# tum-vision/lsd_slam

Measured on AMD Instinct MI355X. Metric: tracked frames/sec (full track+map loop) at 640x480, frames resident in HBM (8-bit upload excluded: value_pcie_inclusive has it), higher is better.
Workload: dtype f32

## Files before the change

### lsd_slam_amd/csrc/lsdhip_internal.hpp

```cpp
#pragma once
#include <hip/hip_runtime.h>
#include <cmath>
#include <cstddef>
#include <cstdint>
#include <cstdio>
#include <cstring>
#include <mutex>
#include <string>
#include <vector>
#include "../../include/lsdhip.h"

#define LSD_LEVELS LSDHIP_PYRAMID_LEVELS
#define LSD_TRACK_MIN_LEVEL 1
#define LSD_TRACK_MAX_LEVEL 5
#define LSD_QUICK_KF_CHECK_LVL 4

void lsd_set_error(const char* fmt, ...);
#define HIPCHK(expr)                                                                       \
  do {                                                                                     \
    hipError_t e_ = (expr);                                                                \
    if (e_ != hipSuccess) {                                                                \
      lsd_set_error("%s failed: %s (%s:%d)", #expr, hipGetErrorString(e_), __FILE__, __LINE__); \
      return LSDHIP_E_HIP;                                                                 \
    }                                                                                      \
  } while (0)

#include "pose_math.hpp"

#include "rcp_exact.hpp"

struct LevelIntr { float fx, fy, cx, cy, fxi, fyi, cxi, cyi; };

#define RS_NUM 48
enum {
  RS_M = 0,
  RS_GOOD, RS_BAD, RS_SUMRES2, RS_SUMSIGNED, RS_SXX, RS_SYY, RS_SX, RS_SY, RS_SW, RS_USAGE,
  RS_WERR,
  RS_A0,
  RS_B0 = RS_A0 + 21,
  RS_ERR = RS_B0 + 6,
  RS_NREF,
  RS_END,
  RS_TOP0 = RS_END
};
static_assert(RS_TOP0 + 3 <= RS_NUM, "record too small");
static_assert(RS_END <= RS_NUM, "record too small");

struct TrackLevel {
  const float* kf_idepth;
  const float* kf_idepthVar;
  const float* kf_image;
  const uint8_t* kf_refBlk;
  const float4* fr_grad;
  const float* pts_pos;
  const float* pts_colvar;
  int npts;
  int w, h;
  int nblocks;
  int singlePass;
  int tilePx;
  float fx, fy, cx, cy, fxi, fyi, cxi, cyi;
  float lambdaInitial, stepSizeMin, convergenceEps;
  int maxIts;
  float minWarped;
  int writeMask;
};

struct TrackJob {
  TrackLevel lv[LSD_LEVELS];
  uint8_t* wasGood;
  float cameraPixelNoise2, var_weight, huber_half;
  float lambdaSuccessFac, lambdaFailFac;
  int useAffine;
  int lastLevel;
  int topLevel;
  lsdm::SE3fH T0;
  float aff_a0, aff_b0;
  int evalOnly;
  int trackFrameSemantics;
};
struct TrackSpec {
  int specC;
  int specGrid;
  int trials[LSD_LEVELS];
  uint8_t* wasGoodSide;
  unsigned maskStride;
  int seq;
  int copyMask;
  unsigned long long dbgCum;
  unsigned long long* dbgCounters;
  int last;
#ifdef LSD_PHASE_TRACE
  int traceWg;
#endif
#ifdef LSD_DEVTOOLS
  int* dbgLog;
#endif
};

#define LSD_SPEC_MAX 6
struct TrackState {
  lsdm::SE3fH T;
  lsdm::SE3fH Tn;
  float R[9], t[3];
  float aff_a, aff_b, aff_a_lastIt, aff_b_lastIt;
  float lastErr, LM_lambda, last_residual;
  int level, iteration, incTry, phase;
  int pending;
  float A[36], b[6];
  float inc[6];
  float bytes;
  int done, diverged;
  int numEvaluations, numWarpUpdates;
  float pointUsage, goodCount, badCount, meanRes;
  int levelEvals[LSD_LEVELS];
  int ncand;
  int lastCand;
  int numLaunches;
};

struct TrackSummary {
  int done;
  int diverged, level, numEvaluations, numWarpUpdates, pad_[3];
  float q[4], t[3];
  float lastResidual, pointUsage, goodCount, badCount, meanRes, aff_a, aff_b, aff_a_lastIt, aff_b_lastIt;
  float sums[RS_NUM];
  double bytes;
  int levelEvals[LSD_LEVELS];
  int numLaunches;
  int lastCand;
  int seq;
  int exhausted;
  unsigned check;
};
#define LSD_SUMMARY_CHECK_WORDS (offsetof(TrackSummary, seq) / 4)
__host__ __device__ static inline unsigned lsd_summary_term(unsigned i, unsigned bits) { return bits * (2u * i + 1u); }

struct DeferredSlot { double sum, count, flag, pad; };
#define LSD_NUM_SLOTS 256
#define LSD_DEFAULT_ASYNC 0
#define LSD_DEFAULT_PIPELINE 0
#define LSD_SPEC_TRIALS_SMALL 6
#define LSD_SPEC_SMALL_PX 6144
#define LSD_SPEC_TRIALS_MID 5
#define LSD_SPEC_MID_PX 90112
#define LSD_SPEC_CAP_WORKGROUPS 80
#define LSD_SPEC_CAP_ABOVE_PX 24576
#ifndef LSD_OBS_SPLIT_MIN_MAPS
#define LSD_OBS_SPLIT_MIN_MAPS 4
#endif
#define LSD_OBS_WALK_WAVES 4096
#define LSD_BATCH_THROUGHPUT_MIN_JOBS 8
#define LSD_BATCH_SPEC_MAX 4
#define LSD_BATCH_SPEC_PIXELS 500000
#define LSD_BATCH_STRIP_WORKGROUPS 768
struct lsdhip_frame;

#define LSD_CTX_LOCK(c) std::lock_guard<std::recursive_mutex> lsd_ctx_lock_((c)->mtx)
struct lsdhip_ctx {
  std::recursive_mutex mtx;
  int device = 0;
  bool async = LSD_DEFAULT_ASYNC != 0;
  DeferredSlot* h_slots = nullptr;
  lsdhip_frame* slot_stats_owner[LSD_NUM_SLOTS] = {};
  lsdhip_frame* slot_rescale_owner[LSD_NUM_SLOTS] = {};
  int slot_next = 0;
  long long enqEpoch = 0, doneEpoch = 0;
  long long slot_epoch[LSD_NUM_SLOTS] = {};
  int w = 0, h = 0;
  bool refBlocksWanted = false;
  int wl[LSD_LEVELS], hl[LSD_LEVELS];
  LevelIntr intr[LSD_LEVELS];
  float K0[9], K0inv[9];
  lsdhip_params params;
  hipStream_t stream = nullptr;
#define LSD_EVR 64
  bool pipeline = LSD_DEFAULT_PIPELINE != 0;
  hipStream_t mstream = nullptr;
  hipEvent_t mEv[LSD_EVR] = {};
  long long mSeq = 0;
  long long mDoneSeq = 0;
  long long tWaitedM = 0;
  long long slot_mseq[LSD_NUM_SLOTS] = {};
  struct PendingMerge { uint8_t* plane; const uint8_t* side; long long* doneSeq; };
  std::vector<PendingMerge> pendingMerges;
  unsigned long long* d_sums = nullptr;
  std::vector<int> sums_meta;
  std::vector<unsigned long long> sums_host;
  int* d_gate = nullptr;
  int gateSeq = 0, gateWaited = 0;
  static constexpr int MAX_LANES = 16;
  hipStream_t lanes[MAX_LANES] = {};
  hipEvent_t lane_done[MAX_LANES] = {};
  hipEvent_t lane_fork = nullptr;
  int lanes_open = 0;
  int lane_cur = -1;
  bool lane_used[MAX_LANES] = {};
  bool lane_record_pending = false;
  hipStream_t aux_stream = nullptr;
  unsigned* d_flagArrive = nullptr;
  hipEvent_t aux_fork = nullptr, aux_done = nullptr;
  bool aux_active = false, aux_pending = false;
  bool prof_on = false;
  unsigned prof_tick = 0;
  hipEvent_t ev_a = nullptr, ev_b = nullptr;
  bool prof_pending = false;
  double prof_ms = 0, prof_bytes = 0;
  long long prof_launches = 0;
  std::vector<hipEvent_t> prof_events;
#define LSD_BPROF_KINDS 5
#define LSD_BPROF_SLOTS 16
#define LSD_BPROF_PERIOD 3
  struct BProfSlot { hipEvent_t a = nullptr, b = nullptr; int kind = -1; double units = 0; bool pending = false; } bprof[LSD_BPROF_SLOTS];
  int bprof_next = 0;
  unsigned bprof_tick[LSD_BPROF_KINDS] = {};
  double bprof_ms[LSD_BPROF_KINDS] = {}, bprof_units[LSD_BPROF_KINDS] = {};
  long long bprof_calls[LSD_BPROF_KINDS] = {};
  unsigned long long* d_obsBatchAcc = nullptr;
  std::vector<void*> free_arenas;
  size_t arena_keep = 16;
  float* d_gtStage = nullptr;
  uint8_t* d_kfPoints = nullptr;
  struct ArgRing {
    static constexpr int NS = 32;
    uint8_t* h = nullptr; uint8_t* d = nullptr; size_t slotBytes = 0; int next = 0; hipEvent_t ev[NS] = {}; bool used[NS] = {};
    int cur = -1; size_t curBytes = 0;
    unsigned long long serial = 0, gen = 0;
  } args;
  struct BatchForm {
    int n = 0, py = 0, nSet = 0, walkWorkgroups = 0;
    bool split = false, candidates = false, synced = false;
    const int* qcountDev = nullptr;
    unsigned long long argsSerial = 0, argsGen = 0;
  } batchForm[2];
  std::vector<struct lsdhip_depthmap*> depthmaps;
  size_t arena_bytes = 0;
};

struct lsdhip_frame {
  lsdhip_ctx* ctx = nullptr;
  int id = 0;
  uint8_t* d_gray = nullptr;
  float* d_image[LSD_LEVELS] = {};
  float4* d_grad[LSD_LEVELS] = {};
  float* d_absgrad = nullptr;
  float* d_maxgrad = nullptr;
  float* d_idepth[LSD_LEVELS] = {};
  float* d_idepthVar[LSD_LEVELS] = {};
  bool hasIDepth = false;
  bool level0Ready = false;
  uint16_t* d_gradCand = nullptr;
  float gradCandTh = -1.0f;
  float* d_idepthW[LSD_LEVELS] = {};
  float* d_idepthVarW[LSD_LEVELS] = {};
  bool depthPending = false;
  long long depthPendingSeq = 0;
  long long depthSeq = 0;
  long long readySeq = 0;
  unsigned depthVersion = 0;
  uint8_t* d_refBlk[LSD_LEVELS] = {};
  uint8_t* d_refBlkW[LSD_LEVELS] = {};
  bool refBlkValid = false, refBlkValidW = false;
  uint8_t* d_wasGood = nullptr;
  bool wasGoodValid = false;
  bool wasGoodPristine = false;
  lsdm::Sim3dH thisToParent_raw;
  lsdhip_frame* trackingParent = nullptr;
  int trackingParentID = -1;
  float initialTrackedResidual = 0;
  int numFramesTrackedOnThis = 0, numMappedOnThis = 0, numMappedOnThisTotal = 0;
  float meanIdepth = 1;
  int numPoints = 0;
  int pendStats = -1;
  int pendRescale = -1;
  bool depthHasBeenUpdatedFlag = false;
  float* d_idepth_reAct = nullptr;
  float* d_idepthVar_reAct = nullptr;
  uint8_t* d_validity_reAct = nullptr;
  bool reActValid = false;
};

struct lsdhip_tracker {
  lsdhip_ctx* ctx = nullptr;
  float lambdaSuccessFac = 0.5f, lambdaFailFac = 2.0f;
  float lambdaInitial[LSD_LEVELS], stepSizeMin[LSD_LEVELS], convergenceEps[LSD_LEVELS];
  int maxItsPerLvl[LSD_LEVELS];
  float lambdaInitialTestTrack = 0, stepSizeMinTestTrack = 1e-3, convergenceEpsTestTrack = 0.98, maxItsTestTrack = 5;
  float huber_d = 3, var_weight = 1.0;
  float pointUsage = 0, lastGoodCount = 0, lastMeanRes = 0, lastBadCount = 0, lastResidual = 0;
  float affineEstimation_a = 1, affineEstimation_b = 0, affineEstimation_a_lastIt = 1, affineEstimation_b_lastIt = 0;
  bool diverged = false, trackingWasGood = false;
  int numEvaluations = 0, numWarpUpdates = 0;
  void (*enqueueHook)(void*) = nullptr;
  void* enqueueHookUser = nullptr;
  bool spinWait = true;
  bool hostLM = false;
  float* d_partials = nullptr;
  int max_blocks = 0;
  TrackState* d_state = nullptr;
  int levelEvaluations[LSD_LEVELS] = {};
  int block = 256;
  int grid_cap = 304;
  int recent[4] = {0, 0, 0, 0};
  int specC = 6;
  int soloMinJobs = -1;
  bool specAuto = true;
  int specCaps[LSD_LEVELS] = {0, 0, 0, 0, 0};
  int specLevel[LSD_LEVELS] = {0, 0, 0, 0, 0};
  int specCap = LSD_SPEC_CAP_WORKGROUPS;
  uint8_t* d_maskSide = nullptr;
  int maskSet = 0;
  long long maskMergeSeq[2] = {0, 0};
  size_t maskStride = 0;
  int numLaunches = 0;
  long long sumPolled = 0, sumLate = 0, sumLateMaxNs = 0, sumLateWords = 0;
  int sumLateFirstWord = -1, sumLateLastWord = -1;
  unsigned long long dbgCum = 0;
  std::vector<unsigned> dumpL0;
  unsigned long long* d_dbg = nullptr;
#ifdef LSD_DEVTOOLS
  int* d_log = nullptr;
  std::vector<int> lastLog;
#endif
  TrackSpec spec = {};
  const lsdhip_frame* jobKf = nullptr;
  unsigned jobKfVersion = 0;
  int jobTag = 0, launchOrdinal = 0;
  int budgetExtra = 2;
  int budgetFixed = 0;
  long long dbgJobs = 0, dbgEnqueued = 0, dbgMisses = 0, dbgWaitNs = 0, dbgLaunchNs = 0;
  TrackSummary* h_summary = nullptr;
  TrackSummary* d_summary = nullptr;
  unsigned long long* d_trace = nullptr;
  int batch_capacity = 0;
  TrackJob* d_bjobs = nullptr;
  TrackJob* h_bjobs = nullptr;
  TrackState* d_bstate = nullptr;
  float* d_bscratch = nullptr;
  int batchRecent[4] = {0, 0, 0, 0};
  int batchTag = 1;
  TrackSummary* h_bsummary = nullptr;
  float* d_pts = nullptr;
  int pts_capacity = 0;
};

#ifdef __HIP_DEVICE_COMPILE__
#define LSD_G __attribute__((address_space(1)))
#else
#define LSD_G
#endif
template <typename T> __host__ __device__ inline LSD_G T* lsd_g(T* p) { return (LSD_G T*)p; }
struct HypPlanes {
  LSD_G uint8_t* valid;
  LSD_G int32_t* blacklisted;
  LSD_G float* nextID;
  LSD_G int32_t* validity;
  LSD_G float* idepth;
  LSD_G float* var;
  LSD_G float* idepth_s;
  LSD_G float* var_s;
};

struct StereoRef {
  LSD_G const float* image;
  LSD_G const uint8_t* wasGood;
  int parentIsKF;
  int id;
  float initialTrackedResidual;
  float K_otherToThis_R[9];
  float K_otherToThis_t[3];
  float otherToThis_t[3];
  float thisToOther_t[3];
  float row0[3], row1[3], row2[3];
};

struct lsdhip_depthmap {
  lsdhip_ctx* ctx = nullptr;
  HypPlanes cur;
  HypPlanes oth;
  uint8_t* d_validSnap = nullptr;
  void* bases[3] = {nullptr, nullptr, nullptr};
  lsdhip_frame* activeKeyFrame = nullptr;
  bool activeKeyFrameIsReactivated = false;
  char* h_stage = nullptr;
  char* d_stage = nullptr;
  size_t stage_bytes = 0;
  int* d_slotCount = nullptr;
  int* d_slots = nullptr;
  int* d_ovfHead = nullptr;
  int2* d_ovf = nullptr;
  float4* d_cand = nullptr;
  int* d_flags = nullptr;
  double* d_red = nullptr;
  size_t redStride = 0;
  bool propClean = false;
  bool lowGradHypPossible = true;
  double* h_red = nullptr;
  hipEvent_t ev[8][2] = {};
  int ev_kind[8] = {};
  bool ev_pending[8] = {};
  int ev_next = 0;
  unsigned long long* d_obs_trace = nullptr;
  size_t obs_trace_words = 0;
  double gpu_ms[4] = {0, 0, 0, 0};
  long long gpu_calls[4] = {0, 0, 0, 0};
  unsigned obs_tick = 0;
  unsigned long long* d_obsCounters = nullptr;
  unsigned long long* d_obsAcc = nullptr;
  int obsCounterWaves = 0;
  float4* d_obsQueue = nullptr;
  unsigned ev_tick[3] = {0, 0, 0};
  float msUpdate = 0, msCreate = 0, msFinalize = 0, msObserve = 0, msRegularize = 0, msPropagate = 0, msFillHoles = 0,
        msSetDepth = 0;
};

inline hipStream_t lsd_transport_stream(lsdhip_ctx* c) { return c->aux_active ? c->aux_stream : c->stream; }
inline hipStream_t lsd_map_stream(lsdhip_ctx* c) { return c->lane_cur >= 0 ? c->lanes[c->lane_cur] : (c->pipeline ? c->mstream : c->stream); }
int lsd_m_begin(lsdhip_ctx* c);
long long lsd_m_record(lsdhip_ctx* c);
int lsd_t_wait_m(lsdhip_ctx* c, long long seq);
bool lsd_m_done(lsdhip_ctx* c, long long seq);
int lsd_sync_all(lsdhip_ctx* c);
struct LsdDevBuf {
  void* p = nullptr;
  ~LsdDevBuf() { if (p) (void)hipFree(p); }
};
#ifdef LSD_DEVTOOLS
int lsd_gate_wait(lsdhip_ctx* c);
int lsd_gate_open(lsdhip_ctx* c);
int lsd_pipe_dummy(lsdhip_ctx* c);
void lsd_trace_sum(lsdhip_ctx* c, hipStream_t s, int kind, int id, const void* p, size_t bytes);
void lsd_trace_val(lsdhip_ctx* c, int kind, int id, unsigned long long v);
#else
inline int lsd_gate_wait(lsdhip_ctx*) { return LSDHIP_OK; }
inline int lsd_gate_open(lsdhip_ctx*) { return LSDHIP_OK; }
inline int lsd_pipe_dummy(lsdhip_ctx*) { return LSDHIP_OK; }
inline void lsd_trace_sum(lsdhip_ctx*, hipStream_t, int, int, const void*, size_t) {}
inline void lsd_trace_val(lsdhip_ctx*, int, int, unsigned long long) {}
#endif
inline float** lsd_depth_w(lsdhip_frame* f) { return f->ctx->pipeline ? f->d_idepthW : f->d_idepth; }
inline float** lsd_depthvar_w(lsdhip_frame* f) { return f->ctx->pipeline ? f->d_idepthVarW : f->d_idepthVar; }
inline uint8_t** lsd_refblk_w(lsdhip_frame* f) { return f->ctx->pipeline ? f->d_refBlkW : f->d_refBlk; }
inline int lsd_gradcand_groups(int pixels) { return (pixels + 1023) >> 10; }
inline size_t lsd_gradcand_bytes(int pixels) { return ((size_t)lsd_gradcand_groups(pixels) * 1024 + (size_t)lsd_gradcand_groups(pixels)) * 2; }
inline int lsd_refblk_blocks(int pixels) { return (pixels + 255) >> 8; }
inline size_t lsd_refblk_bytes(int pixels) { return (size_t)lsd_refblk_blocks(pixels) * (256 + 4); }
inline float** lsd_depth_latest(lsdhip_frame* f) { return f->depthPending ? f->d_idepthW : f->d_idepth; }
inline float** lsd_depthvar_latest(lsdhip_frame* f) { return f->depthPending ? f->d_idepthVarW : f->d_idepthVar; }
int lsd_frame_publish_depth(lsdhip_frame* f);
int lsd_flush_merges(lsdhip_ctx* c);
struct LsdTrackJobScope {
  lsdhip_ctx* c;
  int rc = LSDHIP_OK;
  bool drain;
  LsdTrackJobScope(lsdhip_ctx* c_, bool waitAll) : c(c_), drain(waitAll) { if (c->pipeline && waitAll) rc = lsd_t_wait_m(c, c->mSeq); }
  ~LsdTrackJobScope() { if (c->pipeline && drain) (void)hipStreamSynchronize(c->stream); }
};
int lsd_frame_build_pyramids(lsdhip_frame* f, const uint8_t* src, hipStream_t stream);
int lsd_frames_require_ref_blocks(lsdhip_frame** kfs, int n, hipStream_t stream);
int lsd_frames_require_level0(lsdhip_frame** fs, int n);
int lsd_frame_require_level0(lsdhip_frame* f);
int lsd_frame_require_level0_for_tracking(lsdhip_frame* f);
int lsd_args_push(lsdhip_ctx* c, const void* src, size_t bytes, hipStream_t s, void** dev_out);
int lsd_args_begin(lsdhip_ctx* c, size_t bytes, void** host_out, void** dev_out);
int lsd_args_commit(lsdhip_ctx* c, hipStream_t s);
int lsd_args_release(lsdhip_ctx* c, const void* dev, hipStream_t s);
int lsd_frame_build_idepth_pyramid_batch(lsdhip_frame** f, int n, const double* const* redPartials, int redN, double* const* redOut,
                                         const int* redNs = nullptr);
int lsd_frame_build_idepth_pyramid(lsdhip_frame* f, const double* redPartials = nullptr, int redN = 0, double* redOut = nullptr);
int lsd_frame_ensure_depth_planes(lsdhip_frame* f);
int lsd_frame_ensure_wasgood(lsdhip_frame* f);
void lsd_depthmaps_forget_frame(lsdhip_ctx* c, lsdhip_frame* f);
int lsd_prof_collect(lsdhip_ctx* c);
int lsd_bprof_begin(lsdhip_ctx* c, int kind, hipStream_t s);
int lsd_bprof_end(lsdhip_ctx* c, int slot, hipStream_t s, double units);
int lsd_frame_resolve(lsdhip_frame* f);
int lsd_ctx_take_slot(lsdhip_ctx* c);
int lsd_ctx_claim_stats_slot(lsdhip_ctx* c, lsdhip_frame* f);
int lsd_ctx_claim_rescale_slot(lsdhip_ctx* c, lsdhip_frame* f);
```

### lsd_slam_amd/csrc/track_device.hpp

```cpp
#pragma once
#include "lsdhip_internal.hpp"
#include <type_traits>

template <int CTRL, int ROW_MASK, int BANK_MASK>
__device__ __forceinline__ float dpp_f(float v) {
  return __builtin_bit_cast(float, __builtin_amdgcn_update_dpp(0, __builtin_bit_cast(int, v), CTRL, ROW_MASK, BANK_MASK, true));
}
__device__ __forceinline__ int dpp_max_i(int a, int b) { return a > b ? a : b; }
template <int CTRL, int ROW_MASK, int BANK_MASK>
__device__ __forceinline__ int dpp_i(int v) {
  return __builtin_amdgcn_update_dpp(-1, v, CTRL, ROW_MASK, BANK_MASK, false);
}
template <int CTRL, int ROW_MASK, int BANK_MASK>
__device__ __forceinline__ int dpp_i0(int v) {
  return __builtin_amdgcn_update_dpp(0, v, CTRL, ROW_MASK, BANK_MASK, true);
}
__device__ __forceinline__ int wave_max_to_lane63(int v) {
  int t = dpp_max_i(v, dpp_i<0x111, 0xf, 0xf>(v));
  t = dpp_max_i(t, dpp_i<0x112, 0xf, 0xf>(v));
  t = dpp_max_i(t, dpp_i<0x113, 0xf, 0xf>(v));
  t = dpp_max_i(t, dpp_i<0x114, 0xf, 0xe>(t));
  t = dpp_max_i(t, dpp_i<0x118, 0xf, 0xc>(t));
  t = dpp_max_i(t, dpp_i<0x142, 0xa, 0xf>(t));
  t = dpp_max_i(t, dpp_i<0x143, 0xc, 0xf>(t));
  return t;
}
__device__ __forceinline__ float wave_sum_to_lane63(float v) {
  float t = v + dpp_f<0x111, 0xf, 0xf>(v);
  t = t + dpp_f<0x112, 0xf, 0xf>(v);
  t = t + dpp_f<0x113, 0xf, 0xf>(v);
  t = t + dpp_f<0x114, 0xf, 0xe>(t);
  t = t + dpp_f<0x118, 0xf, 0xc>(t);
  t = t + dpp_f<0x142, 0xa, 0xf>(t);
  t = t + dpp_f<0x143, 0xc, 0xf>(t);
  return t;
}

__device__ __forceinline__ void block_top3(int c0, int c1, int c2, int (*s_wave)[3], int* s_out) {
  const int tid = threadIdx.x, wave = tid >> 6, lane = tid & 63;
#pragma unroll
  for (int r = 0; r < 3; r++) {
    int m = __builtin_amdgcn_readlane(wave_max_to_lane63(c0), 63);
    if (lane == 0) s_wave[wave][r] = m;
    if (c0 == m && m >= 0) { c0 = c1; c1 = c2; c2 = -1; }
  }
  __syncthreads();
  if (wave == 0) {
    const int nw = blockDim.x >> 6;
    int v = (lane < nw * 3) ? s_wave[lane / 3][lane % 3] : -1;
#pragma unroll
    for (int r = 0; r < 3; r++) {
      int m = __builtin_amdgcn_readlane(wave_max_to_lane63(v), 63);
      if (lane == 0) s_out[r] = m;
      if (v == m) v = -1;
    }
  }
  __syncthreads();
}
__device__ __forceinline__ constexpr int tri_index(int r, int c) { return RS_A0 + r * 6 - (r * (r - 1)) / 2 + (c - r); }

__device__ __forceinline__ void top3_insert(int k, int& c0, int& c1, int& c2) {
  const int n0 = max(c0, k);
  int t = min(c0, k);
  const int n1 = max(c1, t);
  t = min(c1, t);
  c2 = max(c2, t);
  c1 = n1;
  c0 = n0;
}

typedef const __attribute__((address_space(1))) float gfloat;
typedef float v4f __attribute__((ext_vector_type(4)));
typedef const __attribute__((address_space(1))) v4f gv4f;
typedef __attribute__((address_space(1))) uint8_t gbyte;
struct EvalCtx {
  gfloat* kf_idepth;
  gfloat* kf_idepthVar;
  gfloat* kf_image;
  gfloat* fr_grad;
  gfloat* pts_pos;
  gfloat* pts_colvar;
  int npts, w, h;
  float fx, fy, cx, cy, fxi, fyi, cxi, cyi;
  float R[9], t[3];
  float aff_a, aff_b;
  float cameraPixelNoise2, var_weight, huber_half;
};
struct PointOut {
  bool in_image;
  bool good;
  float res, c1, c2, hw;
  float usage;
  float werr;
  float w;
  float J[6];
};

struct PointWarp { float Wx, Wy, Wz, u_new, v_new; bool in_image; };
struct Texel3 { float x, y, z; };
struct PointTexels { Texel3 t00, t10, t01, t11; };
__device__ __forceinline__ void eval_warp(const EvalCtx& a, float px, float py, float pz, PointWarp& q) {
  q.Wx = ((a.R[0] * px + a.R[1] * py) + a.R[2] * pz) + a.t[0];
  q.Wy = ((a.R[3] * px + a.R[4] * py) + a.R[5] * pz) + a.t[1];
  q.Wz = ((a.R[6] * px + a.R[7] * py) + a.R[8] * pz) + a.t[2];
  q.u_new = (q.Wx / q.Wz) * a.fx + a.cx;
  q.v_new = (q.Wy / q.Wz) * a.fy + a.cy;
  q.in_image = (q.u_new > 1 && q.v_new > 1 && q.u_new < a.w - 2 && q.v_new < a.h - 2);
}
__device__ __forceinline__ void eval_fetch(const EvalCtx& a, const PointWarp& q, bool fetch, PointTexels& t) {
  const int ix = fetch ? (int)q.u_new : 0;
  const int iy = fetch ? (int)q.v_new : 0;
  gfloat* bp = a.fr_grad + 4 * (ix + __mul24(iy, a.w));
  auto ld = [](gfloat* f) { Texel3 r = {f[0], f[1], f[2]}; return r; };
  t.t00 = ld(bp); t.t10 = ld(bp + 4); t.t01 = ld(bp + 4 * a.w); t.t11 = ld(bp + 4 + 4 * a.w);
}
#ifndef LSD_EVAL_FMA
#define LSD_EVAL_FMA 1
#endif
__device__ __forceinline__ float frcp(float x) { return __builtin_amdgcn_rcpf(x); }
__device__ __forceinline__ float fsqrt(float x) { return __builtin_amdgcn_sqrtf(x); }
__device__ __forceinline__ void eval_finish(const EvalCtx& a, const PointWarp& q, const PointTexels& t, float pz, float I_ref, float var,
                                            PointOut& o) {
  const float Wx = q.Wx, Wy = q.Wy, Wz = q.Wz, u_new = q.u_new, v_new = q.v_new;
  const Texel3 t00 = t.t00, t10 = t.t10, t01 = t.t01, t11 = t.t11;
  int ix = (int)u_new;
  int iy = (int)v_new;
  float dx = u_new - ix;
  float dy = v_new - iy;
  float dxdy = dx * dy;
  float w11 = dxdy, w01 = dy - dxdy, w10 = dx - dxdy, w00 = 1 - dx - dy + dxdy;
  float rx = w11 * t11.x + w01 * t01.x + w10 * t10.x + w00 * t00.x;
  float ry = w11 * t11.y + w01 * t01.y + w10 * t10.y + w00 * t00.y;
  float rz = w11 * t11.z + w01 * t01.z + w10 * t10.z + w00 * t00.z;

  float c1 = a.aff_a * I_ref + a.aff_b;
  float c2 = rz;
  float residual = c1 - c2;
  o.res = residual; o.c1 = c1; o.c2 = c2;
  o.hw = fabsf(residual) < 5.0f ? 1 : 5.0f * frcp(fabsf(residual));
  o.good = residual * residual < (40.0f * 40.0f + 0.5f * 0.5f * (rx * rx + ry * ry));
  float gx = a.fx * rx;
  float gy = a.fy * ry;
  float d = frcp(pz);
  float z = frcp(Wz);
  float depthChange = pz * z;
  o.usage = depthChange < 1 ? depthChange : 1;

  float pz2d = frcp((Wz * Wz) * d);
#if LSD_EVAL_FMA
  float g0 = __builtin_fmaf(Wz, a.t[0], 0.0f - Wx * a.t[2]) * pz2d;
  float g1 = __builtin_fmaf(Wz, a.t[1], 0.0f - Wy * a.t[2]) * pz2d;
  float drpdd = __builtin_fmaf(g0, gx, g1 * gy);
  float w_p = frcp(__builtin_fmaf(drpdd, drpdd * (a.var_weight * var), a.cameraPixelNoise2));
#else
  float g0 = (Wz * a.t[0] - Wx * a.t[2]) * pz2d;
  float g1 = (Wz * a.t[1] - Wy * a.t[2]) * pz2d;
  float drpdd = g0 * gx + g1 * gy;
  float w_p = frcp(a.cameraPixelNoise2 + drpdd * (drpdd * (a.var_weight * var)));
#endif
  float wr = residual * fsqrt(w_p);
  wr = fmaxf(wr, 0.0f - wr);
  float wh = (wr < a.huber_half) ? 1.0f : a.huber_half * frcp(wr);
  o.werr = wh * (wr * wr);
  o.w = wh * w_p;

  o.J[0] = z * gx;
  o.J[1] = z * gy;
  float v1 = (Wx * gy) * z;
  float v2 = (Wy * gx) * z;
  o.J[5] = v1 - v2;
  float z2 = z * z;
  v1 = (Wx * gx) * z2;
  v2 = (Wy * gy) * z2;
  o.J[2] = 0.0f - (v1 + v2);
#if LSD_EVAL_FMA
  o.J[3] = 0.0f - __builtin_fmaf(v2, Wy, __builtin_fmaf(v1, Wy, gy));
  o.J[4] = __builtin_fmaf(v2, Wx, __builtin_fmaf(v1, Wx, gx));
#else
  o.J[3] = 0.0f - ((v2 * Wy) + (gy + v1 * Wy));
  o.J[4] = (gx + v1 * Wx) + v2 * Wx;
#endif
}
__device__ __forceinline__ void eval_point(const EvalCtx& a, float px, float py, float pz, float I_ref, float var, PointOut& o) {
  PointWarp q;
  eval_warp(a, px, py, pz, q);
  o.in_image = q.in_image;
  if (!o.in_image) return;
  PointTexels t;
  eval_fetch(a, q, true, t);
  eval_finish(a, q, t, pz, I_ref, var, o);
}

__device__ __forceinline__ bool fetch_point(const EvalCtx& a, int i, float& px, float& py, float& pz, float& I_ref,
                                            float& var, int& maskIdx) {
  if (a.npts >= 0) {
    if (i >= a.npts) return false;
    px = a.pts_pos[3 * i]; py = a.pts_pos[3 * i + 1]; pz = a.pts_pos[3 * i + 2];
    I_ref = a.pts_colvar[2 * i]; var = a.pts_colvar[2 * i + 1];
    maskIdx = -1;
    return true;
  }
  if (i >= a.w * a.h) return false;
  int x = i % a.w, y = i / a.w;
  if (x < 1 || x >= a.w - 1 || y < 1 || y >= a.h - 1) return false;
  var = a.kf_idepthVar[i];
  float id = a.kf_idepth[i];
  if (var <= 0 || id == 0) return false;
  float inv = lsd_rcp_exact(id);
  px = inv * (a.fxi * x + a.cxi);
  py = inv * (a.fyi * y + a.cyi);
  pz = inv * 1.0f;
  I_ref = a.kf_image[i];
  maskIdx = i;
  return true;
}

__device__ __forceinline__ void set_eval_pose(TrackState& s, const lsdm::SE3fH& T) {
  s.Tn = T;
  lsdm::quatf_to_rot(T.q, s.R);
  s.t[0] = T.t[0]; s.t[1] = T.t[1]; s.t[2] = T.t[2];
}
__device__ __forceinline__ float rl(float v, int l) { return __int_as_float(__builtin_amdgcn_readlane(__float_as_int(v), l)); }
__device__ __forceinline__ int rli(int v, int l) { return __builtin_amdgcn_readlane(v, l); }

__device__ __forceinline__ void gj6_solve_wave(const float* A , const float* bvec , const float damp, float* s_m ,
                                               const int lane, float (&x)[6]) {
  const int i = lane >> 3, j = lane & 7;
  const bool act = i < 6 && j < 7;
  const int ii = act ? i : 0, jj = act ? (j < 6 ? j : 0) : 0;
  float m = (j == 6) ? -bvec[ii] : A[ii * 6 + jj];
  if (i == j) m *= damp;
#pragma unroll
  for (int k = 0; k < 6; k++) {
    if (act) s_m[i * 8 + j] = m;
    __builtin_amdgcn_fence(__ATOMIC_RELEASE, "wavefront");
    __builtin_amdgcn_wave_barrier();
    __builtin_amdgcn_fence(__ATOMIC_ACQUIRE, "wavefront");
    const float d = s_m[k * 8 + k], rk = s_m[k * 8 + (act ? j : 0)], ck = s_m[ii * 8 + k];
    const float f = ck * frcp(d);
    const float upd = m - f * rk;
    m = (i == k || d == 0.0f) ? m : upd;
    __builtin_amdgcn_wave_barrier();
  }
  if (act) s_m[i * 8 + j] = m;
  __builtin_amdgcn_fence(__ATOMIC_RELEASE, "wavefront");
  __builtin_amdgcn_wave_barrier();
  __builtin_amdgcn_fence(__ATOMIC_ACQUIRE, "wavefront");
#pragma unroll
  for (int r = 0; r < 6; r++) {
    const float d = s_m[r * 8 + r];
    x[r] = d != 0.0f ? s_m[r * 8 + 6] * frcp(d) : 0.0f;
  }
}

__device__ __forceinline__ void sincos_small(const float xx, float* sn, float* cs) {
  if (fabsf(xx) < 0.5f) {
    const float x2 = xx * xx;
    *sn = xx * (1.0f + x2 * (-1.0f / 6.0f + x2 * (1.0f / 120.0f + x2 * (-1.0f / 5040.0f + x2 * (1.0f / 362880.0f + x2 * (-1.0f / 39916800.0f))))));
    *cs = 1.0f + x2 * (-0.5f + x2 * (1.0f / 24.0f + x2 * (-1.0f / 720.0f + x2 * (1.0f / 40320.0f + x2 * (-1.0f / 3628800.0f + x2 * (1.0f / 479001600.0f))))));
  } else {
    sincosf(xx, sn, cs);
  }
}

__device__ __forceinline__ void q_normalize_wave(lsdm::Quatf& q, const int lane) {
  const float rn = __builtin_amdgcn_rsqf(q.x * q.x + q.y * q.y + q.z * q.z + q.w * q.w);
  const float c = (lane & 3) == 0 ? q.w : ((lane & 3) == 1 ? q.x : ((lane & 3) == 2 ? q.y : q.z));
  const float r = c * rn;
  q.w = rl(r, 0); q.x = rl(r, 1); q.y = rl(r, 2); q.z = rl(r, 3);
}

__device__ __forceinline__ lsdm::SE3fH se3f_exp_wave(const float (&a)[6], const int lane) {
  const float eps = static_cast<float>(1e-5);
  const float ox = a[3], oy = a[4], oz = a[5];
  const float theta_sq = ox * ox + (oy * oy + oz * oz);
  const float theta = fsqrt(theta_sq);
  const float half_theta = 0.5f * theta;
  float sn, cs;
  sincos_small((lane & 1) ? theta : half_theta, &sn, &cs);
  const float sin_half = rl(sn, 0), cos_half = rl(cs, 0), sin_theta = rl(sn, 1), cos_theta = rl(cs, 1);
  float imag, real;
  if (theta < eps) {
    const float theta_po4 = theta_sq * theta_sq;
    imag = 0.5f - static_cast<float>(1.0 / 48.0) * theta_sq + static_cast<float>(1.0 / 3840.0) * theta_po4;
    real = 1.0f - 0.5f * theta_sq + static_cast<float>(1.0 / 384.0) * theta_po4;
  } else {
    imag = sin_half * frcp(theta);
    real = cos_half;
  }
  lsdm::SE3fH r;
  r.q = {real, imag * ox, imag * oy, imag * oz};
  q_normalize_wave(r.q, lane);
  const float Om[9] = {0, -oz, oy, oz, 0, -ox, -oy, ox, 0};
  float Om2[9];
#pragma unroll
  for (int i = 0; i < 3; i++)
#pragma unroll
    for (int j = 0; j < 3; j++) {
      float acc = Om[i * 3 + 0] * Om[0 * 3 + j];
      acc += Om[i * 3 + 1] * Om[1 * 3 + j];
      acc += Om[i * 3 + 2] * Om[2 * 3 + j];
      Om2[i * 3 + j] = acc;
    }
  float V[9];
  if (theta < eps) {
    lsdm::q_to_rot<lsdm::Quatf, float>(r.q, V);
  } else {
    const float tsq = theta * theta;
    const float ca = (1.0f - cos_theta) * frcp(tsq);
    const float cb = (theta - sin_theta) * frcp(tsq * theta);
#pragma unroll
    for (int i = 0; i < 9; i++) V[i] = (((i % 4) == 0 ? 1.0f : 0.0f) + ca * Om[i]) + cb * Om2[i];
  }
#pragma unroll
  for (int i = 0; i < 3; i++) {
    float acc = V[i * 3 + 0] * a[0];
    acc += V[i * 3 + 1] * a[1];
    acc += V[i * 3 + 2] * a[2];
    r.t[i] = acc;
  }
  return r;
}
__device__ __forceinline__ lsdm::SE3fH se3f_mul_wave(const lsdm::SE3fH& a, const lsdm::SE3fH& b, const int lane) {
  lsdm::SE3fH r = a;
  float rt[3];
  lsdm::q_rotate<lsdm::Quatf, float>(a.q, b.t, rt);
#pragma unroll
  for (int i = 0; i < 3; i++) r.t[i] = a.t[i] + rt[i];
  r.q = lsdm::q_mul(a.q, b.q);
  q_normalize_wave(r.q, lane);
  return r;
}

__device__ __forceinline__ void write_summary(const TrackState& s, const float* tot, TrackSummary* out, const int doneWord) {
  unsigned chk = (unsigned)doneWord;
#define SUM_PUT_I(field, value) do { const int v_ = (value); out->field = v_; chk += lsd_summary_term((unsigned)(offsetof(TrackSummary, field) / 4), (unsigned)v_); } while (0)
#define SUM_PUT_F(field, value) do { const float v_ = (value); out->field = v_; chk += lsd_summary_term((unsigned)(offsetof(TrackSummary, field) / 4), __float_as_uint(v_)); } while (0)
#define SUM_PUT_IA(field, i, value) do { const int v_ = (value); out->field[i] = v_; chk += lsd_summary_term((unsigned)(offsetof(TrackSummary, field) / 4 + (i)), (unsigned)v_); } while (0)
#define SUM_PUT_FA(field, i, value) do { const float v_ = (value); out->field[i] = v_; chk += lsd_summary_term((unsigned)(offsetof(TrackSummary, field) / 4 + (i)), __float_as_uint(v_)); } while (0)
  SUM_PUT_I(diverged, s.diverged); SUM_PUT_I(level, s.level); SUM_PUT_I(numEvaluations, s.numEvaluations); SUM_PUT_I(numWarpUpdates, s.numWarpUpdates);
  SUM_PUT_IA(pad_, 0, 0); SUM_PUT_IA(pad_, 1, 0); SUM_PUT_IA(pad_, 2, 0);
  SUM_PUT_FA(q, 0, s.T.q.w); SUM_PUT_FA(q, 1, s.T.q.x); SUM_PUT_FA(q, 2, s.T.q.y); SUM_PUT_FA(q, 3, s.T.q.z);
  SUM_PUT_FA(t, 0, s.T.t[0]); SUM_PUT_FA(t, 1, s.T.t[1]); SUM_PUT_FA(t, 2, s.T.t[2]);
  SUM_PUT_F(lastResidual, s.last_residual); SUM_PUT_F(pointUsage, s.pointUsage); SUM_PUT_F(goodCount, s.goodCount); SUM_PUT_F(badCount, s.badCount);
  SUM_PUT_F(meanRes, s.meanRes); SUM_PUT_F(aff_a, s.aff_a); SUM_PUT_F(aff_b, s.aff_b); SUM_PUT_F(aff_a_lastIt, s.aff_a_lastIt); SUM_PUT_F(aff_b_lastIt, s.aff_b_lastIt);
  for (int i = 0; i < RS_NUM; i++) SUM_PUT_FA(sums, i, tot[i]);
  {
    const double b = (double)s.bytes;
    out->bytes = b;
    const unsigned long long u = (unsigned long long)__double_as_longlong(b);
    chk += lsd_summary_term((unsigned)(offsetof(TrackSummary, bytes) / 4), (unsigned)u) + lsd_summary_term((unsigned)(offsetof(TrackSummary, bytes) / 4 + 1), (unsigned)(u >> 32));
  }
  for (int l = 0; l < LSD_LEVELS; l++) SUM_PUT_IA(levelEvals, l, s.levelEvals[l]);
  SUM_PUT_I(numLaunches, s.numLaunches);
  SUM_PUT_I(lastCand, s.lastCand);
#undef SUM_PUT_I
#undef SUM_PUT_F
#undef SUM_PUT_IA
#undef SUM_PUT_FA
  out->check = chk;
  __threadfence_system();
  out->done = doneWord;
}

struct LmShared {
  float gj[48];
  float tot[RS_NUM];
};
struct LmPar {
  float lambdaInitial, stepSizeMin, convergenceEps, minWarped, lambdaSuccessFac, lambdaFailFac;
  int maxIts, w, h, writeMask, evalOnly, useAffine, tfSemantics, lastLevel, trials;
};
__device__ __forceinline__ void stage_lm_par(const TrackJob& job, int level, LmPar& p, const int trials = 1) {
  const TrackLevel& L = job.lv[level];
  LmPar v;
  v.lambdaInitial = L.lambdaInitial; v.stepSizeMin = L.stepSizeMin; v.convergenceEps = L.convergenceEps; v.minWarped = L.minWarped;
  v.lambdaSuccessFac = job.lambdaSuccessFac; v.lambdaFailFac = job.lambdaFailFac;
  v.maxIts = L.maxIts; v.w = L.w; v.h = L.h; v.writeMask = L.writeMask; v.evalOnly = job.evalOnly; v.useAffine = job.useAffine;
  v.tfSemantics = job.trackFrameSemantics; v.lastLevel = job.lastLevel;
  v.trials = trials;
  p = v;
}

#ifdef LSD_PHASE_TRACE
#define LM_MARK(k) do { if (trp && lane == 0) trp[k] = clock64(); } while (0)
#else
#define LM_MARK(k) do { } while (0)
#endif
__device__ __forceinline__ float lm_werr(float sumWeightedErr, int M) { return sumWeightedErr * frcp((float)((M >> 2) << 2)); }
__device__ __forceinline__ float lm_lambda_fail(float LM_lambda, int incTry, float lambdaFailFac) {
  if (LM_lambda == 0) return 0.2f;
  double p = 1.0;
  for (int i = 0; i < incTry; i++) p *= (double)lambdaFailFac;
  return (float)((double)LM_lambda * p);
}
template <bool SPEC = false>
__device__ __forceinline__ bool lm_wave(const LmPar& par, TrackState& S, const float col, float* tot, const int lane,
                                        TrackSummary* out, unsigned long long* trp, const int consumed = 0, const int mycand = 0, const int doneWord = 1) {
  float* const s_gj = tot - 48;
  S.lastCand = consumed;
  S.ncand = 1;
  const LmPar L = par;
  const int maxIts = L.maxIts;
  const int M = (int)rl(col, RS_M);
  const float refNum = rl(col, RS_NREF);
  const float goodCount = rl(col, RS_GOOD), badCount = rl(col, RS_BAD);
  float aff_a_lastIt, aff_b_lastIt;
  {
    const float sxx = rl(col, RS_SXX), syy = rl(col, RS_SYY), sx = rl(col, RS_SX), sy = rl(col, RS_SY), sw = rl(col, RS_SW);
    const float isw = frcp(sw);
    aff_a_lastIt = fsqrt((syy - sy * sy * isw) * frcp(sxx - sx * sx * isw));
    aff_b_lastIt = (sy - aff_a_lastIt * sx) * isw;
  }
  S.pointUsage = rl(col, RS_USAGE) * frcp(refNum);
  S.goodCount = goodCount;
  S.badCount = badCount;
  S.meanRes = rl(col, RS_SUMSIGNED) * frcp(goodCount);
  S.aff_a_lastIt = aff_a_lastIt;
  S.aff_b_lastIt = aff_b_lastIt;
  S.numEvaluations = S.numEvaluations + 1;
  if (lane == 0) S.levelEvals[S.level] = S.levelEvals[S.level] + 1;
  {
    const float N = refNum, wh = (float)L.w * (float)L.h;
    const float texels = 4.0f * N < wh ? 4.0f * N : wh;
    S.bytes = S.bytes + (20.0f * N + (L.writeMask ? 5.0f * N : 0.0f) + 12.0f * texels);
  }
  S.pending = 0;
  LM_MARK(12);
  if (L.evalOnly) { S.done = 1; if (out && lane == 0) write_summary(S, tot, out, doneWord); return false; }

  if (M < L.minWarped) {
    S.diverged = 1; S.done = 1;
    if (out && lane == 0) write_summary(S, tot, out, doneWord);
    return false;
  }
  const float werr = lm_werr(rl(col, RS_WERR), M);
  const bool useAffine = L.useAffine != 0;
  const bool tfSemantics = L.tfSemantics != 0;

  float LM_lambda = S.LM_lambda, lastErr = S.lastErr;
  int iteration = S.iteration, incTry = S.incTry;
  lsdm::SE3fH T = S.T;
  bool propose = false, start_iteration = false, accepted = false, rejected = false;
  if (S.phase == 0) {
    accepted = true;
    lastErr = werr;
    LM_lambda = L.lambdaInitial;
    iteration = 0;
    start_iteration = true;
  } else {
    const float error = werr;
    if (error < lastErr) {
      accepted = true;
      T = S.Tn;
      S.T = T;
      if (error > L.convergenceEps * lastErr) iteration = maxIts;
      lastErr = error;
      if (tfSemantics) S.last_residual = error;
      if (LM_lambda <= 0.2) LM_lambda = 0;
      else LM_lambda *= L.lambdaSuccessFac;
      iteration++;
      start_iteration = true;
    } else {
      const float i0 = S.inc[0], i1 = S.inc[1], i2 = S.inc[2], i3 = S.inc[3], i4 = S.inc[4], i5 = S.inc[5];
      const float incdot = (i0 * i0 + (i1 * i1 + i2 * i2)) + (i3 * i3 + (i4 * i4 + i5 * i5));
      if (!(incdot > L.stepSizeMin)) {
        iteration = maxIts;
        iteration++;
        start_iteration = true;
      } else {
        LM_lambda = lm_lambda_fail(LM_lambda, incTry, L.lambdaFailFac);
        propose = true;
        rejected = true;
      }
    }
  }
  if (accepted) {
    if (useAffine) { S.aff_a = aff_a_lastIt; S.aff_b = aff_b_lastIt; }
    const float rn = frcp((float)((size_t)6 * (size_t)(M >> 2)));
    const int k = lane - RS_A0;
    if (k >= 0 && k < 21) {
      const int i = (k >= 6) + (k >= 11) + (k >= 15) + (k >= 18) + (k >= 20);
      const int j = k - (i * 6 - (i * (i - 1)) / 2) + i;
      const float v = (0.0f + col) * rn;
      S.A[i * 6 + j] = v;
      S.A[j * 6 + i] = v;
    }
    if (lane >= RS_B0 && lane < RS_B0 + 6) S.b[lane - RS_B0] = (0.0f - col) * rn;
  }
  if (start_iteration && iteration < maxIts) { S.numWarpUpdates = S.numWarpUpdates + 1; incTry = 0; propose = true; }
  S.lastErr = lastErr;
  S.LM_lambda = LM_lambda;
  S.iteration = iteration;
  LM_MARK(13);
  if (propose) {
    const int extra = SPEC ? mycand : 0;
    for (int j = 0; j < extra; j++) { incTry++; LM_lambda = lm_lambda_fail(LM_lambda, incTry, L.lambdaFailFac); }
    S.ncand = L.trials;
    float inc[6];
    const float damp = 1 + LM_lambda;
    LM_MARK(14);
    gj6_solve_wave(S.A, S.b, damp, s_gj, lane, inc);
    LM_MARK(15);
    S.incTry = incTry + 1;
#pragma unroll
    for (int i = 0; i < 6; i++) S.inc[i] = inc[i];
    const lsdm::SE3fH Tn = se3f_mul_wave(se3f_exp_wave(inc, lane), T, lane);
    S.Tn = Tn;
    float R[9];
    lsdm::quatf_to_rot(Tn.q, R);
#pragma unroll
    for (int i = 0; i < 9; i++) S.R[i] = R[i];
    S.t[0] = Tn.t[0]; S.t[1] = Tn.t[1]; S.t[2] = Tn.t[2];
    S.phase = 1;
    LM_MARK(16);
    return true;
  }
  S.incTry = incTry;
  if (!tfSemantics) S.last_residual = lastErr;
  if (S.level == L.lastLevel) {
    S.done = 1;
    if (out && lane == 0) write_summary(S, tot, out, doneWord);
  } else {
    S.level = S.level - 1;
    S.phase = 0;
    S.Tn = T;
    float R[9];
    lsdm::quatf_to_rot(T.q, R);
#pragma unroll
    for (int i = 0; i < 9; i++) S.R[i] = R[i];
    S.t[0] = T.t[0]; S.t[1] = T.t[1]; S.t[2] = T.t[2];
  }
  return false;
}

__device__ __forceinline__ void accumulate_point(const PointOut& o, float (&acc)[RS_END]) {
  acc[RS_M] += 1.f;
  acc[RS_SXX] = __builtin_fmaf(o.c1 * o.c1, o.hw, acc[RS_SXX]);
  acc[RS_SYY] = __builtin_fmaf(o.c2 * o.c2, o.hw, acc[RS_SYY]);
  acc[RS_SX] = __builtin_fmaf(o.c1, o.hw, acc[RS_SX]);
  acc[RS_SY] = __builtin_fmaf(o.c2, o.hw, acc[RS_SY]);
  acc[RS_SW] += o.hw;
  if (o.good) { acc[RS_GOOD] += 1.f; acc[RS_SUMRES2] = __builtin_fmaf(o.res, o.res, acc[RS_SUMRES2]); acc[RS_SUMSIGNED] += o.res; }
  else acc[RS_BAD] += 1.f;
  acc[RS_USAGE] += o.usage;
  acc[RS_WERR] += o.werr;
#pragma unroll
  for (int r = 0; r < 6; r++) {
    float Jw = o.J[r] * o.w;
#pragma unroll
    for (int c = r; c < 6; c++) acc[tri_index(r, c)] = __builtin_fmaf(Jw, o.J[c], acc[tri_index(r, c)]);
  }
  float resw = o.res * o.w;
#pragma unroll
  for (int r = 0; r < 6; r++) acc[RS_B0 + r] = __builtin_fmaf(resw, o.J[r], acc[RS_B0 + r]);
  acc[RS_ERR] = __builtin_fmaf(resw, o.res, acc[RS_ERR]);
}

__device__ __forceinline__ void make_ctx_dev(const TrackJob& jobr, const TrackState& S, int level, EvalCtx& a) {
  const TrackJob* job = &jobr;
  const TrackLevel& L = job->lv[level];
  a.kf_idepth = (gfloat*)L.kf_idepth; a.kf_idepthVar = (gfloat*)L.kf_idepthVar; a.kf_image = (gfloat*)L.kf_image; a.fr_grad = (gfloat*)L.fr_grad;
  a.pts_pos = (gfloat*)L.pts_pos; a.pts_colvar = (gfloat*)L.pts_colvar; a.npts = L.npts; a.w = L.w; a.h = L.h;
  a.fx = L.fx; a.fy = L.fy; a.cx = L.cx; a.cy = L.cy; a.fxi = L.fxi; a.fyi = L.fyi; a.cxi = L.cxi; a.cyi = L.cyi;
#pragma unroll
  for (int i = 0; i < 9; i++) a.R[i] = S.R[i];
#pragma unroll
  for (int i = 0; i < 3; i++) a.t[i] = S.t[i];
  a.aff_a = S.aff_a; a.aff_b = S.aff_b;
  a.cameraPixelNoise2 = job->cameraPixelNoise2; a.var_weight = job->var_weight; a.huber_half = job->huber_half;
}

template <int N>
__device__ __forceinline__ void copy_words(void* dst, const void* src, int tid, int nthreads) {
  const unsigned* s = (const unsigned*)src;
  unsigned* d = (unsigned*)dst;
  for (int i = tid; i < N; i += nthreads) d[i] = s[i];
}

__device__ __forceinline__ int xcd_tile(int b, int nb) { return (nb & 7) == 0 ? (b & 7) * (nb >> 3) + (b >> 3) : b; }


#define RS_COLS 44
struct TrackScratch {
  float* sums;
  int4* topkey;
  float* topval;
  int max_rows;
  int cmax;
  float* recs;
#ifdef LSD_PHASE_TRACE
  unsigned long long* trace;
#endif
};
```

### lsd_slam_amd/csrc/tracker.hip

```cpp
#include <atomic>
#include <chrono>
#include "track_device.hpp"


#ifdef LSD_PHASE_TRACE
#define PHASE_MARK(k) do { if (trOn_ && threadIdx.x == 0) tr_[k] = clock64(); } while (0)
#define LSD_TRACE_WORDS 32
#else
#define PHASE_MARK(k) do { } while (0)
#endif

#ifdef LSD_DEVTOOLS
#define LAUNCH_LOG(exitCode, pendingIn, ncandIn, pcUsed) do { \
    if (!BATCH && MODE == TS_FUSED && blockIdx.x == 0 && threadIdx.x == 0 && spec.dbgLog && spec.seq != 0) { \
      int* lg_ = spec.dbgLog + ((spec.seq & 0xFFF) * 16); \
      lg_[0] = spec.seq; lg_[1] = (exitCode); lg_[2] = parity | (first << 1) | (spec.last << 2); lg_[3] = lvlIn_; lg_[4] = (pendingIn); lg_[5] = (ncandIn); \
      lg_[6] = (pcUsed); lg_[7] = S.level; lg_[8] = S.numEvaluations; lg_[9] = S.numLaunches; lg_[10] = S.done; lg_[11] = S.phase; lg_[12] = S.incTry; \
      lg_[13] = S.ncand; lg_[14] = S.pending; lg_[15] = numLaunchesIn_; } } while (0)
#else
#define LAUNCH_LOG(exitCode, pendingIn, ncandIn, pcUsed) do { } while (0)
#endif

enum { TS_FUSED = 0, TS_LM = 1, TS_EVAL = 2 };
__device__ __forceinline__ void track_state_begin(TrackState& S, const TrackJob& job, const int tid) {
  if (tid == 0) {
    S.T = job.T0;
    set_eval_pose(S, job.T0);
    S.aff_a = job.aff_a0; S.aff_b = job.aff_b0; S.aff_a_lastIt = job.aff_a0; S.aff_b_lastIt = job.aff_b0;
    S.lastErr = 0; S.LM_lambda = 0; S.last_residual = 0;
    S.level = job.topLevel; S.iteration = 0; S.incTry = 0; S.phase = 0; S.pending = 0;
    S.done = 0; S.diverged = 0; S.numEvaluations = 0; S.numWarpUpdates = 0;
    S.pointUsage = 0; S.goodCount = 0; S.badCount = 0; S.meanRes = 0;
    S.bytes = 0;
    for (int l = 0; l < LSD_LEVELS; l++) S.levelEvals[l] = 0;
    S.ncand = 1; S.lastCand = 0; S.numLaunches = 0;
  }
  if (tid < 36) S.A[tid] = 0;
  if (tid < 6) { S.b[tid] = 0; S.inc[tid] = 0; }
}
__device__ __forceinline__ void tail_row(const PointOut& o, float* row) {
  row[0] = o.werr;
  int k = 1;
#pragma unroll
  for (int rr = 0; rr < 6; rr++) {
    const float Jw = o.J[rr] * o.w;
#pragma unroll
    for (int cc = rr; cc < 6; cc++) row[k++] = Jw * o.J[cc];
  }
  const float resw = o.res * o.w;
#pragma unroll
  for (int rr = 0; rr < 6; rr++) row[k++] = resw * o.J[rr];
  row[k++] = resw * o.res;
}

template <int BLOCK, bool BATCH, int MODE>
__device__ __forceinline__ void track_step_impl(const TrackJob& jobv, const TrackJob* __restrict__ jobs, TrackState* __restrict__ st2,
                                                TrackScratch sc, TrackSummary* __restrict__ out, int parity, int first, const TrackSpec& spec) {
  const TrackJob& job = BATCH ? jobs[blockIdx.y] : jobv;
  unsigned warm = 0;
  if (!BATCH) {
    typedef const unsigned __attribute__((address_space(4))) cuint;
    cuint* ka = (cuint*)__builtin_amdgcn_kernarg_segment_ptr();
#pragma unroll
    for (int i = 0; i < (int)(sizeof(TrackJob) / 4); i += 32) warm ^= ka[i];
    asm volatile("" ::"s"(warm));
  }
  if (BATCH) {
    const size_t j = blockIdx.y, rows = (size_t)sc.max_rows, cm = (size_t)sc.cmax;
    st2 += 2 * j;
    out += j;
    sc.sums += j * 2 * cm * RS_COLS * rows;
    sc.topkey += j * 2 * cm * rows;
    sc.topval += j * 2 * cm * rows * 96;
    if (sc.recs) sc.recs += j * 2 * cm * 32;
  }
  constexpr int WAVES = BLOCK / 64;
  constexpr int SUMW = WAVES - 1;
  constexpr int NSLICE = (SUMW * 64) / RS_END;
  constexpr int QMAX = 20;
  __shared__ TrackState S;
  __shared__ LmShared sh;
  __shared__ LmPar s_par;
  constexpr int NPASS = 1;
  constexpr int CPP = (RS_END + NPASS - 1) / NPASS;
  constexpr int RSLICE_ = BLOCK / CPP;
  __shared__ float s_sum[(NSLICE > RSLICE_ ? NSLICE : RSLICE_)][64];
  __shared__ __attribute__((aligned(16))) float s_red[CPP * (BLOCK + 1) + 8];
  __shared__ int s_wtop[WAVES][3];
  __shared__ int s_top[3];
  const int tid = threadIdx.x;
  const int wave = tid >> 6, lane = tid & 63;
  const int max_rows = sc.max_rows;
  int cand = 0, bx = (int)blockIdx.x;
  const bool leader = blockIdx.x == 0;
  const int cmax = sc.cmax;
  TrackState* next = st2 + (1 - parity);
  const int outp = MODE == TS_EVAL ? parity : 1 - parity;
  const float* sums_in0 = sc.sums + (size_t)parity * cmax * RS_COLS * max_rows;
  float* sums_out = sc.sums + (size_t)outp * cmax * RS_COLS * max_rows;
  const int4* topkey_in0 = sc.topkey + (size_t)parity * cmax * max_rows;
  int4* topkey_out = sc.topkey + (size_t)outp * cmax * max_rows;
  const float* topval_in0 = sc.topval + (size_t)parity * cmax * max_rows * 96;
  float* topval_out = sc.topval + (size_t)outp * cmax * max_rows * 96;
  constexpr int NSLOT = 16;
  constexpr int TRIALS_MAX = BATCH ? (MODE == TS_EVAL ? 1 : LSD_BATCH_SPEC_MAX) : LSD_SPEC_MAX;
  constexpr bool SPEC_LM = MODE != TS_EVAL;
  static_assert(TRIALS_MAX * (NSLOT * RS_COLS + 96 + 1) <= CPP * (BLOCK + 1) + 8, "the finishing phase's tables must fit the reduction buffer");
  float (*const s_sumT)[NSLOT][RS_COLS] = (float (*)[NSLOT][RS_COLS])s_red;
  float (*const s_subT)[3][32] = (float (*)[3][32])(s_red + TRIALS_MAX * NSLOT * RS_COLS);
  int* const s_nsubT = (int*)(s_red + TRIALS_MAX * (NSLOT * RS_COLS + 96));
  __shared__ float s_rec[TRIALS_MAX][32];
#ifdef LSD_PHASE_TRACE
  __shared__ unsigned long long* s_trp;
  unsigned long long* tr_ = sc.trace;
  const bool trOn_ = sc.trace != nullptr && (int)blockIdx.x == (BATCH ? spec.traceWg : 0) && (!BATCH || blockIdx.y == 0);
  if (trOn_ && tid == 0) {
    unsigned long long n = sc.trace[0];
    sc.trace[0] = n + 1;
    tr_ = sc.trace + 1 + (n % 4096) * LSD_TRACE_WORDS;
    for (int k = 0; k < LSD_TRACE_WORDS; k++) tr_[k] = 0;
    tr_[8] = wall_clock64();
    tr_[24] = (unsigned long long)gridDim.x; tr_[25] = (unsigned long long)gridDim.y;
    s_trp = tr_;
  }
#endif
  PHASE_MARK(0);
  if (!BATCH && MODE == TS_FUSED && !first && !leader && st2[parity].done) return;
  if (!BATCH && MODE == TS_FUSED && leader && tid == 0 && spec.seq != 0) out->seq = spec.seq;
  if (first) {
    track_state_begin(S, job, tid);
  } else {
    copy_words<sizeof(TrackState) / 4>(&S, st2 + parity, tid, BLOCK);
    if (SPEC_LM && cmax > 1 && tid < 32 * TRIALS_MAX) (&s_rec[0][0])[tid] = sc.recs[(size_t)parity * cmax * 32 + (tid < 32 * cmax ? tid : 0)];
  }
  __syncthreads();
  PHASE_MARK(1);
#ifdef LSD_DEVTOOLS
  const int lvlIn_ = S.level, numLaunchesIn_ = S.numLaunches, pendingIn_ = S.pending, ncandIn_ = S.ncand;
  int pcLog_ = -1;
#endif
  if (S.done) {
    LAUNCH_LOG(1, pendingIn_, ncandIn_, -1);
    if (MODE != TS_EVAL && leader) { copy_words<sizeof(TrackState) / 4>(next, &S, tid, BLOCK); }
    return;
  }
  const int lvlPending = S.level;
  const int doneWord = (MODE == TS_FUSED && spec.seq != 0) ? (BATCH ? spec.seq : (spec.seq >> 12)) : 1;
  if (MODE == TS_FUSED) {
    const int nbl = job.lv[lvlPending].nblocks;
    const int tr = (spec.specC > 1 && spec.trials[lvlPending] > 1) ? spec.trials[lvlPending] : 1;
    cand = (int)blockIdx.x / nbl;
    bx = (int)blockIdx.x - cand * nbl;
    const bool needTrial = S.pending ? cand < tr : cand == 0;
    const bool needNext = S.pending && lvlPending > job.lastLevel && (int)blockIdx.x < job.lv[lvlPending - 1].nblocks;
    if (!leader && !needTrial && !needNext) return;
  }

  if (BATCH && MODE == TS_LM) {
    cand = (int)blockIdx.x;
    bx = 0;
    const int tr = (spec.specC > 1 && spec.trials[lvlPending] > 1) ? spec.trials[lvlPending] : 1;
    if (!leader && !(S.pending && cand < tr)) return;
  }
  if (BATCH && MODE == TS_EVAL) {
    const int nbl = job.lv[lvlPending].nblocks;
    cand = (int)blockIdx.x / nbl;
    bx = (int)blockIdx.x - cand * nbl;
  }

  constexpr int CHMAX = 8;
  int cntv = 0;
  unsigned ow[CHMAX];
  auto strip_request = [&](const int lvl, const int tile_) {
    const TrackLevel& L = job.lv[lvl];
    const int px = L.w * L.h;
    const int base_ = tile_ * L.tilePx;
    const int b0_ = base_ >> 8;
    const int mblk_ = (min(base_ + L.tilePx, px) - base_ + 255) >> 8;
    const gbyte* offs = (const gbyte*)L.kf_refBlk;
    const __attribute__((address_space(1))) int* cnts = (const __attribute__((address_space(1))) int*)(offs + ((size_t)((px + 255) >> 8) << 8));
    cntv = lane < mblk_ ? cnts[b0_ + lane] : 0;
#pragma unroll
    for (int c = 0; c < CHMAX; c++) {
      const int blk = c * 4 + wave;
      ow[c] = blk < mblk_ ? *(const __attribute__((address_space(1))) unsigned*)(offs + ((size_t)(b0_ + blk) << 8) + (lane << 2)) : 0u;
    }
  };
  bool havePre = false;
  if (BATCH && MODE == TS_FUSED && S.pending && job.lv[lvlPending].tilePx > 0) {
    const int tr = (spec.specC > 1 && spec.trials[lvlPending] > 1) ? spec.trials[lvlPending] : 1;
    havePre = cand < tr;
    if (havePre) strip_request(lvlPending, xcd_tile(bx, job.lv[lvlPending].nblocks));
  }

  if (MODE != TS_EVAL && S.pending) {
    const int ncandPending = S.ncand < 1 ? 1 : (S.ncand > TRIALS_MAX ? TRIALS_MAX : S.ncand);
    const int level = S.level;
    const int nb = job.lv[level].nblocks;
    const size_t trialStrideF4 = (size_t)RS_COLS * max_rows / 4;
      auto tail_two = [&](const int ca, const int cb, auto krn) {
        constexpr int KROWS = decltype(krn)::value;
        const int cbb = cb < 0 ? ca : cb;
        const int4* tka = topkey_in0 + (size_t)ca * max_rows;
        const int4* tkb = topkey_in0 + (size_t)cbb * max_rows;
        int4 kva[KROWS], kvb[KROWS];
#pragma unroll
        for (int q = 0; q < KROWS; q++) {
          const int row = lane + 64 * q;
          const int4 ka = tka[row < max_rows ? row : 0];
          const int4 kb = tkb[row < max_rows ? row : 0];
          kva[q] = row < nb ? ka : make_int4(-1, -1, -1, -1);
          kvb[q] = row < nb ? kb : make_int4(-1, -1, -1, -1);
        }
        auto merge = [&](const int4 (&kv)[KROWS], int (&keys)[3], int (&src)[3]) {
          int k0 = -1, k1 = -1, k2 = -1, e0 = 0, e1 = 0, e2 = 0;
#pragma unroll
          for (int q = 0; q < KROWS; q++) {
            const int e = (lane + 64 * q) * 3;
            const int ks[3] = {kv[q].x, kv[q].y, kv[q].z};
#pragma unroll
            for (int rr = 0; rr < 3; rr++) {
              const int k = ks[rr], ek = e + rr;
              const bool g0 = k > k0, g1 = k > k1, g2 = k > k2;
              k2 = g1 ? k1 : (g2 ? k : k2); e2 = g1 ? e1 : (g2 ? ek : e2);
              k1 = g0 ? k0 : (g1 ? k : k1); e1 = g0 ? e0 : (g1 ? ek : e1);
              k0 = g0 ? k : k0; e0 = g0 ? ek : e0;
            }
          }
#pragma unroll
          for (int r = 0; r < 3; r++) {
            const int m = __builtin_amdgcn_readlane(wave_max_to_lane63(k0), 63);
            const unsigned long long own = __ballot(k0 == m && m >= 0);
            const int owner = own ? (int)__ffsll((long long)own) - 1 : 0;
            keys[r] = m;
            src[r] = __builtin_amdgcn_readlane(e0, owner);
            if (k0 == m && m >= 0) { k0 = k1; e0 = e1; k1 = k2; e1 = e2; k2 = -1; }
          }
        };
        const bool single = job.lv[level].singlePass != 0 || job.lv[level].tilePx > 0;
        const int j = lane & 31, rj = lane >> 5;
        int keysA[3], srcA[3], keysB[3], srcB[3];
        float a0 = 0.f, a2 = 0.f, b0 = 0.f, b2 = 0.f;
        merge(kva, keysA, srcA);
        if (single && j < 29) {
          const float* tv = topval_in0 + (size_t)ca * max_rows * 96;
          if (keysA[rj] >= 0) a0 = tv[(size_t)srcA[rj] * 32 + j];
          if (rj == 0 && keysA[2] >= 0) a2 = tv[(size_t)srcA[2] * 32 + j];
        }
        if (cb >= 0) {
          merge(kvb, keysB, srcB);
          if (single && j < 29) {
            const float* tv = topval_in0 + (size_t)cb * max_rows * 96;
            if (keysB[rj] >= 0) b0 = tv[(size_t)srcB[rj] * 32 + j];
            if (rj == 0 && keysB[2] >= 0) b2 = tv[(size_t)srcB[2] * 32 + j];
          }
        }
        if (lane == 0) {
          s_nsubT[ca] = (keysA[0] >= 0) + (keysA[1] >= 0) + (keysA[2] >= 0);
          if (cb >= 0) s_nsubT[cb] = (keysB[0] >= 0) + (keysB[1] >= 0) + (keysB[2] >= 0);
        }
        if (single) {
          if (j < 29) {
            if (keysA[rj] >= 0) s_subT[ca][rj][j] = a0;
            if (rj == 0 && keysA[2] >= 0) s_subT[ca][2][j] = a2;
            if (cb >= 0) {
              if (keysB[rj] >= 0) s_subT[cb][rj][j] = b0;
              if (rj == 0 && keysB[2] >= 0) s_subT[cb][2][j] = b2;
            }
          }
        } else {
          const bool second = lane >= 3;
          const int r = second ? lane - 3 : lane;
          const int c = second ? cb : ca;
          int key = -1;
          if (lane < 6 && c >= 0) key = second ? (r == 0 ? keysB[0] : (r == 1 ? keysB[1] : keysB[2])) : (r == 0 ? keysA[0] : (r == 1 ? keysA[1] : keysA[2]));
          if (key >= 0) {
            EvalCtx a;
            make_ctx_dev(job, S, level, a);
            if (c > 0) {
              const float* rec = s_rec[c];
#pragma unroll
              for (int i = 0; i < 9; i++) a.R[i] = rec[13 + i];
#pragma unroll
              for (int i = 0; i < 3; i++) a.t[i] = rec[22 + i];
            }
            const int idx = (a.npts >= 0) ? key : ((key / a.h) + (key % a.h) * a.w);
            float px, py, pz, I_ref, var;
            int maskIdx;
            fetch_point(a, idx, px, py, pz, I_ref, var, maskIdx);
            PointOut o;
            eval_point(a, px, py, pz, I_ref, var, o);
            float* sub = s_subT[c][r];
            sub[0] = o.werr;
            int k = 1;
#pragma unroll
            for (int rr = 0; rr < 6; rr++) {
              float Jw = o.J[rr] * o.w;
#pragma unroll
              for (int cc = rr; cc < 6; cc++) sub[k++] = Jw * o.J[cc];
            }
            float resw = o.res * o.w;
#pragma unroll
            for (int rr = 0; rr < 6; rr++) sub[k++] = resw * o.J[rr];
            sub[k++] = resw * o.res;
          }
        }
      };
      auto tail_rows = [&](const int ca, const int cb, auto nqn) {
        constexpr int NQ = decltype(nqn)::value;
        const int cbb = cb < 0 ? ca : cb;
        const float4* ta = (const float4*)(topval_in0 + (size_t)ca * max_rows * 96);
        const float4* tb = (const float4*)(topval_in0 + (size_t)cbb * max_rows * 96);
        const int nf4 = nb * 24;
        float4 va[NQ], vb[NQ];
#pragma unroll
        for (int q = 0; q < NQ; q++) {
          const int f = q * 64 + lane;
          va[q] = ta[f < nf4 ? f : 0];
          vb[q] = tb[f < nf4 ? f : 0];
        }
        auto pick = [&](const float4 (&v)[NQ], const int c) {
          int k0 = -1, k1 = -1, k2 = -1, e0 = 0, e1 = 0, e2 = 0;
#pragma unroll
          for (int q = 0; q < NQ; q++) {
            const int f = q * 64 + lane;
            const int k = ((lane & 7) == 7 && f < nf4) ? __float_as_int(v[q].w) : -1, ek = f >> 3;
            const bool g0 = k > k0, g1 = k > k1, g2 = k > k2;
            k2 = g1 ? k1 : (g2 ? k : k2); e2 = g1 ? e1 : (g2 ? ek : e2);
            k1 = g0 ? k0 : (g1 ? k : k1); e1 = g0 ? e0 : (g1 ? ek : e1);
            k0 = g0 ? k : k0; e0 = g0 ? ek : e0;
          }
          int nsub = 0;
#pragma unroll
          for (int r = 0; r < 3; r++) {
            const int m = __builtin_amdgcn_readlane(wave_max_to_lane63(k0), 63);
            const unsigned long long own = __ballot(k0 == m && m >= 0);
            const int owner = own ? (int)__ffsll((long long)own) - 1 : 0;
            const int row = __builtin_amdgcn_readlane(e0, owner);
            if (k0 == m && m >= 0) { k0 = k1; e0 = e1; k1 = k2; e1 = e2; k2 = -1; }
            if (m >= 0) {
              nsub++;
              const int qsel = row >> 3;
#pragma unroll
              for (int q = 0; q < NQ; q++) {
                if (q == qsel) {
                  float4 w4 = v[q];
                  asm volatile("" : "+v"(w4.x), "+v"(w4.y), "+v"(w4.z), "+v"(w4.w));
                  if ((lane >> 3) == (row & 7)) *(float4*)&s_subT[c][r][(lane & 7) * 4] = w4;
                }
              }
            }
          }
          if (lane == 0) s_nsubT[c] = nsub;
        };
        pick(va, ca);
        if (cb >= 0) pick(vb, cb);
      };
    auto wave_tail = [&]() {
      const int ca = WAVES - 1 - wave;
      const int cb = ca + WAVES < ncandPending ? ca + WAVES : -1;
      if (ca < ncandPending) {
        if (BATCH && job.lv[level].tilePx > 0 && nb <= 24) {
          if (nb <= 5) tail_rows(ca, cb, std::integral_constant<int, 2>());
          else if (nb <= 13) tail_rows(ca, cb, std::integral_constant<int, 5>());
          else tail_rows(ca, cb, std::integral_constant<int, 9>());
        } else if (nb <= 128) tail_two(ca, cb, std::integral_constant<int, 2>());
        else tail_two(ca, cb, std::integral_constant<int, 5>());
      }
    };
    if (tid == SUMW * 64 - 1) stage_lm_par(job, level, s_par, (spec.specC > 1 && spec.trials[level] > 1) ? spec.trials[level] : 1);
    if (wave < SUMW) {
      const int t = tid;
      const int slot_ = t / (RS_COLS / 4);
      const bool sumLane = slot_ < NSLOT;
      const int slot = sumLane ? slot_ : 0, c4 = sumLane ? t - slot_ * (RS_COLS / 4) : 0;
      {
        const int K = (nb + NSLOT - 1) / NSLOT;
        const float4* p = (const float4*)sums_in0 + c4;
        const size_t trialStrideF4 = (size_t)RS_COLS * max_rows / 4;
        auto colsum = [&](auto qn, auto ntn, const int base) {
          constexpr int Q = decltype(qn)::value, NT = decltype(ntn)::value;
          float4 v[NT][Q];
#pragma unroll
          for (int c = 0; c < NT; c++) {
            const int pc = base + c < ncandPending ? base + c : ncandPending - 1;
            const float4* pp = p + (size_t)pc * trialStrideF4;
#pragma unroll
            for (int q = 0; q < Q; q++) {
              const int r = slot + NSLOT * q;
              v[c][q] = pp[(size_t)(r < nb ? r : slot) * (RS_COLS / 4)];
            }
          }
#pragma unroll
          for (int c = 0; c < NT; c++) {
            float4 a4 = make_float4(0.f, 0.f, 0.f, 0.f);
#pragma unroll
            for (int q = 0; q < Q; q++) {
              const bool live = q < K && slot + NSLOT * q < nb;
              a4.x += live ? v[c][q].x : 0.f;
              a4.y += live ? v[c][q].y : 0.f;
              a4.z += live ? v[c][q].z : 0.f;
              a4.w += live ? v[c][q].w : 0.f;
            }
            if (sumLane && base + c < ncandPending) *(float4*)&s_sumT[base + c][slot][c4 * 4] = a4;
          }
        };
        typedef std::integral_constant<int, 1> I1;
        typedef std::integral_constant<int, 3> I3;
        typedef std::integral_constant<int, TRIALS_MAX> IM;
        if (ncandPending == 1) {
          if (K <= 2) colsum(std::integral_constant<int, 2>(), I1(), 0);
          else if (K <= 5) colsum(std::integral_constant<int, 5>(), I1(), 0);
          else if (K <= 10) colsum(std::integral_constant<int, 10>(), I1(), 0);
          else colsum(std::integral_constant<int, QMAX>(), I1(), 0);
        } else if (K <= 2) colsum(std::integral_constant<int, 2>(), IM(), 0);
        else if (K <= 5) colsum(std::integral_constant<int, 5>(), IM(), 0);
        else if (K <= 10) { for (int base = 0; base < ncandPending; base += 3) colsum(std::integral_constant<int, 10>(), I3(), base); }
        else { for (int base = 0; base < ncandPending; base++) colsum(std::integral_constant<int, QMAX>(), I1(), base); }
#ifdef LSD_PHASE_TRACE
        if (trOn_ && tid == 0) tr_[17] = clock64();
#endif
      }
    }
    wave_tail();
#ifdef LSD_PHASE_TRACE
    if (trOn_ && tid == SUMW * 64) s_trp[18] = clock64();
#endif
    __syncthreads();
    PHASE_MARK(2);
    if (wave == 0) {
      int pc = 0;
      if (ncandPending > 1) {
        const int c = tid < ncandPending ? tid : 0;
        float Mf = s_sumT[c][0][RS_M], ws = s_sumT[c][0][RS_WERR];
#pragma unroll
        for (int k = 1; k < NSLOT; k++) { Mf += s_sumT[c][k][RS_M]; ws += s_sumT[c][k][RS_WERR]; }
        const int Mc = (int)Mf;
        int needc = Mc & 3;
        if (needc > s_nsubT[c]) needc = s_nsubT[c];
        if (needc > 0) ws -= s_subT[c][0][0];
        if (needc > 1) ws -= s_subT[c][1][0];
        if (needc > 2) ws -= s_subT[c][2][0];
        const float werrc = lm_werr(ws, Mc);
        const float* ic = c == 0 ? S.inc : s_rec[c];
        const float i0 = ic[0], i1 = ic[1], i2 = ic[2], i3 = ic[3], i4 = ic[4], i5 = ic[5];
        const float incdot = (i0 * i0 + (i1 * i1 + i2 * i2)) + (i3 * i3 + (i4 * i4 + i5 * i5));
        const bool stop = Mc < s_par.minWarped || werrc < S.lastErr || !(incdot > s_par.stepSizeMin);
        const unsigned long long sm = __ballot(stop && tid < ncandPending);
        pc = sm ? (int)__ffsll((long long)sm) - 1 : ncandPending - 1;
        if (pc > 0) {
          float lam = S.LM_lambda;
          const int it0 = S.incTry;
          for (int j = 0; j < pc; j++) lam = lm_lambda_fail(lam, it0 + j, s_par.lambdaFailFac);
          float skipped;
          {
            float NR = s_sumT[0][0][RS_NREF];
#pragma unroll
            for (int k = 1; k < NSLOT; k++) NR += s_sumT[0][k][RS_NREF];
            const float wh = (float)s_par.w * (float)s_par.h;
            const float texels = 4.0f * NR < wh ? 4.0f * NR : wh;
            skipped = 20.0f * NR + (s_par.writeMask ? 5.0f * NR : 0.0f) + 12.0f * texels;
          }
          const float* rec = s_rec[pc];
          const float bytes0 = S.bytes;
          const int ne0 = S.numEvaluations, le0 = S.levelEvals[level];
          float bytes1 = bytes0;
          for (int j = 0; j < pc; j++) bytes1 = bytes1 + skipped;
          S.LM_lambda = lam;
          S.incTry = it0 + pc;
          S.numEvaluations = ne0 + pc;
          if (tid == 0) S.levelEvals[level] = le0 + pc;
          S.bytes = bytes1;
          if (tid < 6) S.inc[tid] = rec[tid];
          if (tid < 7) ((float*)&S.Tn)[tid] = rec[6 + tid];
          if (tid < 9) S.R[tid] = rec[13 + tid];
          if (tid < 3) S.t[tid] = rec[22 + tid];
        }
      }
      {
        float Mf = s_sumT[pc][0][RS_M];
#pragma unroll
        for (int k = 1; k < NSLOT; k++) Mf += s_sumT[pc][k][RS_M];
        float s = 0.f;
        if (tid < RS_END) {
          s = s_sumT[pc][0][tid];
#pragma unroll
          for (int k = 1; k < NSLOT; k++) s += s_sumT[pc][k][tid];
        }
        const int M = (int)Mf;
        int need = M & 3;
        if (need > s_nsubT[pc]) need = s_nsubT[pc];
        const int subIdx = (tid == RS_WERR) ? 0 : ((tid >= RS_A0 && tid < RS_B0) ? 1 + tid - RS_A0 : ((tid >= RS_B0 && tid < RS_ERR) ? 22 + tid - RS_B0 : (tid == RS_ERR ? 28 : -1)));
        const float sub0 = s_subT[pc][0][subIdx < 0 ? 0 : subIdx], sub1 = s_subT[pc][1][subIdx < 0 ? 0 : subIdx], sub2 = s_subT[pc][2][subIdx < 0 ? 0 : subIdx];
        if (subIdx >= 0) {
          if (need > 0) s -= sub0;
          if (need > 1) s -= sub1;
          if (need > 2) s -= sub2;
        }
        if (tid < RS_NUM) sh.tot[tid] = s;
#ifdef LSD_ORDER_CHECK
        if (!BATCH && spec.dbgCounters) {
          unsigned hv = tid < RS_END ? __float_as_uint(s) * (2654435761u * (unsigned)(tid + 1)) : 0u;
          hv += (unsigned)pc * 97u;
          for (int off = 32; off > 0; off >>= 1) hv += __shfl_xor(hv, off);
          if (tid == 0) {
            const unsigned long long slot = 8 + 2 * ((spec.dbgCum / 400ull) % 8192ull);
            __hip_atomic_fetch_min(&spec.dbgCounters[slot], (unsigned long long)hv, __ATOMIC_RELAXED, __HIP_MEMORY_SCOPE_AGENT);
            __hip_atomic_fetch_max(&spec.dbgCounters[slot + 1], (unsigned long long)hv, __ATOMIC_RELAXED, __HIP_MEMORY_SCOPE_AGENT);
          }
        }
#endif
        PHASE_MARK(3);
#ifdef LSD_PHASE_TRACE
        if (trOn_ && tid == 0) { tr_[19] = (unsigned long long)ncandPending; tr_[7] = (unsigned long long)pc; }
        lm_wave<SPEC_LM>(s_par, S, s, sh.tot, tid, leader ? out : nullptr, trOn_ ? tr_ : nullptr, pc, cand, doneWord);
#else
        lm_wave<SPEC_LM>(s_par, S, s, sh.tot, tid, leader ? out : nullptr, nullptr, pc, cand, doneWord);
#endif
      }
    }
    __syncthreads();
    PHASE_MARK(4);
    if (S.done) {
      if (!BATCH && MODE == TS_FUSED && S.lastCand > 0 && spec.copyMask != 0 && job.lv[level].writeMask && cand == 0 && bx < nb) {
        const uint8_t* side = spec.wasGoodSide + (size_t)(S.lastCand - 1) * spec.maskStride;
        EvalCtx a;
        make_ctx_dev(job, S, level, a);
        const int work = a.npts >= 0 ? a.npts : a.w * a.h;
        for (int i = bx * BLOCK + tid; i < work; i += nb * BLOCK) {
          float px, py, pz, I_ref, var;
          int maskIdx;
          if (fetch_point(a, i, px, py, pz, I_ref, var, maskIdx) && maskIdx >= 0) job.wasGood[maskIdx] = side[maskIdx];
        }
      }
      if (leader) copy_words<sizeof(TrackState) / 4>(next, &S, tid, BLOCK);
      LAUNCH_LOG(2, pendingIn_, ncandIn_, S.lastCand);
      return;
    }
    if (cand > 0 && bx == 0 && S.phase == 1 && cand < S.ncand && tid < 25) {
      float v;
      if (tid < 6) v = S.inc[tid];
      else if (tid < 13) v = ((const float*)&S.Tn)[tid - 6];
      else if (tid < 22) v = S.R[tid - 13];
      else v = S.t[tid - 22];
      sc.recs[((size_t)outp * cmax + cand) * 32 + tid] = v;
    }
  }

  if (MODE == TS_LM) {
    __syncthreads();
    if (tid == 0) { S.pending = 1; S.numLaunches = S.numLaunches + 1; }
    __syncthreads();
    if (leader) copy_words<sizeof(TrackState) / 4>(next, &S, tid, BLOCK);
    return;
  }

  const int level = S.level;
  const int nb = job.lv[level].nblocks;
  if (MODE == TS_FUSED && level != lvlPending) { cand = 0; bx = (int)blockIdx.x; }
  if (bx >= nb || cand >= S.ncand) return;
  sums_out += (size_t)cand * RS_COLS * max_rows;
  topkey_out += (size_t)cand * max_rows;
  topval_out += (size_t)cand * max_rows * 96;
  const int tile = xcd_tile(bx, nb);
  EvalCtx a;
  make_ctx_dev(job, S, level, a);
  if (BATCH && MODE == TS_EVAL && cand > 0) {
    const float* rec = sc.recs + ((size_t)parity * cmax + cand) * 32;
#pragma unroll
    for (int i = 0; i < 9; i++) a.R[i] = rec[13 + i];
#pragma unroll
    for (int i = 0; i < 3; i++) a.t[i] = rec[22 + i];
  }
  gbyte* wasGood = (gbyte*)(job.lv[level].writeMask ? (cand == 0 ? job.wasGood : spec.wasGoodSide + (size_t)(cand - 1) * spec.maskStride) : nullptr);
  const int work = a.npts >= 0 ? a.npts : a.w * a.h;
  float acc[RS_END];
#pragma unroll
  for (int k = 0; k < RS_END; k++) acc[k] = 0.f;
  int key0 = -1, key1 = -1, key2 = -1;

  if (BATCH && job.lv[level].tilePx > 0) {
    unsigned* s_list = (unsigned*)s_red;
    const int tilePx = job.lv[level].tilePx;
    const int base = tile * tilePx;
    const int stripEnd = min(base + tilePx, work);
    const int b0 = base >> 8;
    const int mblk = (stripEnd - base + 255) >> 8;
    const float inv_w = 1.0f / (float)a.w;
    if (!(havePre && level == lvlPending)) strip_request(level, tile);
    int incl = cntv + dpp_i0<0x111, 0xf, 0xf>(cntv);
    incl += dpp_i0<0x112, 0xf, 0xf>(cntv);
    incl += dpp_i0<0x113, 0xf, 0xf>(cntv);
    incl += dpp_i0<0x114, 0xf, 0xe>(incl);
    incl += dpp_i0<0x118, 0xf, 0xc>(incl);
    incl += dpp_i0<0x142, 0xa, 0xf>(incl);
    const int total = __builtin_amdgcn_readlane(incl, 31);
    const int waveU = __builtin_amdgcn_readfirstlane(wave);
    PHASE_MARK(20);
#pragma unroll
    for (int c = 0; c < CHMAX; c++) {
      const int blk = c * 4 + waveU;
      if (blk < mblk) {
        const int cb = __builtin_amdgcn_readlane(cntv, blk);
        const int pb = __builtin_amdgcn_readlane(incl, blk) - cb;
#pragma unroll
        for (int k = 0; k < 4; k++) {
          const int sl = lane + 64 * k;
          if (sl < cb) {
            const int i = ((b0 + blk) << 8) + (int)((ow[c] >> (8 * k)) & 255u);
            int y = (int)((float)i * inv_w);
            int x = i - y * a.w;
            if (x < 0) { y--; x += a.w; }
            if (x >= a.w) { y++; x -= a.w; }
            s_list[pb + sl] = (unsigned)x | ((unsigned)y << 16);
          }
        }
      }
    }
    __syncthreads();
    PHASE_MARK(21);
#ifdef LSD_PHASE_TRACE
    if (trOn_ && tid == 0) tr_[23] = (unsigned long long)total;
#endif
    if (total > 0) {
      struct StA { unsigned xy; float var, id, img; bool live; };
      struct StB { unsigned xy; float pz, I_ref, var; PointWarp q; PointTexels t; bool live; };
      auto stageA = [&](int p, StA& A) {
        A.live = p < total;
        A.xy = s_list[A.live ? p : 0];
        const int i = __mul24((int)(A.xy >> 16), a.w) + (int)(A.xy & 0xffffu);
        A.var = a.kf_idepthVar[i];
        A.id = a.kf_idepth[i];
        A.img = a.kf_image[i];
      };
      auto stageB = [&](const StA& A, StB& B) {
        B.live = A.live;
        B.xy = A.xy;
        const int bx_ = (int)(A.xy & 0xffffu), by_ = (int)(A.xy >> 16);
        const float inv = lsd_rcp_exact(A.id);
        const float px = inv * (a.fxi * bx_ + a.cxi), py = inv * (a.fyi * by_ + a.cyi);
        B.pz = inv * 1.0f;
        B.I_ref = A.img; B.var = A.var;
        eval_warp(a, px, py, B.pz, B.q);
        eval_fetch(a, B.q, B.live && B.q.in_image, B.t);
      };
      const int rounds = (total + BLOCK - 1) / BLOCK;
      StA A1, A2;
      StB B0, B1;
      stageA(tid, A1);
      stageB(A1, B0);
      stageA(tid + BLOCK, A1);
      PHASE_MARK(22);
      auto stageC = [&](const StB& B) {
        if (B.live) {
          const int x_ = (int)(B.xy & 0xffffu), y_ = (int)(B.xy >> 16);
          const int i = __mul24(y_, a.w) + x_;
          acc[RS_NREF] += 1.f;
          if (!B.q.in_image) {
            if (wasGood) wasGood[i] = 0;
          } else {
            PointOut o;
            eval_finish(a, B.q, B.t, B.pz, B.I_ref, B.var, o);
            if (wasGood) wasGood[i] = o.good ? 1 : 0;
            top3_insert(__mul24(x_, a.h) + y_, key0, key1, key2);
            accumulate_point(o, acc);
          }
        }
      };
      for (int r = 0; r < rounds; r += 2) {
        stageB(A1, B1);
        stageA(tid + (r + 2) * BLOCK, A2);
        stageC(B0);
        stageB(A2, B0);
        stageA(tid + (r + 3) * BLOCK, A1);
        stageC(B1);
      }
    }
    __syncthreads();
  } else
  for (int i = tile * BLOCK + tid; i < work; i += nb * BLOCK) {
    float px, py, pz, I_ref, var;
    int maskIdx;
    if (fetch_point(a, i, px, py, pz, I_ref, var, maskIdx)) {
      acc[RS_NREF] += 1.f;
      PointOut o;
      eval_point(a, px, py, pz, I_ref, var, o);
      if (!o.in_image) {
        if (wasGood && maskIdx >= 0) wasGood[maskIdx] = 0;
      } else {
        if (wasGood && maskIdx >= 0) wasGood[maskIdx] = o.good ? 1 : 0;
        top3_insert(a.npts >= 0 ? i : (i % a.w) * a.h + (i / a.w), key0, key1, key2);
        accumulate_point(o, acc);
      }
    }
  }

  PHASE_MARK(5);
#ifdef LSD_PHASE_TRACE
  if (trOn_ && tid == 0) { tr_[10] = (unsigned long long)level; tr_[11] = (unsigned long long)nb; tr_[26] = (unsigned long long)lvlPending; }
#endif
  constexpr int RSLICE = BLOCK / CPP;
  constexpr int RRUN = (BLOCK + RSLICE - 1) / RSLICE;
  const bool stripRows = BATCH && job.lv[level].tilePx > 0;
  const bool candLane = tid >= BLOCK - 64 && tid < BLOCK - 61;
  int cKey = -1, cX = 0, cY = 0;
  float cVar = 0.f, cId = 1.f, cImg = 0.f, cPz = 0.f;
  PointWarp cq;
  PointTexels ct;
  if (stripRows) {
    block_top3(key0, key1, key2, s_wtop, s_top);
    if (candLane) {
      cKey = s_top[tid - (BLOCK - 64)];
      if (cKey >= 0) {
        cX = cKey / a.h;
        cY = cKey - cX * a.h;
        const int ci = __mul24(cY, a.w) + cX;
        cVar = a.kf_idepthVar[ci];
        cId = a.kf_idepth[ci];
        cImg = a.kf_image[ci];
      }
    }
  }
#pragma unroll
  for (int hp = 0; hp < NPASS; hp++) {
    if (hp > 0) __syncthreads();
#pragma unroll
    for (int k = 0; k < CPP; k++)
      if (hp * CPP + k < RS_END) s_red[k * (BLOCK + 1) + tid] = acc[hp * CPP + k];
    __syncthreads();
    if (MODE == TS_FUSED && hp == 0 && tid == 0) { S.pending = 1; S.numLaunches = S.numLaunches + 1; }
    if (stripRows && hp == 0 && candLane && cKey >= 0) {
      const float inv = lsd_rcp_exact(cId);
      const float px = inv * (a.fxi * cX + a.cxi), py = inv * (a.fyi * cY + a.cyi);
      cPz = inv * 1.0f;
      eval_warp(a, px, py, cPz, cq);
      eval_fetch(a, cq, cq.in_image, ct);
    }
    {
      const int slice = tid / CPP, k = tid - slice * CPP;
      if (slice < RSLICE) {
        const float* row = s_red + k * (BLOCK + 1);
        const int j0 = slice * RRUN;
        float v[RRUN];
#pragma unroll
        for (int j = 0; j < RRUN; j++) v[j] = row[j0 + j];
        float s = 0.f;
#pragma unroll
        for (int j = 0; j < RRUN; j++) s += (j0 + j < BLOCK) ? v[j] : 0.f;
        s_sum[slice][k] = s;
      }
    }
    __syncthreads();
    if (stripRows && hp == 0 && candLane) {
      float* row = topval_out + (size_t)(tile * 3 + (tid - (BLOCK - 64))) * 32;
      if (cKey >= 0) {
        PointOut o;
        eval_finish(a, cq, ct, cPz, cImg, cVar, o);
        tail_row(o, row);
      }
      ((int*)row)[31] = cKey;
    }
    if (tid < CPP && hp * CPP + tid < RS_END) {
      float s = s_sum[0][tid];
#pragma unroll
      for (int sl = 1; sl < RSLICE; sl++) s += s_sum[sl][tid];
      sums_out[(size_t)tile * RS_COLS + (hp * CPP + tid)] = s;
    }
  }
  if (!stripRows) block_top3(key0, key1, key2, s_wtop, s_top);
  if (tid == 0) topkey_out[tile] = make_int4(s_top[0], s_top[1], s_top[2], -1);
  if (job.lv[level].singlePass && key0 >= 0) {
    const int r = key0 == s_top[0] ? 0 : (key0 == s_top[1] ? 1 : (key0 == s_top[2] ? 2 : -1));
    if (r >= 0) {
      float* dst = topval_out + (size_t)(tile * 3 + r) * 32;
      dst[0] = acc[RS_WERR];
#pragma unroll
      for (int k = 0; k < 21; k++) dst[1 + k] = acc[RS_A0 + k];
#pragma unroll
      for (int k = 0; k < 6; k++) dst[22 + k] = acc[RS_B0 + k];
      dst[28] = acc[RS_ERR];
    }
  }
  if (MODE == TS_FUSED && leader) copy_words<sizeof(TrackState) / 4>(next, &S, tid, BLOCK);
 
  if (MODE == TS_FUSED && leader && tid == 0 && spec.last != 0) out->exhausted = spec.seq;
  LAUNCH_LOG(3, pendingIn_, ncandIn_, S.lastCand);
  PHASE_MARK(6);
#ifdef LSD_PHASE_TRACE
  if (trOn_ && tid == 0) tr_[9] = wall_clock64();
#endif
}

template <int BLOCK, bool BATCH, int MODE = TS_FUSED>
__global__ __launch_bounds__(BLOCK) void k_track_step(TrackJob jobv, const TrackJob* __restrict__ jobs, TrackState* __restrict__ st2,
                                                       TrackScratch sc, TrackSummary* __restrict__ out, int parity, int first, TrackSpec spec) {
#ifdef LSD_ORDER_CHECK
  if (!BATCH && spec.dbgCounters && threadIdx.x == 0) {
    const unsigned long long fin = __hip_atomic_load(&spec.dbgCounters[0], __ATOMIC_RELAXED, __HIP_MEMORY_SCOPE_AGENT);
    if (fin < spec.dbgCum) {
      __hip_atomic_fetch_add(&spec.dbgCounters[1], 1ull, __ATOMIC_RELAXED, __HIP_MEMORY_SCOPE_AGENT);
      __hip_atomic_fetch_max(&spec.dbgCounters[2], spec.dbgCum - fin, __ATOMIC_RELAXED, __HIP_MEMORY_SCOPE_AGENT);
    }
  }
#endif
  track_step_impl<BLOCK, BATCH, MODE>(jobv, jobs, st2, sc, out, parity, first, spec);
#ifdef LSD_ORDER_CHECK
  __syncthreads();
  if (!BATCH && spec.dbgCounters && threadIdx.x == 0) __hip_atomic_fetch_add(&spec.dbgCounters[0], 1ull, __ATOMIC_RELEASE, __HIP_MEMORY_SCOPE_AGENT);
#endif
}

#define LSD_SOLO_MAX_PX 4800
#define LSD_SOLO_TRIPS 9
#define LSD_SOLO_MAX_PTS (LSD_SOLO_TRIPS * 512)
#define LSD_SOLO_LDS_PTS 4544
static_assert(LSD_SOLO_LDS_PTS <= LSD_SOLO_MAX_PTS, "every point of the LDS lists has a register slot");
constexpr int lsd_solo_max_interior() {
  int best = 0;
  for (int w = 3; w <= LSD_SOLO_MAX_PX / 3; w++) {
    const int h = LSD_SOLO_MAX_PX / w;
    if ((w - 2) * (h - 2) > best) best = (w - 2) * (h - 2);
  }
  return best;
}
static_assert(lsd_solo_max_interior() <= LSD_SOLO_LDS_PTS, "the dense interior of any level k_track_solo takes fits its LDS lists");
#define LSD_SOLO_MIN_JOBS 24
template <int BLOCK>
__global__ __launch_bounds__(BLOCK) void k_track_solo(const TrackJob* __restrict__ jobs, TrackState* __restrict__ st2, TrackSummary* __restrict__ outs,
                                                          const int parity, const int doneWord) {
  const TrackJob& job = jobs[blockIdx.x];
  st2 += 2 * (size_t)blockIdx.x;
  TrackSummary* out = outs + blockIdx.x;
  constexpr int WAVES = BLOCK / 64;
  constexpr int HALF = BLOCK / 2;
  constexpr int CPP = RS_END;
  constexpr int RSLICE = BLOCK / CPP;
  constexpr int RRUN = (HALF + RSLICE - 1) / RSLICE;
  constexpr int TRIPS = LSD_SOLO_TRIPS;
  static_assert(WAVES * 3 <= 64, "top-3 merge in one wave");
  static_assert((size_t)TRIPS * BLOCK * 4 <= sizeof(float) * (CPP * (HALF + 1) + RRUN), "the level's list borrows the reduction buffer");
  __shared__ TrackState S;
  __shared__ LmShared sh;
  __shared__ LmPar s_par;
  __shared__ __attribute__((aligned(16))) float s_red[CPP * (HALF + 1) + RRUN];
  __shared__ float s_sum[RSLICE][64];
  __shared__ float s_sub[3][32];
  __shared__ int s_wtop[WAVES][3];
  __shared__ v4f s_tex[LSD_SOLO_MAX_PX];
  __shared__ float s_var[LSD_SOLO_LDS_PTS], s_img[LSD_SOLO_LDS_PTS];
  const int tid = threadIdx.x, wave = tid >> 6, lane = tid & 63;
  track_state_begin(S, job, tid);
  __syncthreads();
  int listLevel = -1, total = 0;
  EvalCtx a;
  unsigned pXY[TRIPS];
  float pZ[TRIPS];
  auto taps = [&](const PointWarp& q, const bool fetch, PointTexels& t) {
    const int ix = fetch ? (int)q.u_new : 0;
    const int iy = fetch ? (int)q.v_new : 0;
    const v4f* bp = s_tex + (ix + __mul24(iy, a.w));
    const v4f v00 = bp[0], v10 = bp[1], v01 = bp[a.w], v11 = bp[a.w + 1];
    t.t00 = Texel3{v00.x, v00.y, v00.z}; t.t10 = Texel3{v10.x, v10.y, v10.z};
    t.t01 = Texel3{v01.x, v01.y, v01.z}; t.t11 = Texel3{v11.x, v11.y, v11.z};
  };
  for (int guard = 0; guard < 4096; guard++) {
    const int level = S.level;
    if (S.done) break;
    const TrackLevel& L = job.lv[level];
    const int work = L.w * L.h;
    if (L.tilePx <= 0 || work > LSD_SOLO_MAX_PX || L.writeMask) break;
    if (level != listLevel) {
      make_ctx_dev(job, S, level, a);
      if (tid == BLOCK - 1) stage_lm_par(job, level, s_par, 1);
      const int mblk = (work + 255) >> 8;
      const gbyte* offs = (const gbyte*)L.kf_refBlk;
      const __attribute__((address_space(1))) int* cnts = (const __attribute__((address_space(1))) int*)(offs + ((size_t)mblk << 8));
      const int cntv = lane < mblk ? cnts[lane] : 0;
      int incl = cntv + dpp_i0<0x111, 0xf, 0xf>(cntv);
      incl += dpp_i0<0x112, 0xf, 0xf>(cntv);
      incl += dpp_i0<0x113, 0xf, 0xf>(cntv);
      incl += dpp_i0<0x114, 0xf, 0xe>(incl);
      incl += dpp_i0<0x118, 0xf, 0xc>(incl);
      incl += dpp_i0<0x142, 0xa, 0xf>(incl);
      total = __builtin_amdgcn_readlane(incl, 31);
      if (total > LSD_SOLO_LDS_PTS) break;
      {
        gv4f* src = (gv4f*)a.fr_grad;
        for (int i = tid; i < work; i += BLOCK) s_tex[i] = src[i];
      }
      unsigned* s_list = (unsigned*)s_red;
      const int waveU = __builtin_amdgcn_readfirstlane(wave);
      const float inv_w = 1.0f / (float)a.w;
      for (int blk = waveU; blk < mblk; blk += WAVES) {
        const int cb = __builtin_amdgcn_readlane(cntv, blk);
        const int pb = __builtin_amdgcn_readlane(incl, blk) - cb;
        const unsigned ow = *(const __attribute__((address_space(1))) unsigned*)(offs + ((size_t)blk << 8) + (lane << 2));
#pragma unroll
        for (int k = 0; k < 4; k++) {
          const int sl = lane + 64 * k;
          if (sl < cb) {
            const int i = (blk << 8) + (int)((ow >> (8 * k)) & 255u);
            int y = (int)((float)i * inv_w);
            int x = i - y * a.w;
            if (x < 0) { y--; x += a.w; }
            if (x >= a.w) { y++; x -= a.w; }
            s_list[pb + sl] = (unsigned)x | ((unsigned)y << 16);
          }
        }
      }
      __syncthreads();
      {
        float var[TRIPS], id[TRIPS], img[TRIPS];
#pragma unroll
        for (int r = 0; r < TRIPS; r++) {
          const int p = tid + r * BLOCK;
          const unsigned xy = s_list[p < total ? p : 0];
          const int i = __mul24((int)(xy >> 16), a.w) + (int)(xy & 0xffffu);
          pXY[r] = xy;
          var[r] = a.kf_idepthVar[i];
          id[r] = a.kf_idepth[i];
          img[r] = a.kf_image[i];
        }
#pragma unroll
        for (int r = 0; r < TRIPS; r++) {
          const int p = tid + r * BLOCK;
          if (p < total) { s_var[p] = var[r]; s_img[p] = img[r]; }
          pZ[r] = (p < total) ? lsd_rcp_exact(id[r]) * 1.0f : 1.0f;
        }
      }
      listLevel = level;
      __syncthreads();
    } else {
#pragma unroll
      for (int i = 0; i < 9; i++) a.R[i] = S.R[i];
#pragma unroll
      for (int i = 0; i < 3; i++) a.t[i] = S.t[i];
      a.aff_a = S.aff_a; a.aff_b = S.aff_b;
    }
    auto uni = [](float v) { return __int_as_float(__builtin_amdgcn_readfirstlane(__float_as_int(v))); };
#pragma unroll
    for (int i = 0; i < 9; i++) a.R[i] = uni(a.R[i]);
#pragma unroll
    for (int i = 0; i < 3; i++) a.t[i] = uni(a.t[i]);
    a.aff_a = uni(a.aff_a); a.aff_b = uni(a.aff_b);
    float acc[RS_END];
#pragma unroll
    for (int k = 0; k < RS_END; k++) acc[k] = 0.f;
    int key0 = -1, key1 = -1, key2 = -1;
    {
      const int rounds = (total + BLOCK - 1) / BLOCK;
      struct StT { PointWarp q; PointTexels t; };
      StT T0;
      auto stageB = [&](const int r, StT& T) {
        const bool live = tid + r * BLOCK < total;
        const int bx_ = (int)(pXY[r] & 0xffffu), by_ = (int)(pXY[r] >> 16);
        const float px = pZ[r] * (a.fxi * bx_ + a.cxi), py = pZ[r] * (a.fyi * by_ + a.cyi);
        eval_warp(a, px, py, pZ[r], T.q);
        taps(T.q, live && T.q.in_image, T.t);
      };
      auto stageC = [&](const int r, const StT& T) {
        if (tid + r * BLOCK < total) {
          acc[RS_NREF] += 1.f;
          if (T.q.in_image) {
            PointOut o;
            eval_finish(a, T.q, T.t, pZ[r], s_img[tid + r * BLOCK], s_var[tid + r * BLOCK], o);
            top3_insert(__mul24((int)(pXY[r] & 0xffffu), a.h) + (int)(pXY[r] >> 16), key0, key1, key2);
            accumulate_point(o, acc);
          }
        }
      };
#pragma unroll
      for (int r = 0; r < TRIPS; r++) {
        if (r < rounds) { stageB(r, T0); stageC(r, T0); }
      }
    }
    {
      int c0 = key0, c1 = key1, c2 = key2;
#pragma unroll
      for (int r = 0; r < 3; r++) {
        const int m = __builtin_amdgcn_readlane(wave_max_to_lane63(c0), 63);
        if (lane == 0) s_wtop[wave][r] = m;
        if (c0 == m && m >= 0) { c0 = c1; c1 = c2; c2 = -1; }
      }
    }
    if (tid >= HALF) {
#pragma unroll
      for (int k = 0; k < CPP; k++) s_red[k * (HALF + 1) + tid - HALF] = acc[k];
    }
    __syncthreads();
    int cKey = -1, cX = 0, cY = 0;
    float cVar = 0.f, cId = 1.f, cImg = 0.f;
    if (wave == 0) {
      int v = lane < WAVES * 3 ? s_wtop[lane / 3][lane - 3 * (lane / 3)] : -1;
      int top[3];
#pragma unroll
      for (int r = 0; r < 3; r++) {
        top[r] = __builtin_amdgcn_readlane(wave_max_to_lane63(v), 63);
        if (v == top[r]) v = -1;
      }
      cKey = lane == 0 ? top[0] : (lane == 1 ? top[1] : (lane == 2 ? top[2] : -1));
      if (cKey >= 0) {
        cX = cKey / a.h;
        cY = cKey - cX * a.h;
        const int ci = __mul24(cY, a.w) + cX;
        cVar = a.kf_idepthVar[ci];
        cId = a.kf_idepth[ci];
        cImg = a.kf_image[ci];
      }
    }
    if (tid < HALF) {
#pragma unroll
      for (int k = 0; k < CPP; k++) s_red[k * (HALF + 1) + tid] = acc[k] + s_red[k * (HALF + 1) + tid];
    }
    __syncthreads();
    {
      const int slice = tid / CPP, k = tid - slice * CPP;
      if (slice < RSLICE) {
        const float* row = s_red + k * (HALF + 1);
        const int j0 = slice * RRUN;
        float sacc = 0.f;
#pragma unroll
        for (int j = 0; j < RRUN; j++) { const float v = row[j0 + j]; sacc += (j0 + j < HALF) ? v : 0.f; }
        s_sum[slice][k] = sacc;
      }
    }
    __syncthreads();
    if (wave == 0) {
      float sv = 0.f;
      if (lane < CPP) {
        sv = s_sum[0][lane];
#pragma unroll
        for (int sl = 1; sl < RSLICE; sl++) sv += s_sum[sl][lane];
      }
      if (cKey >= 0) {
        const float inv = lsd_rcp_exact(cId);
        const float px = inv * (a.fxi * cX + a.cxi), py = inv * (a.fyi * cY + a.cyi);
        const float cPz = inv * 1.0f;
        PointWarp cq;
        PointTexels ct;
        eval_warp(a, px, py, cPz, cq);
        taps(cq, cq.in_image, ct);
        PointOut o;
        eval_finish(a, cq, ct, cPz, cImg, cVar, o);
        float* row = s_sub[lane];
        tail_row(o, row);
      }
      __builtin_amdgcn_fence(__ATOMIC_RELEASE, "wavefront");
      __builtin_amdgcn_wave_barrier();
      __builtin_amdgcn_fence(__ATOMIC_ACQUIRE, "wavefront");
      const int M = (int)rl(sv, RS_M);
      const int nsub = (__builtin_amdgcn_readlane(cKey, 0) >= 0) + (__builtin_amdgcn_readlane(cKey, 1) >= 0) + (__builtin_amdgcn_readlane(cKey, 2) >= 0);
      int need = M & 3;
      if (need > nsub) need = nsub;
      const int subIdx = (lane == RS_WERR) ? 0 : ((lane >= RS_A0 && lane < RS_B0) ? 1 + lane - RS_A0 : ((lane >= RS_B0 && lane < RS_ERR) ? 22 + lane - RS_B0 : (lane == RS_ERR ? 28 : -1)));
      if (subIdx >= 0) {
        if (need > 0) sv -= s_sub[0][subIdx];
        if (need > 1) sv -= s_sub[1][subIdx];
        if (need > 2) sv -= s_sub[2][subIdx];
      }
      if (lane < RS_NUM) sh.tot[lane] = sv;
      lm_wave<false>(s_par, S, sv, sh.tot, lane, out, nullptr, 0, 0, doneWord);
    }
    __syncthreads();
  }
  copy_words<sizeof(TrackState) / 4>(st2 + (1 - parity), &S, tid, BLOCK);
  if (S.done) copy_words<sizeof(TrackState) / 4>(st2 + parity, &S, tid, BLOCK);
}

__global__ __launch_bounds__(256) void k_mask_merge(uint32_t* __restrict__ plane, const uint32_t* __restrict__ side, int nwords) {
  const int i = blockIdx.x * 256 + threadIdx.x;
  if (i >= nwords) return;
  const uint32_t a = plane[i], b = side[i];
  uint32_t m = 0;
#pragma unroll
  for (int k = 0; k < 4; k++) if (((a >> (8 * k)) & 0xFFu) != 0xFFu) m |= 0xFFu << (8 * k);
  plane[i] = (a & ~m) | (b & m);
}

int lsd_flush_merges(lsdhip_ctx* c) {
  const int nwords = (int)((((size_t)c->wl[LSD_TRACK_MIN_LEVEL] * c->hl[LSD_TRACK_MIN_LEVEL]) + 3) / 4);
  for (const lsdhip_ctx::PendingMerge& m : c->pendingMerges) {
    hipLaunchKernelGGL(k_mask_merge, dim3((nwords + 255) / 256), dim3(256), 0, c->mstream, (uint32_t*)m.plane, (const uint32_t*)m.side, nwords);
    *m.doneSeq = c->mSeq + 1;
  }
  c->pendingMerges.clear();
  HIPCHK(hipGetLastError());
  return LSDHIP_OK;
}

__global__ __launch_bounds__(256) void k_overlap(const float* __restrict__ pos, int n, EvalCtx a, float* __restrict__ out) {
  __shared__ float s_w[4];
  float acc = 0.f;
  for (int i = threadIdx.x; i < n; i += 256) {
    float px = pos[3 * i], py = pos[3 * i + 1], pz = pos[3 * i + 2];
    float Wx = ((a.R[0] * px + a.R[1] * py) + a.R[2] * pz) + a.t[0];
    float Wy = ((a.R[3] * px + a.R[4] * py) + a.R[5] * pz) + a.t[1];
    float Wz = ((a.R[6] * px + a.R[7] * py) + a.R[8] * pz) + a.t[2];
    float u_new = (Wx / Wz) * a.fx + a.cx;
    float v_new = (Wy / Wz) * a.fy + a.cy;
    if (u_new > 0 && v_new > 0 && u_new < a.w - 1 && v_new < a.h - 1) {
      float depthChange = pz / Wz;
      acc += depthChange < 1 ? depthChange : 1;
    }
  }
  float s = wave_sum_to_lane63(acc);
  if ((threadIdx.x & 63) == 63) s_w[threadIdx.x >> 6] = s;
  __syncthreads();
  if (threadIdx.x == 0) out[0] = ((s_w[0] + s_w[1]) + s_w[2]) + s_w[3];
}

__global__ __launch_bounds__(64) void k_devtest_se3f_lm_step(const float* __restrict__ A, const float* __restrict__ b, const float* __restrict__ damp,
                                                              const float* __restrict__ T7, float* __restrict__ inc6, float* __restrict__ Tn7) {
  __shared__ TrackState S;
  __shared__ LmShared sh;
  const int lane = threadIdx.x, c = blockIdx.x;
  if (lane < 36) S.A[lane] = A[c * 36 + lane];
  if (lane < 6) S.b[lane] = b[c * 6 + lane];
  __syncthreads();
  const float* p = T7 + c * 7;
  lsdm::SE3fH T;
  T.q = {p[0], p[1], p[2], p[3]};
  T.t[0] = p[4]; T.t[1] = p[5]; T.t[2] = p[6];
  float inc[6];
  gj6_solve_wave(S.A, S.b, damp[c], sh.gj, lane, inc);
  const lsdm::SE3fH Tn = se3f_mul_wave(se3f_exp_wave(inc, lane), T, lane);
  if (lane == 0) {
#pragma unroll
    for (int i = 0; i < 6; i++) inc6[c * 6 + i] = inc[i];
    float* o = Tn7 + c * 7;
    o[0] = Tn.q.w; o[1] = Tn.q.x; o[2] = Tn.q.y; o[3] = Tn.q.z; o[4] = Tn.t[0]; o[5] = Tn.t[1]; o[6] = Tn.t[2];
  }
}

struct ScratchLayout { size_t topkey, topval, recs, end; };
static constexpr ScratchLayout scratch_layout(size_t jobs, size_t trials, size_t rows) {
  const size_t slots = jobs * 2 * trials;
  const size_t topkey = slots * RS_COLS * rows, topval = topkey + slots * 4 * rows, recs = topval + slots * 96 * rows;
  return {topkey, topval, recs, recs + slots * 32};
}
static_assert(scratch_layout(1, LSD_SPEC_MAX, 304).end * 4 == (size_t)LSD_SPEC_MAX * (2 * RS_COLS * 304 * 4 + 2 * 304 * 16 + 2 * 304 * 96 * 4 + 2 * 32 * 4) &&
              scratch_layout(8, LSD_BATCH_SPEC_MAX, 304).end * 4 == 8 * (size_t)LSD_BATCH_SPEC_MAX * (2 * RS_COLS * 304 * 4 + 2 * 304 * 16 + 2 * 304 * 96 * 4 + 2 * 32 * 4) &&
              scratch_layout(8, LSD_BATCH_SPEC_MAX, 304).recs == 8 * (size_t)LSD_BATCH_SPEC_MAX * (2 * RS_COLS * 304 + 2 * 4 * 304 + 2 * 96 * 304),
              "scratch arena: byte count and offsets");
static TrackScratch scratch_at(const lsdhip_tracker* t, float* base, size_t jobs, size_t trials, int cmax) {
  const ScratchLayout lay = scratch_layout(jobs, trials, (size_t)t->max_blocks);
  TrackScratch sc;
  sc.sums = base;
  sc.topkey = (int4*)(base + lay.topkey);
  sc.topval = base + lay.topval;
  sc.recs = cmax > 1 ? base + lay.recs : nullptr;
  sc.max_rows = t->max_blocks;
  sc.cmax = cmax;
#ifdef LSD_PHASE_TRACE
  sc.trace = t->d_trace;
#endif
  return sc;
}

extern "C" int lsdhip_tracker_create(lsdhip_ctx* c, lsdhip_tracker** out) {
  if (!c || !out) return LSDHIP_E_ARG;
  HIPCHK(hipSetDevice(c->device));
  lsdhip_tracker* t = new lsdhip_tracker();
  t->ctx = c;
  const int maxIterations[6] = {5, 20, 50, 100, 100, 100};
  for (int l = 0; l < LSD_LEVELS; l++) {
    t->lambdaInitial[l] = 0;
    t->stepSizeMin[l] = 1e-8;
    t->convergenceEps[l] = 0.999f;
    t->maxItsPerLvl[l] = maxIterations[l];
  }
  if (const char* e = getenv("LSDHIP_TRACK_BLOCK")) t->block = atoi(e);
  if (const char* e = getenv("LSDHIP_TRACK_CAP")) t->grid_cap = atoi(e);
  if (t->block != 256) { lsd_set_error("LSDHIP_TRACK_BLOCK must be 256"); delete t; return LSDHIP_E_ARG; }
  if (t->grid_cap < 8) t->grid_cap = 8;
  t->grid_cap &= ~7;
  {
    const int nslice = ((t->block / 64 - 1) * 64) / RS_END;
    if (t->grid_cap > 80 * nslice) t->grid_cap = (80 * nslice) & ~7;
  }
  t->max_blocks = t->grid_cap;
  const size_t partials_bytes = scratch_layout(1, LSD_SPEC_MAX, (size_t)t->max_blocks).end * sizeof(float);
  if (const char* e = getenv("LSDHIP_SPEC")) t->specC = atoi(e);
  if (t->specC < 1) t->specC = 1;
  if (t->specC > LSD_SPEC_MAX) t->specC = LSD_SPEC_MAX;
  if (const char* e = getenv("LSDHIP_SPEC_CAP")) t->specCap = atoi(e) & ~7;
  if (const char* e = getenv("LSDHIP_SPEC_CAPS")) {
    int v[LSD_LEVELS] = {0, 0, 0, 0, 0};
    sscanf(e, "%d,%d,%d,%d,%d", &v[0], &v[1], &v[2], &v[3], &v[4]);
    for (int l = 0; l < LSD_LEVELS; l++) t->specCaps[l] = v[l] < 0 ? 0 : (v[l] & ~7);
  }
  if (const char* e = getenv("LSDHIP_SPEC_LEVELS")) {
    int v[LSD_LEVELS] = {0, 0, 0, 0, 0};
    sscanf(e, "%d,%d,%d,%d,%d", &v[0], &v[1], &v[2], &v[3], &v[4]);
    for (int l = 0; l < LSD_LEVELS; l++) t->specLevel[l] = v[l] < 0 ? 0 : (v[l] > LSD_SPEC_MAX ? LSD_SPEC_MAX : v[l]);
  }
  t->maskStride = (((size_t)c->wl[LSD_TRACK_MIN_LEVEL] * c->hl[LSD_TRACK_MIN_LEVEL]) + 255) & ~(size_t)255;
  HIPCHK(hipMalloc((void**)&t->d_maskSide, 2 * t->maskStride * (LSD_SPEC_MAX - 1)));
  HIPCHK(hipMemsetAsync(t->d_maskSide, 0, 2 * t->maskStride * (LSD_SPEC_MAX - 1), c->stream));
  HIPCHK(hipMalloc((void**)&t->d_partials, partials_bytes));
  HIPCHK(hipMemsetAsync(t->d_partials, 0, partials_bytes, c->stream));
#ifdef LSD_ORDER_CHECK
  {
    const size_t nd = 8 + 2 * 8192;
    HIPCHK(hipMalloc((void**)&t->d_dbg, nd * 8));
    std::vector<unsigned long long> init(nd, 0);
    for (size_t i = 8; i < nd; i += 2) init[i] = ~0ull;
    HIPCHK(hipMemcpy(t->d_dbg, init.data(), nd * 8, hipMemcpyHostToDevice));
  }
#endif
#ifdef LSD_DEVTOOLS
  HIPCHK(hipMalloc((void**)&t->d_log, 4096 * 16 * 4));
  HIPCHK(hipMemset(t->d_log, 0, 4096 * 16 * 4));
#endif
  HIPCHK(hipMalloc((void**)&t->d_state, 2 * sizeof(TrackState)));
  HIPCHK(hipMemsetAsync(t->d_state, 0, 2 * sizeof(TrackState), c->stream));
#ifdef LSD_PHASE_TRACE
  HIPCHK(hipMalloc((void**)&t->d_trace, (1 + 4096 * LSD_TRACE_WORDS) * 8));
  HIPCHK(hipMemsetAsync(t->d_trace, 0, (1 + 4096 * LSD_TRACE_WORDS) * 8, c->stream));
#endif
  HIPCHK(hipHostMalloc((void**)&t->h_summary, sizeof(TrackSummary), hipHostMallocMapped));
  HIPCHK(hipHostGetDevicePointer((void**)&t->d_summary, t->h_summary, 0));
  memset(t->h_summary, 0, sizeof(TrackSummary));
  const char* env = getenv("LSDHIP_HOST_LM");
  t->hostLM = env && env[0] == '1';
  if (const char* e = getenv("LSDHIP_SPIN")) t->spinWait = e[0] != '0';
  if (const char* e = getenv("LSDHIP_BUDGET_EXTRA")) { t->budgetExtra = atoi(e); if (t->budgetExtra < 1) t->budgetExtra = 1; }
  if (const char* e = getenv("LSDHIP_BUDGET_FIXED")) { t->budgetFixed = atoi(e); if (t->budgetFixed < 1) t->budgetFixed = 0; }
  *out = t;
  return LSDHIP_OK;
}
extern "C" void lsdhip_tracker_destroy(lsdhip_tracker* t) {
  if (!t) return;
  {
    lsdhip_ctx* c = t->ctx;
    LSD_CTX_LOCK(c);
    for (size_t i = 0; i < c->pendingMerges.size();)
      if (c->pendingMerges[i].doneSeq == &t->maskMergeSeq[0] || c->pendingMerges[i].doneSeq == &t->maskMergeSeq[1]) c->pendingMerges.erase(c->pendingMerges.begin() + i);
      else i++;
  }
#ifdef LSD_DEVTOOLS
  if (getenv("LSDHIP_TRACK_DEBUG") && t->dbgJobs > 0)
    fprintf(stderr, "TRACKDBG jobs %lld launches enqueued %.2f/job, budget misses %lld, host launch %.1f us/job, host wait %.1f us/job\n", t->dbgJobs,
            (double)t->dbgEnqueued / t->dbgJobs, t->dbgMisses, t->dbgLaunchNs / 1e3 / t->dbgJobs, t->dbgWaitNs / 1e3 / t->dbgJobs);
#endif
  (void)hipSetDevice(t->ctx->device);
  (void)hipStreamSynchronize(t->ctx->stream);
#ifdef LSD_ORDER_CHECK
  {
    std::vector<unsigned long long> h(8 + 2 * 8192, 0);
    (void)hipMemcpy(h.data(), t->d_dbg, h.size() * 8, hipMemcpyDeviceToHost);
    int used = 0, split = 0;
    for (size_t i = 8; i < h.size(); i += 2) if (h[i] != ~0ull) { used++; if (h[i] != h[i + 1]) split++; }
    if (const char* path = getenv("LSDHIP_ORDER_DUMP")) {
      if (FILE* f = fopen(path, "w")) {
        for (size_t i = 8; i < h.size(); i += 2) if (h[i] != ~0ull) fprintf(f, "%zu %llx %llx\n", (i - 8) / 2, h[i], h[i + 1]);
        fclose(f);
      }
    }
    fprintf(stderr, "ORDERCHECK: %llu workgroups finished (%llu launched), %llu started before every earlier workgroup had finished (largest deficit %llu); "
                    "%d launch slots hashed, %d in which the workgroups did NOT all see the same totals\n", h[0], t->dbgCum, h[1], h[2], used, split);
  }
#endif
  if (t->d_dbg) (void)hipFree(t->d_dbg);
#ifdef LSD_PHASE_TRACE
  if (const char* path = getenv("LSDHIP_TRACE_FILE")) {
    std::vector<unsigned long long> h(1 + 4096 * LSD_TRACE_WORDS);
    if (hipMemcpy(h.data(), t->d_trace, h.size() * 8, hipMemcpyDeviceToHost) == hipSuccess) {
      if (FILE* f = fopen(path, "w")) {
        unsigned long long n = h[0] < 4096 ? h[0] : 4096;
        for (unsigned long long i = 0; i < n; i++) {
          for (int k = 0; k < LSD_TRACE_WORDS; k++) fprintf(f, "%llu ", h[1 + i * LSD_TRACE_WORDS + k]);
          fprintf(f, "\n");
        }
        fclose(f);
      }
    }
  }
  (void)hipFree(t->d_trace);
#endif
  if (t->d_bjobs) { (void)hipFree(t->d_bjobs); (void)hipFree(t->d_bstate); (void)hipFree(t->d_bscratch); (void)hipHostFree(t->h_bjobs); (void)hipHostFree(t->h_bsummary); }
  (void)hipFree(t->d_partials);
  (void)hipFree(t->d_maskSide);
  (void)hipFree(t->d_state);
#ifdef LSD_DEVTOOLS
  (void)hipFree(t->d_log);
#endif
  (void)hipHostFree(t->h_summary);
  if (t->d_pts) (void)hipFree(t->d_pts);
  delete t;
}
extern "C" int lsdhip_tracker_set_enqueue_hook(lsdhip_tracker* t, lsdhip_enqueue_hook fn, void* user) {
  if (!t) return LSDHIP_E_ARG;
  t->enqueueHook = fn;
  t->enqueueHookUser = user;
  return LSDHIP_OK;
}
extern "C" int lsdhip_tracker_get_settings(const lsdhip_tracker* t, lsdhip_tracker_settings* o) {
  if (!t || !o) return LSDHIP_E_ARG;
  o->lambdaSuccessFac = t->lambdaSuccessFac; o->lambdaFailFac = t->lambdaFailFac;
  for (int l = 0; l < LSD_LEVELS; l++) {
    o->lambdaInitial[l] = t->lambdaInitial[l]; o->stepSizeMin[l] = t->stepSizeMin[l]; o->convergenceEps[l] = t->convergenceEps[l];
    o->maxItsPerLvl[l] = t->maxItsPerLvl[l];
  }
  o->lambdaInitialTestTrack = t->lambdaInitialTestTrack; o->stepSizeMinTestTrack = t->stepSizeMinTestTrack;
  o->convergenceEpsTestTrack = t->convergenceEpsTestTrack; o->maxItsTestTrack = t->maxItsTestTrack;
  o->huber_d = t->huber_d; o->var_weight = t->var_weight;
  return LSDHIP_OK;
}
extern "C" int lsdhip_tracker_set_settings(lsdhip_tracker* t, const lsdhip_tracker_settings* in) {
  if (!t || !in) return LSDHIP_E_ARG;
  t->lambdaSuccessFac = in->lambdaSuccessFac; t->lambdaFailFac = in->lambdaFailFac;
  for (int l = 0; l < LSD_LEVELS; l++) {
    t->lambdaInitial[l] = in->lambdaInitial[l]; t->stepSizeMin[l] = in->stepSizeMin[l]; t->convergenceEps[l] = in->convergenceEps[l];
    t->maxItsPerLvl[l] = in->maxItsPerLvl[l];
  }
  t->lambdaInitialTestTrack = in->lambdaInitialTestTrack; t->stepSizeMinTestTrack = in->stepSizeMinTestTrack;
  t->convergenceEpsTestTrack = in->convergenceEpsTestTrack; t->maxItsTestTrack = in->maxItsTestTrack;
  t->huber_d = in->huber_d; t->var_weight = in->var_weight;
  return LSDHIP_OK;
}
extern "C" int lsdhip_tracker_exec_stats(const lsdhip_tracker* t, int out[8]) {
  if (!t || !out) return LSDHIP_E_ARG;
  out[0] = 0; out[1] = 0; out[2] = 0;
  for (int l = 0; l < LSD_LEVELS; l++) out[3 + l] = t->levelEvaluations[l];
  return LSDHIP_OK;
}
extern "C" int lsdhip_tracker_set_speculation(lsdhip_tracker* t, int trials, int finestLevelWorkgroups) {
  if (!t || trials < 1 || trials > LSD_SPEC_MAX || finestLevelWorkgroups < 0) { lsd_set_error("lsdhip_tracker_set_speculation: trials must be 1..%d", LSD_SPEC_MAX); return LSDHIP_E_ARG; }
  LSD_CTX_LOCK(t->ctx);
  t->specC = trials;
  t->specAuto = false;
  if (finestLevelWorkgroups > 0) t->specCap = finestLevelWorkgroups < 8 ? 8 : (finestLevelWorkgroups & ~7);
  for (int l = 0; l < LSD_LEVELS; l++) t->specLevel[l] = 0;
  for (int i = 0; i < 4; i++) t->recent[i] = 0;
  return LSDHIP_OK;
}
extern "C" int lsdhip_tracker_set_batch_coarse_min_jobs(lsdhip_tracker* t, int minJobs) {
  if (!t || minJobs < 0) { lsd_set_error("lsdhip_tracker_set_batch_coarse_min_jobs: minJobs must be >= 0"); return LSDHIP_E_ARG; }
  LSD_CTX_LOCK(t->ctx);
  t->soloMinJobs = minJobs;
  return LSDHIP_OK;
}
#ifdef LSD_DEVTOOLS
extern "C" int lsdhip_tracker_debug_log(const lsdhip_tracker* t, int* out, int maxInts) {
  if (!t || !out) return -1;
  const int n = (int)t->lastLog.size() < maxInts ? (int)t->lastLog.size() : maxInts;
  memcpy(out, t->lastLog.data(), (size_t)n * 4);
  return n;
}
#endif
extern "C" int lsdhip_tracker_launch_stats(const lsdhip_tracker* t, int out[2]) {
  if (!t || !out) return LSDHIP_E_ARG;
  out[0] = t->numLaunches; out[1] = t->specC;
  return LSDHIP_OK;
}
extern "C" int lsdhip_tracker_step_stats(const lsdhip_tracker* t, int out[4]) {
  if (!t || !out) return LSDHIP_E_ARG;
  out[0] = t->numLaunches; out[1] = 0; out[2] = 0; out[3] = t->specC;
  return LSDHIP_OK;
}
extern "C" int lsdhip_tracker_set_max_its(lsdhip_tracker* t, const int its[LSD_LEVELS]) {
  if (!t || !its) return LSDHIP_E_ARG;
  for (int l = 0; l < LSD_LEVELS; l++) t->maxItsPerLvl[l] = its[l];
  return LSDHIP_OK;
}

static const float MIN_GOODPERGOODBAD_PIXEL = 0.5f;
static const float MIN_GOODPERALL_PIXEL = 0.04f;
static const float MIN_GOODPERALL_PIXEL_ABSMIN = 0.01f;

struct BatchShape { int jobs, cap; };
static BatchShape batch_shape(const lsdhip_tracker* t, int n) {
  if (n <= 1) return {0, 0};
  const int cap = (t->grid_cap / n) & ~7;
  return {n, cap < 16 ? 16 : cap};
}

static long long env_num(const char* name, long long dflt) { const char* e = getenv(name); return e ? atoll(e) : dflt; }
struct BatchEnv {
  int specMax = (int)std::clamp<long long>(env_num("LSDHIP_BATCH_SPEC", LSD_BATCH_SPEC_MAX), 1, LSD_BATCH_SPEC_MAX);
  long long specPixels = env_num("LSDHIP_BATCH_SPEC_PIXELS", LSD_BATCH_SPEC_PIXELS);
  int fused = (int)env_num("LSDHIP_BATCH_FUSED", 2);
  int margin = (int)env_num("LSDHIP_BATCH_MARGIN", 3);
  bool poll = !(getenv("LSDHIP_BATCH_POLL") && getenv("LSDHIP_BATCH_POLL")[0] == '0');
  int soloMin = (int)env_num("LSDHIP_BATCH_SOLO_MIN", LSD_SOLO_MIN_JOBS);
  int stripWgs = (int)env_num("LSDHIP_BATCH_WGS", LSD_BATCH_STRIP_WORKGROUPS);
  int traceWg = (int)env_num("LSDHIP_TRACE_WG", 0);
};
static const BatchEnv& batch_env() { static const BatchEnv env; return env; }

static int fill_level(lsdhip_tracker* t, TrackJob& job, BatchShape shape, int level, lsdhip_frame* kf, lsdhip_frame* frame, const float* pts_pos,
                      const float* pts_colvar, int npts) {
  lsdhip_ctx* c = t->ctx;
  LSD_CTX_LOCK(c);
  TrackLevel& L = job.lv[level];
  const LevelIntr& in = c->intr[level];
  L.w = c->wl[level]; L.h = c->hl[level];
  L.fx = in.fx; L.fy = in.fy; L.cx = in.cx; L.cy = in.cy; L.fxi = in.fxi; L.fyi = in.fyi; L.cxi = in.cxi; L.cyi = in.cyi;
  L.fr_grad = frame->d_grad[level];
  if (level == 0) { if (int rc = lsd_frame_require_level0_for_tracking(frame)) return rc; }
  if (npts >= 0) {
    L.pts_pos = pts_pos; L.pts_colvar = pts_colvar; L.npts = npts;
    L.kf_idepth = L.kf_idepthVar = L.kf_image = nullptr;
    L.kf_refBlk = nullptr;
  } else {
    L.kf_idepth = kf->d_idepth[level]; L.kf_idepthVar = kf->d_idepthVar[level]; L.kf_image = kf->d_image[level];
    L.kf_refBlk = kf->d_refBlk[level];
    L.pts_pos = L.pts_colvar = nullptr; L.npts = -1;
  }
  int work = npts >= 0 ? npts : L.w * L.h;
  L.nblocks = (work + t->block - 1) / t->block;
  if (L.nblocks >= 16) L.nblocks = (L.nblocks + 7) & ~7;
  const int cap = shape.cap > 0 ? shape.cap : t->grid_cap;
  if (L.nblocks > cap) L.nblocks = cap;
  if (L.nblocks < 1) L.nblocks = 1;
  L.singlePass = (long long)L.nblocks * t->block >= work ? 1 : 0;
  L.tilePx = 0;
  if (shape.jobs >= LSD_BATCH_THROUGHPUT_MIN_JOBS && npts < 0 && L.kf_refBlk != nullptr) {
    const int wgTarget = batch_env().stripWgs;
    long long px = (((long long)work * shape.jobs + wgTarget - 1) / wgTarget + 255) & ~255LL;
    if (px < 1024) px = 1024;
    if (px > 8192) px = 8192;
    if ((work + px - 1) / px <= t->max_blocks) {
      L.tilePx = (int)px;
      L.nblocks = (int)((work + px - 1) / px);
      L.singlePass = 0;
    }
  }
  L.lambdaInitial = t->lambdaInitial[level]; L.stepSizeMin = t->stepSizeMin[level]; L.convergenceEps = t->convergenceEps[level];
  L.maxIts = t->maxItsPerLvl[level];
  L.minWarped = MIN_GOODPERALL_PIXEL_ABSMIN * (c->w >> level) * (c->h >> level);
  L.writeMask = 0;
  return LSDHIP_OK;
}
static void fill_job_common(lsdhip_tracker* t, TrackJob& job) {
  lsdhip_ctx* c = t->ctx;
  LSD_CTX_LOCK(c);
  memset(&job, 0, sizeof(job));
  job.cameraPixelNoise2 = c->params.cameraPixelNoise2;
  job.var_weight = t->var_weight;
  job.huber_half = t->huber_d / 2;
  job.lambdaSuccessFac = t->lambdaSuccessFac;
  job.lambdaFailFac = t->lambdaFailFac;
  job.useAffine = c->params.useAffineLightningEstimation;
}
static lsdm::SE3fH pose_from7(const float* T7) {
  lsdm::SE3fH T;
  T.q = {T7[0], T7[1], T7[2], T7[3]};
  T.t[0] = T7[4]; T.t[1] = T7[5]; T.t[2] = T7[6];
  return T;
}
static lsdm::SE3fH pose_of(const TrackSummary* S) {
  const float T7[7] = {S->q[0], S->q[1], S->q[2], S->q[3], S->t[0], S->t[1], S->t[2]};
  return pose_from7(T7);
}
static void take_summary(lsdhip_tracker* t, const TrackSummary* S) {
  t->numEvaluations = S->numEvaluations;
  t->numWarpUpdates = S->numWarpUpdates;
  t->pointUsage = S->pointUsage; t->lastGoodCount = S->goodCount; t->lastBadCount = S->badCount; t->lastMeanRes = S->meanRes;
  t->affineEstimation_a = S->aff_a; t->affineEstimation_b = S->aff_b;
  t->affineEstimation_a_lastIt = S->aff_a_lastIt; t->affineEstimation_b_lastIt = S->aff_b_lastIt;
  t->lastResidual = S->lastResidual;
}
static bool tracking_was_good(const lsdhip_tracker* t, int level) {
  const lsdhip_ctx* c = t->ctx;
  return t->lastGoodCount / (c->wl[level] * c->hl[level]) > MIN_GOODPERALL_PIXEL &&
         t->lastGoodCount / (t->lastGoodCount + t->lastBadCount) > MIN_GOODPERGOODBAD_PIXEL;
}

static TrackScratch scratch_of(lsdhip_tracker* t) { return scratch_at(t, t->d_partials, 1, LSD_SPEC_MAX, LSD_SPEC_MAX); }
static void launch_step(lsdhip_tracker* t, const TrackJob& job, int grid, int parity, int first) {
  lsdhip_ctx* c = t->ctx;
  LSD_CTX_LOCK(c);
  TrackScratch sc = scratch_of(t);
  t->launchOrdinal++;
  t->spec.seq = t->jobTag ? ((t->jobTag << 12) | (t->launchOrdinal & 0xFFF)) : 0;
#ifdef LSD_DEVTOOLS
  t->spec.dbgLog = t->d_log;
#endif
#ifdef LSD_ORDER_CHECK
  t->spec.dbgCum = t->dbgCum;
  t->spec.dbgCounters = t->d_dbg;
  t->dbgCum += (unsigned long long)grid;
#endif
  hipLaunchKernelGGL((k_track_step<256, false>), dim3(grid), dim3(256), 0, c->stream, job, (const TrackJob*)nullptr, t->d_state, sc,
                     t->d_summary, parity, first, t->spec);
}
static int launch_steps(lsdhip_tracker* t, TrackJob& job, int steps, int* parity, int* first) {
  int grid = 1;
  for (int l = job.lastLevel; l <= job.topLevel; l++) if (job.lv[l].nblocks > grid) grid = job.lv[l].nblocks;
  t->spec.specGrid = 0;
  if (t->spec.specC > 1) {
    for (int l = job.lastLevel; l <= job.topLevel; l++) {
      const int g = job.lv[l].nblocks * (t->spec.trials[l] > 1 ? t->spec.trials[l] : 1);
      if (g > grid) grid = g;
    }
    t->spec.specGrid = grid;
  }
#ifdef LSD_DEVTOOLS
  const auto tl0 = std::chrono::steady_clock::now();
#endif
  for (int i = 0; i < steps; i++) {
    t->spec.last = (i + 1 == steps) ? 1 : 0;
    launch_step(t, job, grid, *parity, *first);
    lsdhip_host_mark(20);
    *first = 0;
    *parity ^= 1;
  }
#ifdef LSD_DEVTOOLS
  t->dbgEnqueued += steps;
  t->dbgLaunchNs += std::chrono::duration_cast<std::chrono::nanoseconds>(std::chrono::steady_clock::now() - tl0).count();
#endif
  HIPCHK(hipGetLastError());
  return LSDHIP_OK;
}

static int prof_collect(lsdhip_ctx* c);
struct EvalOut {
  int warped_size;
  float retval;
  float weightedError;
  float A[36], b[6], lsError;
  double num_constraints;
};

static void eval_out_of(const TrackSummary* S, EvalOut* eo) {
  const float* r = S->sums;
  int M = (int)r[RS_M];
  eo->warped_size = M;
  eo->retval = r[RS_SUMRES2] / r[RS_GOOD];
  eo->weightedError = r[RS_WERR] / ((M >> 2) << 2);
  size_t num_constraints = (size_t)6 * (size_t)(M >> 2);
  float n = (float)num_constraints;
  int k = RS_A0;
  for (int i = 0; i < 6; i++)
    for (int j = i; j < 6; j++, k++) {
      float v = (0.0f + r[k]) / n;
      eo->A[i * 6 + j] = v;
      eo->A[j * 6 + i] = v;
    }
  for (int i = 0; i < 6; i++) eo->b[i] = (0.0f - r[RS_B0 + i]) / n;
  eo->lsError = (0.0f + r[RS_ERR]) / n;
  eo->num_constraints = (double)num_constraints;
}

static int evaluate_pose(lsdhip_tracker* t, TrackJob& job, const lsdm::SE3fH& T, int level, EvalOut* eo) {
  lsdhip_ctx* c = t->ctx;
  LSD_CTX_LOCK(c);
  job.evalOnly = 1;
  job.lastLevel = level;
  job.topLevel = level;
  job.T0 = T;
  job.aff_a0 = t->affineEstimation_a; job.aff_b0 = t->affineEstimation_b;
  t->h_summary->done = 0;
  t->spec = TrackSpec{};
  t->jobTag = 0;
  if (int rcp = prof_collect(c)) return rcp;
  if (c->prof_on) HIPCHK(hipEventRecord(c->ev_a, c->stream));
  t->spec.last = 0;
  launch_step(t, job, job.lv[level].nblocks, 0, 1);
  if (c->prof_on) HIPCHK(hipEventRecord(c->ev_b, c->stream));
  launch_step(t, job, 1, 1, 0);
  HIPCHK(hipGetLastError());
  HIPCHK(hipStreamSynchronize(c->stream));
  const TrackSummary* S = t->h_summary;
  if (c->prof_on) {
    float ms = 0;
    HIPCHK(hipEventElapsedTime(&ms, c->ev_a, c->ev_b));
    c->prof_ms += ms;
    c->prof_launches++;
    c->prof_bytes += S->bytes;
  }
  t->numEvaluations++;
  t->pointUsage = S->pointUsage; t->lastGoodCount = S->goodCount; t->lastBadCount = S->badCount; t->lastMeanRes = S->meanRes;
  t->affineEstimation_a_lastIt = S->aff_a_lastIt; t->affineEstimation_b_lastIt = S->aff_b_lastIt;
  eval_out_of(S, eo);
  return LSDHIP_OK;
}

static void record_of(const TrackSummary* S, lsdhip_residual_record* out) {
  EvalOut ev;
  eval_out_of(S, &ev);
  out->warped_size = ev.warped_size;
  out->goodCount = S->goodCount; out->badCount = S->badCount; out->pointUsage = S->pointUsage;
  out->meanRes = S->meanRes; out->retval = ev.retval;
  out->affine_a_lastIt = S->aff_a_lastIt; out->affine_b_lastIt = S->aff_b_lastIt;
  out->weightedError = ev.weightedError;
  memcpy(out->A, ev.A, sizeof(ev.A)); memcpy(out->b, ev.b, sizeof(ev.b));
  out->lsError = ev.lsError; out->num_constraints = ev.num_constraints;
}

static int lm_level_host(lsdhip_tracker* t, TrackJob& job, int lvl, lsdm::SE3fH& referenceToFrame, float* lastResidualOut) {
  lsdhip_ctx* c = t->ctx;
  LSD_CTX_LOCK(c);
  const TrackLevel& L = job.lv[lvl];
  EvalOut ev;
  int rc = evaluate_pose(t, job, referenceToFrame, lvl, &ev);
  if (rc) return rc;
  if (ev.warped_size < L.minWarped) return LSDHIP_DIVERGED;
  if (c->params.useAffineLightningEstimation) {
    t->affineEstimation_a = t->affineEstimation_a_lastIt;
    t->affineEstimation_b = t->affineEstimation_b_lastIt;
  }
  float lastErr = ev.weightedError;
  float LM_lambda = L.lambdaInitial;
  EvalOut cur = ev;
  for (int iteration = 0; iteration < L.maxIts; iteration++) {
    t->numWarpUpdates++;
    int incTry = 0;
    while (true) {
      float b[6], A[36], inc[6];
      for (int i = 0; i < 6; i++) b[i] = -cur.b[i];
      memcpy(A, cur.A, sizeof(A));
      for (int i = 0; i < 6; i++) A[i * 6 + i] *= 1 + LM_lambda;
      lsdm::ldlt6_solve(A, b, inc);
      incTry++;
      lsdm::SE3fH new_referenceToFrame = lsdm::se3f_mul(lsdm::se3f_exp(inc), referenceToFrame);
      EvalOut nev;
      rc = evaluate_pose(t, job, new_referenceToFrame, lvl, &nev);
      if (rc) return rc;
      if (nev.warped_size < L.minWarped) return LSDHIP_DIVERGED;
      float error = nev.weightedError;
      if (error < lastErr) {
        referenceToFrame = new_referenceToFrame;
        cur = nev;
        if (c->params.useAffineLightningEstimation) {
          t->affineEstimation_a = t->affineEstimation_a_lastIt;
          t->affineEstimation_b = t->affineEstimation_b_lastIt;
        }
        if (error / lastErr > L.convergenceEps) iteration = L.maxIts;
        lastErr = error;
        if (job.trackFrameSemantics) *lastResidualOut = error;
        if (LM_lambda <= 0.2) LM_lambda = 0;
        else LM_lambda *= t->lambdaSuccessFac;
        break;
      } else {
        float incdot = (inc[0] * inc[0] + (inc[1] * inc[1] + inc[2] * inc[2])) + (inc[3] * inc[3] + (inc[4] * inc[4] + inc[5] * inc[5]));
        if (!(incdot > L.stepSizeMin)) { iteration = L.maxIts; break; }
        if (LM_lambda == 0) LM_lambda = 0.2;
        else LM_lambda *= std::pow(t->lambdaFailFac, incTry);
      }
    }
  }
  if (!job.trackFrameSemantics) *lastResidualOut = lastErr;
  return LSDHIP_OK;
}

static int prof_collect(lsdhip_ctx* c) {
  if (!c->prof_pending) return LSDHIP_OK;
  HIPCHK(hipEventSynchronize(c->ev_b));
  float ms = 0;
  HIPCHK(hipEventElapsedTime(&ms, c->ev_a, c->ev_b));
  c->prof_ms += ms;
  c->prof_pending = false;
  return LSDHIP_OK;
}
int lsd_prof_collect(lsdhip_ctx* c) { return prof_collect(c); }

static int summary_wait_consistent(lsdhip_tracker* t, const int doneWord, const TrackSummary* rec = nullptr) {
  if (!rec) rec = t->h_summary;
  volatile const unsigned* w = (volatile const unsigned*)rec;
  t->sumPolled++;
  unsigned first[LSD_SUMMARY_CHECK_WORDS];
  std::chrono::steady_clock::time_point t0;
  for (unsigned spins = 0;; spins++) {
    unsigned cur[LSD_SUMMARY_CHECK_WORDS];
    unsigned chk = (unsigned)doneWord;
    for (unsigned i = 1; i < LSD_SUMMARY_CHECK_WORDS; i++) { cur[i] = w[i]; chk += lsd_summary_term(i, cur[i]); }
    const unsigned want = *(volatile const unsigned*)&rec->check;
    if (chk == want) {
      if (spins > 0) {
        const long long ns = std::chrono::duration_cast<std::chrono::nanoseconds>(std::chrono::steady_clock::now() - t0).count();
        if (ns > t->sumLateMaxNs) t->sumLateMaxNs = ns;
        for (unsigned i = 1; i < LSD_SUMMARY_CHECK_WORDS; i++)
          if (first[i] != cur[i]) {
            t->sumLateWords++;
            if (t->sumLateFirstWord < 0 || (int)i < t->sumLateFirstWord) t->sumLateFirstWord = (int)i;
            if ((int)i > t->sumLateLastWord) t->sumLateLastWord = (int)i;
          }
      }
      std::atomic_thread_fence(std::memory_order_acquire);
      return LSDHIP_OK;
    }
    if (spins == 0) {
      t->sumLate++;
      t0 = std::chrono::steady_clock::now();
      memcpy(first, cur, sizeof(first));
    }
    if ((spins & 0xFFFFu) == 0xFFFFu && std::chrono::steady_clock::now() - t0 > std::chrono::seconds(2)) {
      lsd_set_error("tracking summary in pinned memory never became consistent (check %08x, sum %08x)", want, chk);
      return LSDHIP_E_STATE;
    }
    __builtin_ia32_pause();
  }
}
extern "C" int lsdhip_tracker_summary_stats(const lsdhip_tracker* t, long long out[6]) {
  if (!t || !out) return LSDHIP_E_ARG;
  out[0] = t->sumPolled; out[1] = t->sumLate; out[2] = t->sumLateMaxNs; out[3] = t->sumLateWords; out[4] = t->sumLateFirstWord; out[5] = t->sumLateLastWord;
  return LSDHIP_OK;
}

static int track_device(lsdhip_tracker* t, TrackJob& job, int topLevel, const lsdm::SE3fH& T0, lsdm::SE3fH* Tout) {
  lsdhip_ctx* c = t->ctx;
  job.evalOnly = 0;
  job.topLevel = topLevel;
  job.T0 = T0;
  job.aff_a0 = 1.0f; job.aff_b0 = 0.0f;
  t->spec.specC = t->specC;
  t->spec.specGrid = 0;
  t->maskSet ^= 1;
  t->spec.wasGoodSide = t->d_maskSide + (size_t)t->maskSet * t->maskStride * (LSD_SPEC_MAX - 1);
  t->spec.maskStride = (unsigned)t->maskStride;
  t->spec.copyMask = c->pipeline ? 0 : 1;
  if (c->pipeline && t->maskMergeSeq[t->maskSet] != 0) {
    if (t->maskMergeSeq[t->maskSet] < 0) { if (int rcf = lsd_flush_merges(c)) return rcf; }
    if (t->maskMergeSeq[t->maskSet] > c->mSeq && lsd_m_record(c) < 0) return LSDHIP_E_HIP;
    if (int rcw = lsd_t_wait_m(c, t->maskMergeSeq[t->maskSet])) return rcw;
    t->maskMergeSeq[t->maskSet] = 0;
  }
  for (int l = 0; l < LSD_LEVELS; l++) t->spec.trials[l] = 1;
  if (t->specC > 1) {
    for (int l = job.lastLevel; l <= topLevel; l++) {
      TrackLevel& L = job.lv[l];
      const long long work = L.npts >= 0 ? L.npts : (long long)L.w * L.h;
      int trials, cap = t->specCaps[l];
      if (t->specLevel[l] > 0) trials = t->specLevel[l];
      else if (!t->specAuto) trials = t->specC;
      else trials = work <= LSD_SPEC_SMALL_PX ? LSD_SPEC_TRIALS_SMALL : (work <= LSD_SPEC_MID_PX ? LSD_SPEC_TRIALS_MID : 1);
      if (trials > t->specC) trials = t->specC;
      if (cap <= 0 && trials > 1 && (t->specAuto ? work > LSD_SPEC_CAP_ABOVE_PX : l == job.lastLevel)) cap = t->specCap > 0 ? t->specCap : ((t->grid_cap / 2 + 7) & ~7);
      t->spec.trials[l] = trials;
      if (trials > 1 && cap > 0 && L.nblocks > cap && L.tilePx == 0) {
        L.nblocks = cap;
        L.singlePass = (long long)L.nblocks * t->block >= work ? 1 : 0;
      }
    }
  }
  t->h_summary->done = 0;
  const TrackSummary* S = t->h_summary;
  const long long myEpoch = ++c->enqEpoch;
  int budget = 12;
  if (t->recent[0] > 0) {
    budget = 0;
    for (int i = 0; i < 4; i++) if (t->recent[i] > budget) budget = t->recent[i];
    budget += t->budgetExtra;
  }
  if (t->budgetFixed > 0) budget = t->budgetFixed;
  const bool sample = c->prof_on && ((c->prof_tick++ & 7) == 0);
#ifdef LSD_DEVTOOLS
  t->dbgJobs++;
#endif
  t->jobTag = (t->jobTag % 0x7FFFF) + 1;
  t->launchOrdinal = 0;
  t->h_summary->seq = 0;
  t->h_summary->exhausted = 0;
  int guard = 0;
  int parity = 0, first = 1;
  if (int rc = prof_collect(c)) return rc;
  lsdhip_host_mark(2);
  while (true) {
    if (sample) HIPCHK(hipEventRecord(c->ev_a, c->stream));
    int rc = LSDHIP_OK;
    rc = launch_steps(t, job, budget, &parity, &first);
    if (rc) return rc;
    if (sample) { HIPCHK(hipEventRecord(c->ev_b, c->stream)); c->prof_pending = true; }
    lsdhip_host_mark(3);
    if (guard == 0 && t->enqueueHook && job.trackFrameSemantics) t->enqueueHook(t->enqueueHookUser);
    lsdhip_host_mark(4);
#ifdef LSD_DEVTOOLS
    const auto tw0 = std::chrono::steady_clock::now();
    struct WaitClock { lsdhip_tracker* t; std::chrono::steady_clock::time_point t0; ~WaitClock() { t->dbgWaitNs += std::chrono::duration_cast<std::chrono::nanoseconds>(std::chrono::steady_clock::now() - t0).count(); } } waitClock_{t, tw0};
#endif
    c->mtx.unlock();
    struct Relock { std::recursive_mutex& m; ~Relock() { m.lock(); } };
    {
    Relock relock_{c->mtx};
    if (t->spinWait) {
      volatile const int* done = &S->done;
      volatile const int* exhausted = &S->exhausted;
      const int lastSeq = t->spec.seq;
      const auto tStart = std::chrono::steady_clock::now();
      unsigned spins = 0;
      while (*done != t->jobTag) {
        if (*exhausted == lastSeq) break;
        if ((++spins & 0xFFFFFu) == 0) {
          hipError_t q = hipStreamQuery(c->stream);
          if (q == hipSuccess) break;
          if (q != hipErrorNotReady) { lsd_set_error("hipStreamQuery failed: %s", hipGetErrorString(q)); return LSDHIP_E_HIP; }
          if (std::chrono::steady_clock::now() - tStart > std::chrono::seconds(5)) { HIPCHK(hipStreamSynchronize(c->stream)); break; }
        }
        __builtin_ia32_pause();
      }
      std::atomic_thread_fence(std::memory_order_acquire);
    } else {
      HIPCHK(hipStreamSynchronize(c->stream));
    }
    }
    lsdhip_host_mark(5);
    if (*(volatile const int*)&S->done == t->jobTag) break;
#ifdef LSD_DEVTOOLS
    t->dbgMisses++;
#endif
    HIPCHK(hipStreamSynchronize(c->stream));
#ifdef LSD_DEVTOOLS
    {
      static const bool dumpL0 = getenv("LSDHIP_DUMP_L0") != nullptr;
      if (dumpL0 && guard == 0 && t->budgetFixed == 1) {
        const TrackScratch sc = scratch_of(t);
        const size_t rows = (size_t)t->max_blocks;
        const int nb = job.lv[topLevel].nblocks;
        t->dumpL0.assign((size_t)nb * (RS_COLS + 4 + 96) + sizeof(TrackState) / 4, 0u);
        unsigned* d = t->dumpL0.data();
        HIPCHK(hipMemcpy(d, sc.sums + (size_t)(1 * LSD_SPEC_MAX + 0) * RS_COLS * rows, (size_t)nb * RS_COLS * 4, hipMemcpyDeviceToHost));
        HIPCHK(hipMemcpy(d + (size_t)nb * RS_COLS, sc.topkey + (size_t)(1 * LSD_SPEC_MAX + 0) * rows, (size_t)nb * 16, hipMemcpyDeviceToHost));
        HIPCHK(hipMemcpy(d + (size_t)nb * (RS_COLS + 4), sc.topval + (size_t)(1 * LSD_SPEC_MAX + 0) * rows * 96, (size_t)nb * 96 * 4, hipMemcpyDeviceToHost));
        HIPCHK(hipMemcpy(d + (size_t)nb * (RS_COLS + 4 + 96), t->d_state + 1, sizeof(TrackState), hipMemcpyDeviceToHost));
      }
    }
#endif
    if (*(volatile const int*)&S->done == t->jobTag) break;
    if (int rc2 = prof_collect(c)) return rc2;
    if (t->jobKf && t->jobKf->depthVersion != t->jobKfVersion && guard < 8) {
      t->jobKfVersion = t->jobKf->depthVersion;
      t->h_summary->done = 0;
      parity = 0; first = 1;
      budget = 12;
      ++guard;
      continue;
    }
    budget = t->budgetFixed > 0 ? t->budgetFixed : 6;
    if (++guard > 200) { lsd_set_error("tracking job did not terminate"); return LSDHIP_E_STATE; }
  }
  if (int rcs = summary_wait_consistent(t, t->jobTag)) return rcs;
  if (sample) {
    c->prof_bytes += S->bytes;
    c->prof_launches += S->numLaunches;
  }
  if (myEpoch > c->doneEpoch) c->doneEpoch = myEpoch;
#ifdef LSD_DEVTOOLS
  {
    static const bool keepLog = getenv("LSDHIP_LAUNCH_LOG") != nullptr;
    if (keepLog) {
      HIPCHK(hipStreamSynchronize(c->stream));
      const int n = t->launchOrdinal < 4095 ? t->launchOrdinal + 1 : 4096;
      t->lastLog.assign((size_t)n * 16, 0);
      HIPCHK(hipMemcpy(t->lastLog.data(), t->d_log, (size_t)n * 64, hipMemcpyDeviceToHost));
      HIPCHK(hipMemset(t->d_log, 0, (size_t)n * 64));
    }
  }
#endif
  t->numLaunches = S->numLaunches;
  t->recent[3] = t->recent[2]; t->recent[2] = t->recent[1]; t->recent[1] = t->recent[0]; t->recent[0] = t->numLaunches;
  for (int l = 0; l < LSD_LEVELS; l++) t->levelEvaluations[l] = S->levelEvals[l];
  take_summary(t, S);
  *Tout = pose_of(S);
  return S->diverged ? LSDHIP_DIVERGED : LSDHIP_OK;
}

static void fill_result(lsdhip_tracker* t, const lsdm::SE3dH& T, lsdhip_track_result* out) {
  lsdm::se3d_to7(T, out->frameToReference);
  out->pointUsage = t->pointUsage; out->lastGoodCount = t->lastGoodCount; out->lastBadCount = t->lastBadCount;
  out->lastMeanRes = t->lastMeanRes; out->lastResidual = t->lastResidual;
  out->affineEstimation_a = t->affineEstimation_a; out->affineEstimation_b = t->affineEstimation_b;
  out->diverged = t->diverged; out->trackingWasGood = t->trackingWasGood;
  out->numEvaluations = t->numEvaluations; out->numWarpUpdates = t->numWarpUpdates;
}
static lsdm::SE3dH identity_d() { lsdm::SE3dH I; I.q = {1, 0, 0, 0}; I.t[0] = I.t[1] = I.t[2] = 0; return I; }
static int finish_diverged(lsdhip_tracker* t, lsdhip_track_result* out) {
  t->diverged = true;
  t->trackingWasGood = false;
  fill_result(t, identity_d(), out);
  return LSDHIP_DIVERGED;
}

static int fill_trackframe_job(lsdhip_tracker* t, TrackJob& job, BatchShape shape, lsdhip_frame* kf, lsdhip_frame* frame) {
  fill_job_common(t, job);
  for (int lvl = LSD_TRACK_MIN_LEVEL; lvl < LSD_TRACK_MAX_LEVEL; lvl++)
    if (int rcl = fill_level(t, job, shape, lvl, kf, frame, nullptr, nullptr, -1)) return rcl;
  job.lv[LSD_TRACK_MIN_LEVEL].writeMask = 1;
  int rc = lsd_frame_ensure_wasgood(frame);
  if (rc) return rc;
  job.wasGood = frame->d_wasGood;
  job.lastLevel = LSD_TRACK_MIN_LEVEL;
  job.trackFrameSemantics = 1;
  return LSDHIP_OK;
}
static int fill_eval_job(lsdhip_tracker* t, TrackJob& job, BatchShape shape, lsdhip_frame* kf, lsdhip_frame* frame, int level, const float T7[7],
                         float aff_a, float aff_b) {
  fill_job_common(t, job);
  if (int rcl = fill_level(t, job, shape, level, kf, frame, nullptr, nullptr, -1)) return rcl;
  if (level == LSD_TRACK_MIN_LEVEL) {
    if (int rc = lsd_frame_ensure_wasgood(frame)) return rc;
    job.wasGood = frame->d_wasGood;
    job.lv[level].writeMask = 1;
  }
  job.trackFrameSemantics = 1;
  job.evalOnly = 1;
  job.lastLevel = level;
  job.topLevel = level;
  job.T0 = pose_from7(T7);
  job.aff_a0 = aff_a; job.aff_b0 = aff_b;
  return LSDHIP_OK;
}
static int fill_permaref_job(lsdhip_tracker* t, TrackJob& job, BatchShape shape, const float* pts_pos, const float* pts_colvar, int npts,
                             lsdhip_frame* frame, const lsdm::SE3fH& T0) {
  const int L = LSD_QUICK_KF_CHECK_LVL;
  fill_job_common(t, job);
  if (int rcl = fill_level(t, job, shape, L, nullptr, frame, pts_pos, pts_colvar, npts)) return rcl;
  job.lv[L].lambdaInitial = t->lambdaInitialTestTrack; job.lv[L].stepSizeMin = t->stepSizeMinTestTrack;
  job.lv[L].convergenceEps = t->convergenceEpsTestTrack; job.lv[L].maxIts = (int)t->maxItsTestTrack;
  job.lastLevel = L;
  job.topLevel = L;
  job.trackFrameSemantics = 0;
  job.evalOnly = 0;
  job.T0 = T0;
  job.aff_a0 = 1.0f; job.aff_b0 = 0.0f;
  return LSDHIP_OK;
}
static int finish_permaref(lsdhip_tracker* t, bool diverged, const lsdm::SE3fH& referenceToFrame, lsdhip_track_result* out) {
  if (diverged) return finish_diverged(t, out);
  t->diverged = false;
  t->trackingWasGood = tracking_was_good(t, LSD_QUICK_KF_CHECK_LVL);
  fill_result(t, lsdm::se3d_from_f(referenceToFrame), out);
  return LSDHIP_OK;
}
static int finish_trackframe(lsdhip_tracker* t, const TrackSummary* S, lsdhip_frame* kf, lsdhip_frame* frame, lsdhip_track_result* out) {
  lsdhip_ctx* c = t->ctx;
  LSD_CTX_LOCK(c);
  take_summary(t, S);
  if (S->diverged) return finish_diverged(t, out);
  t->diverged = false;
  t->trackingWasGood = tracking_was_good(t, LSD_TRACK_MIN_LEVEL);
  if (t->trackingWasGood) kf->numFramesTrackedOnThis++;
  frame->initialTrackedResidual = t->lastResidual / t->pointUsage;
  lsdm::SE3dH f2r = lsdm::se3d_from_f(lsdm::se3f_inverse(pose_of(S)));
  frame->thisToParent_raw.q = f2r.q;
  lsdm::q_normalize(frame->thisToParent_raw.q);
  frame->thisToParent_raw.t[0] = f2r.t[0]; frame->thisToParent_raw.t[1] = f2r.t[1]; frame->thisToParent_raw.t[2] = f2r.t[2];
  frame->thisToParent_raw.s = 1;
  frame->trackingParent = kf;
  frame->trackingParentID = kf->id;
  fill_result(t, f2r, out);
  return LSDHIP_OK;
}

extern "C" int lsdhip_tracker_track(lsdhip_tracker* t, lsdhip_frame* kf, lsdhip_frame* frame, const double init[7],
                                    lsdhip_track_result* out) {
  if (!t || !kf || !frame || !init || !out) return LSDHIP_E_ARG;
  if (!kf->hasIDepth) { lsd_set_error("lsdhip_tracker_track: keyframe %d has no depth", kf->id); return LSDHIP_E_STATE; }
  lsdhip_ctx* c = t->ctx;
  LSD_CTX_LOCK(c);
  HIPCHK(hipSetDevice(c->device));
  t->diverged = false;
  t->trackingWasGood = true;
  t->affineEstimation_a = 1; t->affineEstimation_b = 0;
  t->numEvaluations = 0; t->numWarpUpdates = 0;
  TrackJob job;
  LsdTrackJobScope tjob_(c, false);
  if (c->pipeline) {
    long long need = frame->readySeq > kf->readySeq ? frame->readySeq : kf->readySeq;
    if (kf->depthSeq > need) need = kf->depthSeq;
    if (int rcw = lsd_t_wait_m(c, need)) return rcw;
  }
  int rc = fill_trackframe_job(t, job, BatchShape{}, kf, frame);
  if (rc) return rc;
  if (int rcg = lsd_gate_open(c)) return rcg;
  if (int rcd = lsd_pipe_dummy(c)) return rcd;
#ifdef LSD_DEVTOOLS
  static const bool traceInputs = getenv("LSDHIP_TRACE_INPUTS") != nullptr;
  auto trace_inputs = [&](int base) {
    for (int l = 1; l <= 4; l++) {
      const size_t nl = (size_t)c->wl[l] * c->hl[l];
      lsd_trace_sum(c, c->stream, base + 10 + l, frame->id, kf->d_idepth[l], nl * 4);
      lsd_trace_sum(c, c->stream, base + 14 + l, frame->id, kf->d_idepthVar[l], nl * 4);
      lsd_trace_sum(c, c->stream, base + 50 + l, frame->id, kf->d_image[l], nl * 4);
      lsd_trace_sum(c, c->stream, base + 54 + l, frame->id, frame->d_grad[l], nl * 16);
    }
  };
  if (traceInputs) trace_inputs(0);
  {
    unsigned long long pv = 0;
    for (int i = 0; i < 7; i++) { unsigned long long u; memcpy(&u, &init[i], 8); pv = pv * 1000003ull + u; }
    lsd_trace_val(c, 22, frame->id, pv);
    lsd_trace_val(c, 23, frame->id, (unsigned long long)kf->id);
  }
#endif
  lsdm::SE3fH referenceToFrame = lsdm::se3f_from_d(lsdm::se3d_inverse(lsdm::se3d_from7(init)));

  if (t->hostLM) {
    float last_residual = 0;
    rc = LSDHIP_OK;
    for (int lvl = LSD_TRACK_MAX_LEVEL - 1; lvl >= LSD_TRACK_MIN_LEVEL && rc == LSDHIP_OK; lvl--)
      rc = lm_level_host(t, job, lvl, referenceToFrame, &last_residual);
    t->lastResidual = last_residual;
    if (rc == LSDHIP_DIVERGED) return finish_diverged(t, out);
    if (rc) return rc;
    TrackSummary S = *t->h_summary;
    S.diverged = 0;
    S.q[0] = referenceToFrame.q.w; S.q[1] = referenceToFrame.q.x; S.q[2] = referenceToFrame.q.y; S.q[3] = referenceToFrame.q.z;
    S.t[0] = referenceToFrame.t[0]; S.t[1] = referenceToFrame.t[1]; S.t[2] = referenceToFrame.t[2];
    S.lastResidual = last_residual; S.numEvaluations = t->numEvaluations; S.numWarpUpdates = t->numWarpUpdates;
    S.pointUsage = t->pointUsage; S.goodCount = t->lastGoodCount; S.badCount = t->lastBadCount; S.meanRes = t->lastMeanRes;
    S.aff_a = t->affineEstimation_a; S.aff_b = t->affineEstimation_b;
    S.aff_a_lastIt = t->affineEstimation_a_lastIt; S.aff_b_lastIt = t->affineEstimation_b_lastIt;
    return finish_trackframe(t, &S, kf, frame, out);
  }
  t->jobKf = kf;
  t->jobKfVersion = kf->depthVersion;
#ifdef LSD_DEVTOOLS
  const lsdm::SE3fH referenceToFrame0 = referenceToFrame;
  lsd_trace_val(c, 26, frame->id, t->dbgCum / 400ull);
#endif
  rc = track_device(t, job, LSD_TRACK_MAX_LEVEL - 1, referenceToFrame, &referenceToFrame);
  if (rc != LSDHIP_OK && rc != LSDHIP_DIVERGED) { t->jobKf = nullptr; return rc; }
#ifdef LSD_DEVTOOLS
  static const bool replay = getenv("LSDHIP_TRACK_REPLAY") != nullptr;
  if (replay && c->pipeline) {
    unsigned long long pv = 0;
    for (int i = 0; i < 4; i++) { unsigned u; memcpy(&u, &t->h_summary->q[i], 4); pv = pv * 1000003ull + u; }
    for (int i = 0; i < 3; i++) { unsigned u; memcpy(&u, &t->h_summary->t[i], 4); pv = pv * 1000003ull + u; }
    lsd_trace_val(c, 24, frame->id, pv);
    lsd_trace_val(c, 25, frame->id, (unsigned long long)t->h_summary->numEvaluations * 1000 + t->h_summary->lastCand);
    HIPCHK(hipStreamSynchronize(c->mstream));
    HIPCHK(hipStreamSynchronize(c->stream));
    c->mDoneSeq = c->mSeq;
    const std::vector<unsigned> dump1 = t->dumpL0;
    if (traceInputs) trace_inputs(100);
    lsd_trace_val(c, 27, frame->id, t->dbgCum / 400ull);
    referenceToFrame = referenceToFrame0;
    rc = track_device(t, job, LSD_TRACK_MAX_LEVEL - 1, referenceToFrame, &referenceToFrame);
    if (rc != LSDHIP_OK && rc != LSDHIP_DIVERGED) { t->jobKf = nullptr; return rc; }
    HIPCHK(hipStreamSynchronize(c->stream));
    if (!dump1.empty() && dump1.size() == t->dumpL0.size()) {
      const int nb = job.lv[LSD_TRACK_MAX_LEVEL - 1].nblocks;
      int shown = 0;
      for (size_t i = 0; i < dump1.size(); i++)
        if (dump1[i] != t->dumpL0[i] && shown++ < 12) {
          const size_t a = (size_t)nb * RS_COLS, b = a + (size_t)nb * 4, cst = b + (size_t)nb * 96;
          float f1, f2; memcpy(&f1, &dump1[i], 4); memcpy(&f2, &t->dumpL0[i], 4);
          if (i < a) fprintf(stderr, "L0DIFF frame %d: sums tile %zu column %zu: run %.9g (%08x) replay %.9g (%08x)\n", frame->id, i / RS_COLS, i % RS_COLS, f1, dump1[i], f2, t->dumpL0[i]);
          else if (i < b) fprintf(stderr, "L0DIFF frame %d: topkey tile %zu [%zu]: run %d replay %d\n", frame->id, (i - a) / 4, (i - a) % 4, (int)dump1[i], (int)t->dumpL0[i]);
          else if (i < cst) fprintf(stderr, "L0DIFF frame %d: topval tile %zu slot %zu entry %zu: run %.9g replay %.9g\n", frame->id, (i - b) / 96, ((i - b) % 96) / 32, (i - b) % 32, f1, f2);
          else fprintf(stderr, "L0DIFF frame %d: state word %zu: run %08x (%.9g) replay %08x (%.9g)\n", frame->id, i - cst, dump1[i], f1, t->dumpL0[i], f2);
        }
      if (shown) fprintf(stderr, "L0DIFF frame %d: %d words differ after the first launch\n", frame->id, shown);
    }
  }
#endif
  t->jobKf = nullptr;
  lsdhip_host_mark(6);
#ifdef LSD_DEVTOOLS
  {
    unsigned long long pv = 0;
    for (int i = 0; i < 4; i++) { unsigned u; memcpy(&u, &t->h_summary->q[i], 4); pv = pv * 1000003ull + u; }
    for (int i = 0; i < 3; i++) { unsigned u; memcpy(&u, &t->h_summary->t[i], 4); pv = pv * 1000003ull + u; }
    lsd_trace_val(c, 20, frame->id, pv);
    lsd_trace_val(c, 21, frame->id, (unsigned long long)t->h_summary->numEvaluations * 1000 + t->h_summary->lastCand);
  }
#endif
  if (c->pipeline && rc == LSDHIP_OK && t->h_summary->lastCand > 0 && t->h_summary->level == LSD_TRACK_MIN_LEVEL) {
    const uint8_t* side = t->spec.wasGoodSide + (size_t)(t->h_summary->lastCand - 1) * t->maskStride;
    t->maskMergeSeq[t->maskSet] = -1;
    c->pendingMerges.push_back({frame->d_wasGood, side, &t->maskMergeSeq[t->maskSet]});
  }
  rc = finish_trackframe(t, t->h_summary, kf, frame, out);
  lsdhip_host_mark(7);
  return rc;
}

static int batch_reserve(lsdhip_tracker* t, int n) {
  lsdhip_ctx* c = t->ctx;
  LSD_CTX_LOCK(c);
  if (n <= t->batch_capacity) return LSDHIP_OK;
  HIPCHK(hipStreamSynchronize(c->stream));
  if (t->d_bjobs) { (void)hipFree(t->d_bjobs); (void)hipFree(t->d_bstate); (void)hipFree(t->d_bscratch); (void)hipHostFree(t->h_bjobs); (void)hipHostFree(t->h_bsummary); }
  t->batch_capacity = n < 8 ? 8 : n;
  const size_t B = (size_t)t->batch_capacity, bytes = scratch_layout(B, LSD_BATCH_SPEC_MAX, (size_t)t->max_blocks).end * sizeof(float);
  HIPCHK(hipMalloc((void**)&t->d_bjobs, B * sizeof(TrackJob)));
  HIPCHK(hipMalloc((void**)&t->d_bstate, B * 2 * sizeof(TrackState)));
  HIPCHK(hipMalloc((void**)&t->d_bscratch, bytes));
  HIPCHK(hipMemsetAsync(t->d_bscratch, 0, bytes, c->stream));
  HIPCHK(hipHostMalloc((void**)&t->h_bjobs, B * sizeof(TrackJob), hipHostMallocDefault));
  HIPCHK(hipHostMalloc((void**)&t->h_bsummary, B * sizeof(TrackSummary), hipHostMallocMapped));
  return LSDHIP_OK;
}
static TrackScratch batch_scratch(lsdhip_tracker* t, int cmax) {
  return scratch_at(t, t->d_bscratch, (size_t)t->batch_capacity, LSD_BATCH_SPEC_MAX, cmax);
}
static int batch_run(lsdhip_tracker* t, int n, bool callHook = false) {
  lsdhip_ctx* c = t->ctx;
  LSD_CTX_LOCK(c);
  const BatchEnv& env = batch_env();
  int grid = 1;
  bool split = false;
  for (int j = 0; j < n; j++) {
    const TrackJob& job = t->h_bjobs[j];
    for (int l = job.lastLevel; l <= job.topLevel; l++) {
      if (job.lv[l].nblocks > grid) grid = job.lv[l].nblocks;
      if (job.lv[l].tilePx > 0) split = true;
    }
    t->h_bsummary[j].done = 0;
  }
  HIPCHK(hipMemcpyAsync(t->d_bjobs, t->h_bjobs, (size_t)n * sizeof(TrackJob), hipMemcpyHostToDevice, c->stream));
  TrackSpec spec = TrackSpec{};
#ifdef LSD_PHASE_TRACE
  spec.traceWg = env.traceWg;
#endif
  int lmGrid = 1;
  int specMax = env.specMax;
  if (t->specC < specMax) specMax = t->specC;
  if (env.fused == 1) specMax = 1;
  if (split && specMax > 1) {
    for (int l = 0; l < LSD_LEVELS; l++) spec.trials[l] = 1;
    const TrackJob& j0 = t->h_bjobs[0];
    for (int l = j0.lastLevel; l <= j0.topLevel; l++) {
      bool ok = true;
      for (int j = 0; j < n; j++) ok = ok && t->h_bjobs[j].lv[l].tilePx > 0 && !t->h_bjobs[j].lv[l].writeMask && t->h_bjobs[j].lastLevel <= l && t->h_bjobs[j].topLevel >= l;
      if (!ok) continue;
      long long tr = env.specPixels / ((long long)j0.lv[l].w * j0.lv[l].h * n);
      if (tr > specMax) tr = specMax;
      if (tr < 1) tr = 1;
      spec.trials[l] = (int)tr;
      if (tr > lmGrid) lmGrid = (int)tr;
    }
    spec.specC = lmGrid;
    for (int j = 0; j < n; j++) {
      const TrackJob& job = t->h_bjobs[j];
      for (int l = job.lastLevel; l <= job.topLevel; l++) if (job.lv[l].nblocks * spec.trials[l] > grid) grid = job.lv[l].nblocks * spec.trials[l];
    }
  }
  const TrackScratch sc = batch_scratch(t, split && lmGrid > 1 ? LSD_BATCH_SPEC_MAX : 1);
  TrackSummary* d_sum = nullptr;
  HIPCHK(hipHostGetDevicePointer((void**)&d_sum, t->h_bsummary, 0));
  if (int rcp = prof_collect(c)) return rcp;
  int budget = 26;
  if (split && t->batchRecent[0] > 0) {
    budget = 0;
    for (int i = 0; i < 4; i++) if (t->batchRecent[i] > budget) budget = t->batchRecent[i];
    budget += env.margin;
  }
  int parity = 0, first = 1, guard = 0;
  const bool polled = split && env.fused && t->spinWait && env.poll;
  if (polled) {
    t->batchTag = t->batchTag >= 0x3FFFFFFF ? 2 : t->batchTag + 1;
    if (t->batchTag < 2) t->batchTag = 2;
    spec.seq = t->batchTag;
    for (int j = 0; j < n; j++) t->h_bsummary[j].exhausted = 0;
  }
  const int soloMin = t->soloMinJobs >= 0 ? t->soloMinJobs : env.soloMin;
  bool soloDue = split && env.fused && soloMin > 0 && n >= soloMin;
  if (soloDue) {
    bool any = false;
    for (int j = 0; j < n && !any; j++) {
      const TrackLevel& L = t->h_bjobs[j].lv[t->h_bjobs[j].topLevel];
      any = L.tilePx > 0 && !L.writeMask && (long long)L.w * L.h <= LSD_SOLO_MAX_PX;
    }
    soloDue = any;
  }
  while (true) {
    if (c->prof_on) HIPCHK(hipEventRecord(c->ev_a, c->stream));
    if (soloDue) {
      soloDue = false;
      const int dw = polled ? t->batchTag : 1;
      hipLaunchKernelGGL(k_track_solo<512>, dim3(n), dim3(512), 0, c->stream, (const TrackJob*)t->d_bjobs, t->d_bstate, d_sum, parity, dw);
      first = 0;
      parity ^= 1;
    }
    for (int i = 0; i < budget; i++) {
      spec.last = (polled && i == budget - 1) ? 1 : 0;
      if (split && env.fused) {
        hipLaunchKernelGGL((k_track_step<256, true, TS_FUSED>), dim3(grid, n), dim3(256), 0, c->stream, t->h_bjobs[0], (const TrackJob*)t->d_bjobs,
                           t->d_bstate, sc, d_sum, parity, first, spec);
      } else if (split) {
        hipLaunchKernelGGL((k_track_step<256, true, TS_LM>), dim3(lmGrid, n), dim3(256), 0, c->stream, t->h_bjobs[0], (const TrackJob*)t->d_bjobs,
                           t->d_bstate, sc, d_sum, parity, first, spec);
        hipLaunchKernelGGL((k_track_step<256, true, TS_EVAL>), dim3(grid, n), dim3(256), 0, c->stream, t->h_bjobs[0], (const TrackJob*)t->d_bjobs,
                           t->d_bstate, sc, d_sum, 1 - parity, 0, spec);
      } else {
        hipLaunchKernelGGL((k_track_step<256, true>), dim3(grid, n), dim3(256), 0, c->stream, t->h_bjobs[0], (const TrackJob*)t->d_bjobs,
                           t->d_bstate, sc, d_sum, parity, first, TrackSpec{});
      }
      first = 0;
      parity ^= 1;
    }
    HIPCHK(hipGetLastError());
    if (c->prof_on) { HIPCHK(hipEventRecord(c->ev_b, c->stream)); c->prof_pending = true; }
    if (callHook && guard == 0 && t->enqueueHook) t->enqueueHook(t->enqueueHookUser);
    bool all = true;
    if (polled) {
      const auto t0 = std::chrono::steady_clock::now();
      for (int j = 0; j < n && all; j++) {
        volatile const int* done = &t->h_bsummary[j].done;
        volatile const int* exhausted = &t->h_bsummary[j].exhausted;
        for (unsigned spins = 0;; spins++) {
          if (*done == t->batchTag) break;
          if (*exhausted == t->batchTag) { all = false; break; }
          if ((spins & 0xFFFFu) == 0xFFFFu) {
            if (hipStreamQuery(c->stream) != hipErrorNotReady) { all = *done == t->batchTag; if (!all) break; }
            if (std::chrono::steady_clock::now() - t0 > std::chrono::seconds(20)) { lsd_set_error("tracking batch: no progress report from the device"); return LSDHIP_E_STATE; }
          }
          __builtin_ia32_pause();
        }
        if (all) { if (int rcs = summary_wait_consistent(t, t->batchTag, &t->h_bsummary[j])) return rcs; }
      }
      if (!all) {
        HIPCHK(hipStreamSynchronize(c->stream));
        all = true;
        for (int j = 0; j < n; j++) { all = all && t->h_bsummary[j].done == t->batchTag; t->h_bsummary[j].exhausted = 0; }
      }
    } else {
      HIPCHK(hipStreamSynchronize(c->stream));
      for (int j = 0; j < n; j++) all = all && t->h_bsummary[j].done;
    }
    if (all) break;
    if (int rc2 = prof_collect(c)) return rc2;
    budget = 6;
    if (++guard > 200) { lsd_set_error("tracking batch did not terminate"); return LSDHIP_E_STATE; }
  }
  if (c->prof_on)
    for (int j = 0; j < n; j++) { c->prof_bytes += t->h_bsummary[j].bytes; c->prof_launches += t->h_bsummary[j].numEvaluations; }
  if (split) {
    int rounds = 0;
    for (int j = 0; j < n; j++) if (t->h_bsummary[j].numLaunches > rounds) rounds = t->h_bsummary[j].numLaunches;
    t->batchRecent[3] = t->batchRecent[2]; t->batchRecent[2] = t->batchRecent[1]; t->batchRecent[1] = t->batchRecent[0]; t->batchRecent[0] = rounds;
    t->numLaunches = rounds;
  }
  return LSDHIP_OK;
}

extern "C" void lsdhip_build_defaults(lsdhip_build_defaults_t* out) {
  if (!out) return;
  out->ctx_async = LSD_DEFAULT_ASYNC; out->ctx_pipeline = LSD_DEFAULT_PIPELINE;
  out->spec_trials_small = LSD_SPEC_TRIALS_SMALL; out->spec_small_pixels = LSD_SPEC_SMALL_PX;
  out->spec_trials_mid = LSD_SPEC_TRIALS_MID; out->spec_mid_pixels = LSD_SPEC_MID_PX;
  out->spec_workgroups = LSD_SPEC_CAP_WORKGROUPS; out->spec_workgroups_above_pixels = LSD_SPEC_CAP_ABOVE_PX;
  out->spec_trials_max = LSD_SPEC_MAX;
  out->batch_throughput_min_jobs = LSD_BATCH_THROUGHPUT_MIN_JOBS; out->batch_strip_workgroups = LSD_BATCH_STRIP_WORKGROUPS;
  out->batch_coarse_min_jobs = LSD_SOLO_MIN_JOBS; out->batch_coarse_max_pixels = LSD_SOLO_MAX_PX; out->batch_coarse_max_points = LSD_SOLO_LDS_PTS;
}

extern "C" int lsdhip_tracker_track_batch(lsdhip_tracker* t, int n, lsdhip_frame** keyframes, lsdhip_frame** frames,
                                          const double* inits, lsdhip_track_result* results) {
  if (!t || n <= 0 || !keyframes || !frames || !inits || !results) return LSDHIP_E_ARG;
  lsdhip_ctx* c = t->ctx;
  LSD_CTX_LOCK(c);
  HIPCHK(hipSetDevice(c->device));
  for (int j = 0; j < n; j++) {
    if (!keyframes[j] || !frames[j]) return LSDHIP_E_ARG;
    if (!keyframes[j]->hasIDepth) { lsd_set_error("lsdhip_tracker_track_batch: keyframe %d has no depth", keyframes[j]->id); return LSDHIP_E_STATE; }
  }
  if (c->pipeline) {
    long long need = 0;
    for (int j = 0; j < n; j++) {
      need = std::max(need, std::max(frames[j]->readySeq, std::max(keyframes[j]->readySeq, keyframes[j]->depthSeq)));
    }
    if (int rcw = lsd_t_wait_m(c, need)) return rcw;
  }
  if (n >= LSD_BATCH_THROUGHPUT_MIN_JOBS) { if (int rcb = lsd_frames_require_ref_blocks(keyframes, n, c->stream)) return rcb; }
  int rc = batch_reserve(t, n);
  if (rc) return rc;
  const BatchShape shape = batch_shape(t, n);
  for (int j = 0; j < n; j++) {
    TrackJob& job = t->h_bjobs[j];
    rc = fill_trackframe_job(t, job, shape, keyframes[j], frames[j]);
    if (rc) return rc;
    job.evalOnly = 0;
    job.topLevel = LSD_TRACK_MAX_LEVEL - 1;
    job.T0 = lsdm::se3f_from_d(lsdm::se3d_inverse(lsdm::se3d_from7(inits + 7 * (size_t)j)));
    job.aff_a0 = 1.0f; job.aff_b0 = 0.0f;
  }
  rc = batch_run(t, n, true);
  if (rc) return rc;
  int rcAll = LSDHIP_OK;
  for (int j = 0; j < n; j++) {
    rc = finish_trackframe(t, &t->h_bsummary[j], keyframes[j], frames[j], &results[j]);
    if (rc == LSDHIP_DIVERGED) rcAll = LSDHIP_DIVERGED;
    else if (rc) return rc;
  }
  return rcAll;
}

extern "C" int lsdhip_tracker_eval_throughput(lsdhip_tracker* t, int n, lsdhip_frame** keyframes, lsdhip_frame** frames, const float* refToFrame,
                                              int level, int repeats, double* ms_per_launch, double* bytes_per_launch) {
  if (!t || n < 8 || !keyframes || !frames || !refToFrame || level < 0 || level >= LSD_LEVELS || repeats < 1 || !ms_per_launch || !bytes_per_launch)
    return LSDHIP_E_ARG;
  lsdhip_ctx* c = t->ctx;
  LSD_CTX_LOCK(c);
  LsdTrackJobScope tjob_(c, true);
  if (tjob_.rc) return tjob_.rc;
  HIPCHK(hipSetDevice(c->device));
  for (int j = 0; j < n; j++) if (!keyframes[j] || !frames[j] || !keyframes[j]->hasIDepth) return LSDHIP_E_ARG;
  if (int rcb = lsd_frames_require_ref_blocks(keyframes, n, c->stream)) return rcb;
  int rc = batch_reserve(t, n);
  if (rc) return rc;
  const BatchShape shape = batch_shape(t, n);
  int grid = 1;
  for (int j = 0; j < n; j++) {
    TrackJob& job = t->h_bjobs[j];
    rc = fill_eval_job(t, job, shape, keyframes[j], frames[j], level, refToFrame + 7 * (size_t)j, 1.0f, 0.0f);
    if (rc) return rc;
    if (job.lv[level].nblocks > grid) grid = job.lv[level].nblocks;
    if (job.lv[level].tilePx == 0) { lsd_set_error("lsdhip_tracker_eval_throughput: level %d is not in throughput mode", level); return LSDHIP_E_STATE; }
    t->h_bsummary[j].done = 0;
  }
  HIPCHK(hipMemcpyAsync(t->d_bjobs, t->h_bjobs, (size_t)n * sizeof(TrackJob), hipMemcpyHostToDevice, c->stream));
  const TrackScratch sc = batch_scratch(t, 1);
  TrackSummary* d_sum = nullptr;
  HIPCHK(hipHostGetDevicePointer((void**)&d_sum, t->h_bsummary, 0));
  struct EventPair {
    hipEvent_t a = nullptr, b = nullptr;
    ~EventPair() { if (a) (void)hipEventDestroy(a); if (b) (void)hipEventDestroy(b); }
  } evp;
  HIPCHK(hipEventCreate(&evp.a));
  HIPCHK(hipEventCreate(&evp.b));
  const hipEvent_t e0 = evp.a, e1 = evp.b;
  hipLaunchKernelGGL((k_track_step<256, true, TS_LM>), dim3(1, n), dim3(256), 0, c->stream, t->h_bjobs[0], (const TrackJob*)t->d_bjobs, t->d_bstate, sc,
                     d_sum, 0, 1, TrackSpec{});
  auto eval_launch = [&]() -> int {
    hipLaunchKernelGGL((k_track_step<256, true, TS_EVAL>), dim3(grid, n), dim3(256), 0, c->stream, t->h_bjobs[0], (const TrackJob*)t->d_bjobs, t->d_bstate, sc,
                       d_sum, 1, 0, TrackSpec{});
    return LSDHIP_OK;
  };
  if (int rcw = eval_launch()) return rcw;
  HIPCHK(hipEventRecord(e0, c->stream));
  for (int r = 0; r < repeats; r++)
    if (int rce = eval_launch()) return rce;
  HIPCHK(hipEventRecord(e1, c->stream));
  hipLaunchKernelGGL((k_track_step<256, true, TS_LM>), dim3(1, n), dim3(256), 0, c->stream, t->h_bjobs[0], (const TrackJob*)t->d_bjobs, t->d_bstate, sc,
                     d_sum, 1, 0, TrackSpec{});
  HIPCHK(hipGetLastError());
  HIPCHK(hipStreamSynchronize(c->stream));
  float ms = 0;
  HIPCHK(hipEventElapsedTime(&ms, e0, e1));
  double bytes = 0;
  for (int j = 0; j < n; j++) {
    if (!t->h_bsummary[j].done) { lsd_set_error("lsdhip_tracker_eval_throughput: job %d did not finish", j); return LSDHIP_E_STATE; }
    bytes += t->h_bsummary[j].bytes;
  }
  *ms_per_launch = ms / repeats;
  *bytes_per_launch = bytes;
  return LSDHIP_OK;
}

extern "C" int lsdhip_tracker_evaluate(lsdhip_tracker* t, lsdhip_frame* kf, lsdhip_frame* frame, const float T7[7], int level,
                                       float aff_a, float aff_b, lsdhip_residual_record* out) {
  if (!t || !kf || !frame || !T7 || !out || level < 0 || level >= LSD_LEVELS) return LSDHIP_E_ARG;
  if (!kf->hasIDepth) { lsd_set_error("lsdhip_tracker_evaluate: keyframe has no depth"); return LSDHIP_E_STATE; }
  HIPCHK(hipSetDevice(t->ctx->device));
  LSD_CTX_LOCK(t->ctx);
  LsdTrackJobScope tjob_(t->ctx, true);
  if (tjob_.rc) return tjob_.rc;
  t->affineEstimation_a = aff_a; t->affineEstimation_b = aff_b;
  TrackJob job;
  int rc = fill_eval_job(t, job, BatchShape{}, kf, frame, level, T7, aff_a, aff_b);
  if (rc) return rc;
  EvalOut ev;
  rc = evaluate_pose(t, job, job.T0, level, &ev);
  if (rc) return rc;
  record_of(t->h_summary, out);
  return LSDHIP_OK;
}

extern "C" int lsdhip_tracker_evaluate_batch(lsdhip_tracker* t, int n, lsdhip_frame** keyframes, lsdhip_frame** frames, const float* refToFrame,
                                             const float* affine, int level, lsdhip_residual_record* out, int* form) {
  if (!t || n <= 0 || !keyframes || !frames || !refToFrame || !affine || !out) return LSDHIP_E_ARG;
  if (level < LSD_TRACK_MIN_LEVEL || level >= LSD_TRACK_MAX_LEVEL) {
    lsd_set_error("lsdhip_tracker_evaluate_batch: level %d is not a tracking level (%d..%d)", level, LSD_TRACK_MIN_LEVEL, LSD_TRACK_MAX_LEVEL - 1);
    return LSDHIP_E_ARG;
  }
  lsdhip_ctx* c = t->ctx;
  LSD_CTX_LOCK(c);
  LsdTrackJobScope tjob_(c, true);
  if (tjob_.rc) return tjob_.rc;
  HIPCHK(hipSetDevice(c->device));
  for (int j = 0; j < n; j++) {
    if (!keyframes[j] || !frames[j]) return LSDHIP_E_ARG;
    if (!keyframes[j]->hasIDepth) { lsd_set_error("lsdhip_tracker_evaluate_batch: keyframe of job %d has no depth", j); return LSDHIP_E_STATE; }
  }
  if (n >= LSD_BATCH_THROUGHPUT_MIN_JOBS) { if (int rcb = lsd_frames_require_ref_blocks(keyframes, n, c->stream)) return rcb; }
  int rc = batch_reserve(t, n);
  if (rc) return rc;
  const BatchShape shape = batch_shape(t, n);
  for (int j = 0; j < n; j++) {
    rc = fill_eval_job(t, t->h_bjobs[j], shape, keyframes[j], frames[j], level, refToFrame + 7 * (size_t)j, affine[2 * (size_t)j], affine[2 * (size_t)j + 1]);
    if (rc) return rc;
  }
  int recent[4];
  memcpy(recent, t->batchRecent, sizeof(recent));
  const int numLaunches = t->numLaunches;
  rc = batch_run(t, n);
  memcpy(t->batchRecent, recent, sizeof(recent));
  t->numLaunches = numLaunches;
  if (rc) return rc;
  for (int j = 0; j < n; j++) {
    const TrackSummary* S = &t->h_bsummary[j];
    if (!S->done) { lsd_set_error("lsdhip_tracker_evaluate_batch: job %d did not finish", j); return LSDHIP_E_STATE; }
    record_of(S, &out[j]);
    if (form) {
      form[2 * j] = S->numLaunches == 0 ? 1 : 0;
      form[2 * j + 1] = t->h_bjobs[j].lv[level].tilePx;
    }
  }
  return LSDHIP_OK;
}

static int upload_points(lsdhip_tracker* t, const float* pos, const float* colvar, int n) {
  if (n > t->pts_capacity) {
    if (t->d_pts) HIPCHK(hipFree(t->d_pts));
    t->pts_capacity = n > 4096 ? n : 4096;
    HIPCHK(hipMalloc((void**)&t->d_pts, (size_t)t->pts_capacity * 5 * sizeof(float)));
  }
  HIPCHK(hipMemcpyAsync(t->d_pts, pos, (size_t)n * 12, hipMemcpyHostToDevice, t->ctx->stream));
  if (colvar) HIPCHK(hipMemcpyAsync(t->d_pts + (size_t)t->pts_capacity * 3, colvar, (size_t)n * 8, hipMemcpyHostToDevice, t->ctx->stream));
  return LSDHIP_OK;
}

extern "C" int lsdhip_tracker_track_permaref(lsdhip_tracker* t, const float* pos, const float* colvar, int n, lsdhip_frame* frame,
                                             const double refToFrame[7], lsdhip_track_result* out) {
  if (!t || !pos || !colvar || n <= 0 || !frame || !refToFrame || !out) return LSDHIP_E_ARG;
  lsdhip_ctx* c = t->ctx;
  LSD_CTX_LOCK(c);
  LsdTrackJobScope tjob_(c, true);
  if (tjob_.rc) return tjob_.rc;
  HIPCHK(hipSetDevice(c->device));
    int rc = upload_points(t, pos, colvar, n);
  if (rc) return rc;
  lsdm::SE3fH referenceToFrame = lsdm::se3f_from_d(lsdm::se3d_from7(refToFrame));
  t->affineEstimation_a = 1; t->affineEstimation_b = 0;
  t->diverged = false; t->trackingWasGood = true;
  t->numEvaluations = 0; t->numWarpUpdates = 0;
  const int L = LSD_QUICK_KF_CHECK_LVL;
  TrackJob job;
  rc = fill_permaref_job(t, job, BatchShape{}, t->d_pts, t->d_pts + (size_t)t->pts_capacity * 3, n, frame, referenceToFrame);
  if (rc) return rc;
  if (t->hostLM) {
    float lastErr = 0;
    rc = lm_level_host(t, job, L, referenceToFrame, &lastErr);
    t->lastResidual = lastErr;
  } else {
    rc = track_device(t, job, L, referenceToFrame, &referenceToFrame);
  }
  if (rc != LSDHIP_OK && rc != LSDHIP_DIVERGED) return rc;
  return finish_permaref(t, rc == LSDHIP_DIVERGED, referenceToFrame, out);
}

extern "C" int lsdhip_tracker_track_permaref_batch(lsdhip_tracker* t, int n, const float* pos, const float* colvar, const int* counts,
                                                   lsdhip_frame** frames, const double* refToFrame, lsdhip_track_result* results) {
  if (!t || n <= 0 || !pos || !colvar || !counts || !frames || !refToFrame || !results) return LSDHIP_E_ARG;
  lsdhip_ctx* c = t->ctx;
  LSD_CTX_LOCK(c);
  LsdTrackJobScope tjob_(c, true);
  if (tjob_.rc) return tjob_.rc;
  HIPCHK(hipSetDevice(c->device));
  int total = 0;
  for (int j = 0; j < n; j++) { if (counts[j] <= 0 || !frames[j]) return LSDHIP_E_ARG; total += counts[j]; }
  int rc = upload_points(t, pos, colvar, total);
  if (rc) return rc;
  rc = batch_reserve(t, n);
  if (rc) return rc;
  const BatchShape shape = batch_shape(t, n);
  int off = 0;
  for (int j = 0; j < n; j++) {
    rc = fill_permaref_job(t, t->h_bjobs[j], shape, t->d_pts + (size_t)off * 3, t->d_pts + (size_t)t->pts_capacity * 3 + (size_t)off * 2, counts[j],
                           frames[j], lsdm::se3f_from_d(lsdm::se3d_from7(refToFrame + 7 * (size_t)j)));
    if (rc) return rc;
    off += counts[j];
  }
  rc = batch_run(t, n);
  if (rc) return rc;
  int rcAll = LSDHIP_OK;
  for (int j = 0; j < n; j++) {
    const TrackSummary* S = &t->h_bsummary[j];
    take_summary(t, S);
    if (finish_permaref(t, S->diverged != 0, pose_of(S), &results[j]) == LSDHIP_DIVERGED) rcAll = LSDHIP_DIVERGED;
  }
  return rcAll;
}

extern "C" int lsdhip_tracker_check_overlap(lsdhip_tracker* t, const float* pos, int n, const double refToFrame[7], float* usage_out) {
  if (!t || !pos || n <= 0 || !refToFrame || !usage_out) return LSDHIP_E_ARG;
  lsdhip_ctx* c = t->ctx;
  LSD_CTX_LOCK(c);
  LsdTrackJobScope tjob_(c, true);
  if (tjob_.rc) return tjob_.rc;
  HIPCHK(hipSetDevice(c->device));
  int rc = upload_points(t, pos, nullptr, n);
  if (rc) return rc;
  lsdm::SE3fH T = lsdm::se3f_from_d(lsdm::se3d_from7(refToFrame));
  const int L = LSD_QUICK_KF_CHECK_LVL;
  EvalCtx a;
  memset(&a, 0, sizeof(a));
  const LevelIntr& in = c->intr[L];
  a.w = c->wl[L]; a.h = c->hl[L];
  a.fx = in.fx; a.fy = in.fy; a.cx = in.cx; a.cy = in.cy;
  lsdm::quatf_to_rot(T.q, a.R);
  a.t[0] = T.t[0]; a.t[1] = T.t[1]; a.t[2] = T.t[2];
  hipLaunchKernelGGL(k_overlap, dim3(1), dim3(256), 0, c->stream, t->d_pts, n, a, t->d_summary->sums);
  HIPCHK(hipStreamSynchronize(c->stream));
  t->pointUsage = t->h_summary->sums[0] / (float)n;
  *usage_out = t->pointUsage;
  return LSDHIP_OK;
}

extern "C" int lsdhip_devtest_se3f_lm_step(lsdhip_ctx* c, int n, const float* A, const float* b, const float* damp, const float* T,
                                           float* inc, float* Tn) {
  if (!c || n <= 0 || !A || !b || !damp || !T || !inc || !Tn) return LSDHIP_E_ARG;
  LSD_CTX_LOCK(c);
  HIPCHK(hipSetDevice(c->device));
  if (c->pipeline) { if (int rc = lsd_sync_all(c)) return rc; }
  const size_t nin = (size_t)n * (36 + 6 + 1 + 7), nout = (size_t)n * (6 + 7);
  LsdDevBuf buf;
  HIPCHK(hipMalloc(&buf.p, (nin + nout) * sizeof(float)));
  float* d = (float*)buf.p;
  float *dA = d, *db = dA + (size_t)n * 36, *ddamp = db + (size_t)n * 6, *dT = ddamp + n, *dinc = dT + (size_t)n * 7, *dTn = dinc + (size_t)n * 6;
  HIPCHK(hipMemcpyAsync(dA, A, (size_t)n * 36 * sizeof(float), hipMemcpyHostToDevice, c->stream));
  HIPCHK(hipMemcpyAsync(db, b, (size_t)n * 6 * sizeof(float), hipMemcpyHostToDevice, c->stream));
  HIPCHK(hipMemcpyAsync(ddamp, damp, (size_t)n * sizeof(float), hipMemcpyHostToDevice, c->stream));
  HIPCHK(hipMemcpyAsync(dT, T, (size_t)n * 7 * sizeof(float), hipMemcpyHostToDevice, c->stream));
  hipLaunchKernelGGL(k_devtest_se3f_lm_step, dim3(n), dim3(64), 0, c->stream, dA, db, ddamp, dT, dinc, dTn);
  HIPCHK(hipGetLastError());
  HIPCHK(hipMemcpyAsync(inc, dinc, (size_t)n * 6 * sizeof(float), hipMemcpyDeviceToHost, c->stream));
  HIPCHK(hipMemcpyAsync(Tn, dTn, (size_t)n * 7 * sizeof(float), hipMemcpyDeviceToHost, c->stream));
  HIPCHK(hipStreamSynchronize(c->stream));
  return LSDHIP_OK;
}
```

Measured before the change: 5508.

## Speculatively evaluate next pyramid level alongside current level's LM trials

New measurement: 5412. 0.983x the previous value.

```diff
diff --git a/lsd_slam_amd/csrc/lsdhip_internal.hpp b/lsd_slam_amd/csrc/lsdhip_internal.hpp
--- a/lsd_slam_amd/csrc/lsdhip_internal.hpp
+++ b/lsd_slam_amd/csrc/lsdhip_internal.hpp
@@ -78,7 +78,9 @@
   float aff_a0, aff_b0;
   int evalOnly;
   int trackFrameSemantics;
-};
+  int aheadLevels;
+};
+static_assert(sizeof(TrackJob) == LSD_LEVELS * sizeof(TrackLevel) + 8 + 20 * 4, "TrackJob: aheadLevels fills the tail padding (the batch kernels index an array of these)");
 struct TrackSpec {
   int specC;
   int specGrid;
@@ -99,6 +101,7 @@
 };
 
 #define LSD_SPEC_MAX 6
+#define LSD_SPEC_SLOTS (LSD_SPEC_MAX + 1)
 struct TrackState {
   lsdm::SE3fH T;
   lsdm::SE3fH Tn;
@@ -303,6 +306,7 @@
   int grid_cap = 304;
   int recent[4] = {0, 0, 0, 0};
   int specC = 6;
+  bool levelAhead = true;
   int soloMinJobs = -1;
   bool specAuto = true;
   int specCaps[LSD_LEVELS] = {0, 0, 0, 0, 0};
diff --git a/lsd_slam_amd/csrc/track_device.hpp b/lsd_slam_amd/csrc/track_device.hpp
--- a/lsd_slam_amd/csrc/track_device.hpp
+++ b/lsd_slam_amd/csrc/track_device.hpp
@@ -396,7 +396,8 @@
 }
 template <bool SPEC = false>
 __device__ __forceinline__ bool lm_wave(const LmPar& par, TrackState& S, const float col, float* tot, const int lane,
-                                        TrackSummary* out, unsigned long long* trp, const int consumed = 0, const int mycand = 0, const int doneWord = 1) {
+                                        TrackSummary* out, unsigned long long* trp, const int consumed = 0, const int mycand = 0, const int doneWord = 1,
+                                        bool* endedBySmallStep = nullptr) {
   float* const s_gj = tot - 48;
   S.lastCand = consumed;
   S.ncand = 1;
@@ -465,6 +466,7 @@
       const float i0 = S.inc[0], i1 = S.inc[1], i2 = S.inc[2], i3 = S.inc[3], i4 = S.inc[4], i5 = S.inc[5];
       const float incdot = (i0 * i0 + (i1 * i1 + i2 * i2)) + (i3 * i3 + (i4 * i4 + i5 * i5));
       if (!(incdot > L.stepSizeMin)) {
+        if (endedBySmallStep) *endedBySmallStep = true;
         iteration = maxIts;
         iteration++;
         start_iteration = true;
diff --git a/lsd_slam_amd/csrc/tracker.hip b/lsd_slam_amd/csrc/tracker.hip
--- a/lsd_slam_amd/csrc/tracker.hip
+++ b/lsd_slam_amd/csrc/tracker.hip
@@ -81,6 +81,7 @@
   __shared__ TrackState S;
   __shared__ LmShared sh;
   __shared__ LmPar s_par;
+  __shared__ LmPar s_parA;
   constexpr int NPASS = 1;
   constexpr int CPP = (RS_END + NPASS - 1) / NPASS;
   constexpr int RSLICE_ = BLOCK / CPP;
@@ -92,6 +93,8 @@
   const int wave = tid >> 6, lane = tid & 63;
   const int max_rows = sc.max_rows;
   int cand = 0, bx = (int)blockIdx.x;
+  bool aheadIn = false;
+  int nbA = 0, trA = 1, candA = 0;
   const bool leader = blockIdx.x == 0;
   const int cmax = sc.cmax;
   TrackState* next = st2 + (1 - parity);
@@ -105,10 +108,13 @@
   constexpr int NSLOT = 16;
   constexpr int TRIALS_MAX = BATCH ? (MODE == TS_EVAL ? 1 : LSD_BATCH_SPEC_MAX) : LSD_SPEC_MAX;
   constexpr bool SPEC_LM = MODE != TS_EVAL;
-  static_assert(TRIALS_MAX * (NSLOT * RS_COLS + 96 + 1) <= CPP * (BLOCK + 1) + 8, "the finishing phase's tables must fit the reduction buffer");
+  constexpr bool AHEAD_C = !BATCH && MODE == TS_FUSED;
+  constexpr int NTAB = TRIALS_MAX + (AHEAD_C ? 1 : 0);
+  constexpr int AH = TRIALS_MAX;
+  static_assert(NTAB * (NSLOT * RS_COLS + 96 + 1) <= CPP * (BLOCK + 1) + 8, "the finishing phase's tables must fit the reduction buffer");
   float (*const s_sumT)[NSLOT][RS_COLS] = (float (*)[NSLOT][RS_COLS])s_red;
-  float (*const s_subT)[3][32] = (float (*)[3][32])(s_red + TRIALS_MAX * NSLOT * RS_COLS);
-  int* const s_nsubT = (int*)(s_red + TRIALS_MAX * (NSLOT * RS_COLS + 96));
+  float (*const s_subT)[3][32] = (float (*)[3][32])(s_red + NTAB * NSLOT * RS_COLS);
+  int* const s_nsubT = (int*)(s_red + NTAB * (NSLOT * RS_COLS + 96));
   __shared__ float s_rec[TRIALS_MAX][32];
 #ifdef LSD_PHASE_TRACE
   __shared__ unsigned long long* s_trp;
@@ -153,7 +159,21 @@
     bx = (int)blockIdx.x - cand * nbl;
     const bool needTrial = S.pending ? cand < tr : cand == 0;
     const bool needNext = S.pending && lvlPending > job.lastLevel && (int)blockIdx.x < job.lv[lvlPending - 1].nblocks;
-    if (!leader && !needTrial && !needNext) return;
+    bool needAhead = false;
+    if (AHEAD_C && S.pending && ((job.aheadLevels >> lvlPending) & 1)) {
+      const int nbA_ = job.lv[lvlPending - 1].nblocks;
+      aheadIn = S.phase == 1;
+      nbA = nbA_;
+      trA = (spec.trials[lvlPending - 1] > 1) ? spec.trials[lvlPending - 1] : 1;
+      int most = tr * nbl + nbA_;
+      if (aheadIn) {
+        candA = (int)blockIdx.x / nbA_;
+        const int below = trA * nbA_ + (lvlPending - 1 > job.lastLevel ? job.lv[lvlPending - 2].nblocks : 0);
+        most = below > most ? below : most;
+      }
+      needAhead = (int)blockIdx.x < most;
+    }
+    if (!leader && !needTrial && !needNext && !needAhead) return;
   }
 
   if (BATCH && MODE == TS_LM) {
@@ -198,19 +218,22 @@
     const int level = S.level;
     const int nb = job.lv[level].nblocks;
     const size_t trialStrideF4 = (size_t)RS_COLS * max_rows / 4;
-      auto tail_two = [&](const int ca, const int cb, auto krn) {
+      auto tail_two = [&](const int ea, const int eb, auto krn) {
         constexpr int KROWS = decltype(krn)::value;
-        const int cbb = cb < 0 ? ca : cb;
-        const int4* tka = topkey_in0 + (size_t)ca * max_rows;
-        const int4* tkb = topkey_in0 + (size_t)cbb * max_rows;
+        const bool aheadA = AHEAD_C && ea >= ncandPending, aheadB = AHEAD_C && eb >= ncandPending;
+        const int ca = aheadA ? AH : ea, cb = aheadB ? AH : eb;
+        const int ma = aheadA ? cmax - 1 : ea, mb = aheadB ? cmax - 1 : (eb < 0 ? ma : eb);
+        const int nba = aheadA ? nbA : nb, nbb = aheadB ? nbA : nb;
+        const int4* tka = topkey_in0 + (size_t)ma * max_rows;
+        const int4* tkb = topkey_in0 + (size_t)mb * max_rows;
         int4 kva[KROWS], kvb[KROWS];
 #pragma unroll
         for (int q = 0; q < KROWS; q++) {
           const int row = lane + 64 * q;
           const int4 ka = tka[row < max_rows ? row : 0];
           const int4 kb = tkb[row < max_rows ? row : 0];
-          kva[q] = row < nb ? ka : make_int4(-1, -1, -1, -1);
-          kvb[q] = row < nb ? kb : make_int4(-1, -1, -1, -1);
+          kva[q] = row < nba ? ka : make_int4(-1, -1, -1, -1);
+          kvb[q] = row < nbb ? kb : make_int4(-1, -1, -1, -1);
         }
         auto merge = [&](const int4 (&kv)[KROWS], int (&keys)[3], int (&src)[3]) {
           int k0 = -1, k1 = -1, k2 = -1, e0 = 0, e1 = 0, e2 = 0;
@@ -238,19 +261,20 @@
           }
         };
         const bool single = job.lv[level].singlePass != 0 || job.lv[level].tilePx > 0;
+        const bool singleA = single || aheadA, singleB = single || aheadB;
         const int j = lane & 31, rj = lane >> 5;
         int keysA[3], srcA[3], keysB[3], srcB[3];
         float a0 = 0.f, a2 = 0.f, b0 = 0.f, b2 = 0.f;
         merge(kva, keysA, srcA);
-        if (single && j < 29) {
-          const float* tv = topval_in0 + (size_t)ca * max_rows * 96;
+        if (singleA && j < 29) {
+          const float* tv = topval_in0 + (size_t)ma * max_rows * 96;
           if (keysA[rj] >= 0) a0 = tv[(size_t)srcA[rj] * 32 + j];
           if (rj == 0 && keysA[2] >= 0) a2 = tv[(size_t)srcA[2] * 32 + j];
         }
         if (cb >= 0) {
           merge(kvb, keysB, srcB);
-          if (single && j < 29) {
-            const float* tv = topval_in0 + (size_t)cb * max_rows * 96;
+          if (singleB && j < 29) {
+            const float* tv = topval_in0 + (size_t)mb * max_rows * 96;
             if (keysB[rj] >= 0) b0 = tv[(size_t)srcB[rj] * 32 + j];
             if (rj == 0 && keysB[2] >= 0) b2 = tv[(size_t)srcB[2] * 32 + j];
           }
@@ -259,19 +283,27 @@
           s_nsubT[ca] = (keysA[0] >= 0) + (keysA[1] >= 0) + (keysA[2] >= 0);
           if (cb >= 0) s_nsubT[cb] = (keysB[0] >= 0) + (keysB[1] >= 0) + (keysB[2] >= 0);
         }
+        auto put_a = [&]() {
+          if (keysA[rj] >= 0) s_subT[ca][rj][j] = a0;
+          if (rj == 0 && keysA[2] >= 0) s_subT[ca][2][j] = a2;
+        };
+        auto put_b = [&]() {
+          if (keysB[rj] >= 0) s_subT[cb][rj][j] = b0;
+          if (rj == 0 && keysB[2] >= 0) s_subT[cb][2][j] = b2;
+        };
         if (single) {
           if (j < 29) {
-            if (keysA[rj] >= 0) s_subT[ca][rj][j] = a0;
-            if (rj == 0 && keysA[2] >= 0) s_subT[ca][2][j] = a2;
-            if (cb >= 0) {
-              if (keysB[rj] >= 0) s_subT[cb][rj][j] = b0;
-              if (rj == 0 && keysB[2] >= 0) s_subT[cb][2][j] = b2;
-            }
+            put_a();
+            if (cb >= 0) put_b();
           }
         } else {
+          if (AHEAD_C && j < 29) {
+            if (aheadA) put_a();
+            if (aheadB) put_b();
+          }
           const bool second = lane >= 3;
           const int r = second ? lane - 3 : lane;
-          const int c = second ? cb : ca;
+          const int c = second ? (aheadB ? -1 : cb) : (aheadA ? -1 : ca);
           int key = -1;
           if (lane < 6 && c >= 0) key = second ? (r == 0 ? keysB[0] : (r == 1 ? keysB[1] : keysB[2])) : (r == 0 ? keysA[0] : (r == 1 ? keysA[1] : keysA[2]));
           if (key >= 0) {
@@ -357,18 +389,21 @@
         if (cb >= 0) pick(vb, cb);
       };
     auto wave_tail = [&]() {
+      const int nEnt = ncandPending + ((AHEAD_C && aheadIn) ? 1 : 0);
+      const int nbMost = (AHEAD_C && aheadIn && nbA > nb) ? nbA : nb;
       const int ca = WAVES - 1 - wave;
-      const int cb = ca + WAVES < ncandPending ? ca + WAVES : -1;
-      if (ca < ncandPending) {
+      const int cb = ca + WAVES < nEnt ? ca + WAVES : -1;
+      if (ca < nEnt) {
         if (BATCH && job.lv[level].tilePx > 0 && nb <= 24) {
           if (nb <= 5) tail_rows(ca, cb, std::integral_constant<int, 2>());
           else if (nb <= 13) tail_rows(ca, cb, std::integral_constant<int, 5>());
           else tail_rows(ca, cb, std::integral_constant<int, 9>());
-        } else if (nb <= 128) tail_two(ca, cb, std::integral_constant<int, 2>());
+        } else if (nbMost <= 128) tail_two(ca, cb, std::integral_constant<int, 2>());
         else tail_two(ca, cb, std::integral_constant<int, 5>());
       }
     };
     if (tid == SUMW * 64 - 1) stage_lm_par(job, level, s_par, (spec.specC > 1 && spec.trials[level] > 1) ? spec.trials[level] : 1);
+    if (AHEAD_C && aheadIn && tid == SUMW * 64 - 2) stage_lm_par(job, level - 1, s_parA, trA);
     if (wave < SUMW) {
       const int t = tid;
       const int slot_ = t / (RS_COLS / 4);
@@ -405,6 +440,28 @@
             if (sumLane && base + c < ncandPending) *(float4*)&s_sumT[base + c][slot][c4 * 4] = a4;
           }
         };
+        constexpr int QA = 5;
+        const float4* pA = p + (size_t)(cmax - 1) * trialStrideF4;
+        const int KA = (nbA + NSLOT - 1) / NSLOT;
+        float4 vA[QA], aA4 = make_float4(0.f, 0.f, 0.f, 0.f);
+        auto ahead_load = [&](const int q0) {
+#pragma unroll
+          for (int q = 0; q < QA; q++) {
+            const int r = slot + NSLOT * (q0 + q);
+            vA[q] = pA[(size_t)(r < nbA ? r : slot) * (RS_COLS / 4)];
+          }
+        };
+        auto ahead_add = [&](const int q0) {
+#pragma unroll
+          for (int q = 0; q < QA; q++) {
+            const bool live = q0 + q < KA && slot + NSLOT * (q0 + q) < nbA;
+            aA4.x += live ? vA[q].x : 0.f;
+            aA4.y += live ? vA[q].y : 0.f;
+            aA4.z += live ? vA[q].z : 0.f;
+            aA4.w += live ? vA[q].w : 0.f;
+          }
+        };
+        int qDone = 0;
         typedef std::integral_constant<int, 1> I1;
         typedef std::integral_constant<int, 3> I3;
         typedef std::integral_constant<int, TRIALS_MAX> IM;
@@ -413,10 +470,18 @@
           else if (K <= 5) colsum(std::integral_constant<int, 5>(), I1(), 0);
           else if (K <= 10) colsum(std::integral_constant<int, 10>(), I1(), 0);
           else colsum(std::integral_constant<int, QMAX>(), I1(), 0);
-        } else if (K <= 2) colsum(std::integral_constant<int, 2>(), IM(), 0);
+        } else if (K <= 2) {
+          if (AHEAD_C && aheadIn) ahead_load(0);
+          colsum(std::integral_constant<int, 2>(), IM(), 0);
+          if (AHEAD_C && aheadIn) { ahead_add(0); qDone = QA; }
+        }
         else if (K <= 5) colsum(std::integral_constant<int, 5>(), IM(), 0);
         else if (K <= 10) { for (int base = 0; base < ncandPending; base += 3) colsum(std::integral_constant<int, 10>(), I3(), base); }
         else { for (int base = 0; base < ncandPending; base++) colsum(std::integral_constant<int, QMAX>(), I1(), base); }
+        if (AHEAD_C && aheadIn) {
+          for (int q0 = qDone; q0 < KA; q0 += QA) { ahead_load(q0); ahead_add(q0); }
+          if (sumLane) *(float4*)&s_sumT[AH][slot][c4 * 4] = aA4;
+        }
 #ifdef LSD_PHASE_TRACE
         if (trOn_ && tid == 0) tr_[17] = clock64();
 #endif
@@ -477,31 +542,39 @@
           if (tid < 3) S.t[tid] = rec[22 + tid];
         }
       }
-      {
-        float Mf = s_sumT[pc][0][RS_M];
-#pragma unroll
-        for (int k = 1; k < NSLOT; k++) Mf += s_sumT[pc][k][RS_M];
+      auto entry_totals = [&](const int e) {
+        float Mf = s_sumT[e][0][RS_M];
+#pragma unroll
+        for (int k = 1; k < NSLOT; k++) Mf += s_sumT[e][k][RS_M];
         float s = 0.f;
         if (tid < RS_END) {
-          s = s_sumT[pc][0][tid];
-#pragma unroll
-          for (int k = 1; k < NSLOT; k++) s += s_sumT[pc][k][tid];
+          s = s_sumT[e][0][tid];
+#pragma unroll
+          for (int k = 1; k < NSLOT; k++) s += s_sumT[e][k][tid];
         }
         const int M = (int)Mf;
         int need = M & 3;
-        if (need > s_nsubT[pc]) need = s_nsubT[pc];
+        if (need > s_nsubT[e]) need = s_nsubT[e];
         const int subIdx = (tid == RS_WERR) ? 0 : ((tid >= RS_A0 && tid < RS_B0) ? 1 + tid - RS_A0 : ((tid >= RS_B0 && tid < RS_ERR) ? 22 + tid - RS_B0 : (tid == RS_ERR ? 28 : -1)));
-        const float sub0 = s_subT[pc][0][subIdx < 0 ? 0 : subIdx], sub1 = s_subT[pc][1][subIdx < 0 ? 0 : subIdx], sub2 = s_subT[pc][2][subIdx < 0 ? 0 : subIdx];
+        const float sub0 = s_subT[e][0][subIdx < 0 ? 0 : subIdx], sub1 = s_subT[e][1][subIdx < 0 ? 0 : subIdx], sub2 = s_subT[e][2][subIdx < 0 ? 0 : subIdx];
         if (subIdx >= 0) {
           if (need > 0) s -= sub0;
           if (need > 1) s -= sub1;
           if (need > 2) s -= sub2;
         }
         if (tid < RS_NUM) sh.tot[tid] = s;
+        return s;
+      };
+      int e = pc, consumed = pc;
+      int mycand = (AHEAD_C && cand >= s_par.trials) ? 0 : cand;
+      const LmPar* par = &s_par;
+#pragma nounroll
+      for (int pass = 0;; pass++) {
+        const float s = entry_totals(e);
 #ifdef LSD_ORDER_CHECK
         if (!BATCH && spec.dbgCounters) {
           unsigned hv = tid < RS_END ? __float_as_uint(s) * (2654435761u * (unsigned)(tid + 1)) : 0u;
-          hv += (unsigned)pc * 97u;
+          hv += (unsigned)e * 97u;
           for (int off = 32; off > 0; off >>= 1) hv += __shfl_xor(hv, off);
           if (tid == 0) {
             const unsigned long long slot = 8 + 2 * ((spec.dbgCum / 400ull) % 8192ull);
@@ -511,12 +584,17 @@
         }
 #endif
         PHASE_MARK(3);
+        bool smallStep = false;
 #ifdef LSD_PHASE_TRACE
         if (trOn_ && tid == 0) { tr_[19] = (unsigned long long)ncandPending; tr_[7] = (unsigned long long)pc; }
-        lm_wave<SPEC_LM>(s_par, S, s, sh.tot, tid, leader ? out : nullptr, trOn_ ? tr_ : nullptr, pc, cand, doneWord);
+        lm_wave<SPEC_LM>(*par, S, s, sh.tot, tid, leader ? out : nullptr, trOn_ ? tr_ : nullptr, consumed, mycand, doneWord, AHEAD_C ? &smallStep : nullptr);
 #else
-        lm_wave<SPEC_LM>(s_par, S, s, sh.tot, tid, leader ? out : nullptr, nullptr, pc, cand, doneWord);
-#endif
+        lm_wave<SPEC_LM>(*par, S, s, sh.tot, tid, leader ? out : nullptr, nullptr, consumed, mycand, doneWord, AHEAD_C ? &smallStep : nullptr);
+#endif
+        if (!(AHEAD_C && pass == 0 && aheadIn && smallStep)) break;
+        e = AH; consumed = 0;
+        mycand = candA < trA ? candA : 0;
+        par = &s_parA;
       }
     }
     __syncthreads();
@@ -537,6 +615,10 @@
       LAUNCH_LOG(2, pendingIn_, ncandIn_, S.lastCand);
       return;
     }
+    if (AHEAD_C && S.level != level && S.phase == 1) {
+      cand = candA;
+      bx = (int)blockIdx.x - candA * nbA;
+    }
     if (cand > 0 && bx == 0 && S.phase == 1 && cand < S.ncand && tid < 25) {
       float v;
       if (tid < 6) v = S.inc[tid];
@@ -555,16 +637,29 @@
     return;
   }
 
-  const int level = S.level;
-  const int nb = job.lv[level].nblocks;
-  if (MODE == TS_FUSED && level != lvlPending) { cand = 0; bx = (int)blockIdx.x; }
+  int level = S.level;
+  int nb = job.lv[level].nblocks;
+  if (MODE == TS_FUSED && level != lvlPending && (!AHEAD_C || S.phase == 0)) { cand = 0; bx = (int)blockIdx.x; }
+  const bool ahead = AHEAD_C && S.phase == 1 && cand >= S.ncand && ((job.aheadLevels >> level) & 1);
+  int slotOut = cand;
+  if (ahead) {
+    bx = (int)blockIdx.x - S.ncand * nb;
+    level = level - 1;
+    nb = job.lv[level].nblocks;
+    slotOut = cmax - 1;
+    cand = 0;
+  }
   if (bx >= nb || cand >= S.ncand) return;
-  sums_out += (size_t)cand * RS_COLS * max_rows;
-  topkey_out += (size_t)cand * max_rows;
-  topval_out += (size_t)cand * max_rows * 96;
+  sums_out += (size_t)slotOut * RS_COLS * max_rows;
+  topkey_out += (size_t)slotOut * max_rows;
+  topval_out += (size_t)slotOut * max_rows * 96;
   const int tile = xcd_tile(bx, nb);
   EvalCtx a;
   make_ctx_dev(job, S, level, a);
+  if (ahead) {
+    lsdm::quatf_to_rot(S.T.q, a.R);
+    a.t[0] = S.T.t[0]; a.t[1] = S.T.t[1]; a.t[2] = S.T.t[2];
+  }
   if (BATCH && MODE == TS_EVAL && cand > 0) {
     const float* rec = sc.recs + ((size_t)parity * cmax + cand) * 32;
 #pragma unroll
@@ -1138,7 +1233,8 @@
   const size_t topkey = slots * RS_COLS * rows, topval = topkey + slots * 4 * rows, recs = topval + slots * 96 * rows;
   return {topkey, topval, recs, recs + slots * 32};
 }
-static_assert(scratch_layout(1, LSD_SPEC_MAX, 304).end * 4 == (size_t)LSD_SPEC_MAX * (2 * RS_COLS * 304 * 4 + 2 * 304 * 16 + 2 * 304 * 96 * 4 + 2 * 32 * 4) &&
+static_assert(LSD_SPEC_SLOTS == LSD_SPEC_MAX + 1 &&
+              scratch_layout(1, LSD_SPEC_SLOTS, 304).end * 4 == (size_t)(LSD_SPEC_MAX + 1) * (2 * RS_COLS * 304 * 4 + 2 * 304 * 16 + 2 * 304 * 96 * 4 + 2 * 32 * 4) &&
               scratch_layout(8, LSD_BATCH_SPEC_MAX, 304).end * 4 == 8 * (size_t)LSD_BATCH_SPEC_MAX * (2 * RS_COLS * 304 * 4 + 2 * 304 * 16 + 2 * 304 * 96 * 4 + 2 * 32 * 4) &&
               scratch_layout(8, LSD_BATCH_SPEC_MAX, 304).recs == 8 * (size_t)LSD_BATCH_SPEC_MAX * (2 * RS_COLS * 304 + 2 * 4 * 304 + 2 * 96 * 304),
               "scratch arena: byte count and offsets");
@@ -1179,10 +1275,11 @@
     if (t->grid_cap > 80 * nslice) t->grid_cap = (80 * nslice) & ~7;
   }
   t->max_blocks = t->grid_cap;
-  const size_t partials_bytes = scratch_layout(1, LSD_SPEC_MAX, (size_t)t->max_blocks).end * sizeof(float);
+  const size_t partials_bytes = scratch_layout(1, LSD_SPEC_SLOTS, (size_t)t->max_blocks).end * sizeof(float);
   if (const char* e = getenv("LSDHIP_SPEC")) t->specC = atoi(e);
   if (t->specC < 1) t->specC = 1;
   if (t->specC > LSD_SPEC_MAX) t->specC = LSD_SPEC_MAX;
+  if (const char* e = getenv("LSDHIP_LEVEL_AHEAD")) t->levelAhead = atoi(e) != 0;
   if (const char* e = getenv("LSDHIP_SPEC_CAP")) t->specCap = atoi(e) & ~7;
   if (const char* e = getenv("LSDHIP_SPEC_CAPS")) {
     int v[LSD_LEVELS] = {0, 0, 0, 0, 0};
@@ -1433,6 +1530,13 @@
   L.writeMask = 0;
   return LSDHIP_OK;
 }
+static int ahead_levels(const lsdhip_tracker* t, const TrackJob& job) {
+  int mask = 0;
+  if (!t->levelAhead || t->spec.specC <= 1) return 0;
+  for (int l = job.lastLevel + 1; l <= job.topLevel; l++)
+    if (t->spec.trials[l] > 1 && job.lv[l - 1].singlePass != 0 && job.lv[l - 1].writeMask == 0 && job.lv[l - 1].tilePx == 0) mask |= 1 << l;
+  return mask;
+}
 static void fill_job_common(lsdhip_tracker* t, TrackJob& job) {
   lsdhip_ctx* c = t->ctx;
   LSD_CTX_LOCK(c);
@@ -1468,7 +1572,7 @@
          t->lastGoodCount / (t->lastGoodCount + t->lastBadCount) > MIN_GOODPERGOODBAD_PIXEL;
 }
 
-static TrackScratch scratch_of(lsdhip_tracker* t) { return scratch_at(t, t->d_partials, 1, LSD_SPEC_MAX, LSD_SPEC_MAX); }
+static TrackScratch scratch_of(lsdhip_tracker* t) { return scratch_at(t, t->d_partials, 1, LSD_SPEC_SLOTS, LSD_SPEC_SLOTS); }
 static void launch_step(lsdhip_tracker* t, const TrackJob& job, int grid, int parity, int first) {
   lsdhip_ctx* c = t->ctx;
   LSD_CTX_LOCK(c);
@@ -1492,7 +1596,8 @@
   t->spec.specGrid = 0;
   if (t->spec.specC > 1) {
     for (int l = job.lastLevel; l <= job.topLevel; l++) {
-      const int g = job.lv[l].nblocks * (t->spec.trials[l] > 1 ? t->spec.trials[l] : 1);
+      int g = job.lv[l].nblocks * (t->spec.trials[l] > 1 ? t->spec.trials[l] : 1);
+      if ((job.aheadLevels >> l) & 1) g += job.lv[l - 1].nblocks;
       if (g > grid) grid = g;
     }
     t->spec.specGrid = grid;
@@ -1736,6 +1841,7 @@
       }
     }
   }
+  job.aheadLevels = ahead_levels(t, job);
   t->h_summary->done = 0;
   const TrackSummary* S = t->h_summary;
   const long long myEpoch = ++c->enqEpoch;
@@ -1811,9 +1917,9 @@
         const int nb = job.lv[topLevel].nblocks;
         t->dumpL0.assign((size_t)nb * (RS_COLS + 4 + 96) + sizeof(TrackState) / 4, 0u);
         unsigned* d = t->dumpL0.data();
-        HIPCHK(hipMemcpy(d, sc.sums + (size_t)(1 * LSD_SPEC_MAX + 0) * RS_COLS * rows, (size_t)nb * RS_COLS * 4, hipMemcpyDeviceToHost));
-        HIPCHK(hipMemcpy(d + (size_t)nb * RS_COLS, sc.topkey + (size_t)(1 * LSD_SPEC_MAX + 0) * rows, (size_t)nb * 16, hipMemcpyDeviceToHost));
-        HIPCHK(hipMemcpy(d + (size_t)nb * (RS_COLS + 4), sc.topval + (size_t)(1 * LSD_SPEC_MAX + 0) * rows * 96, (size_t)nb * 96 * 4, hipMemcpyDeviceToHost));
+        HIPCHK(hipMemcpy(d, sc.sums + (size_t)(1 * LSD_SPEC_SLOTS + 0) * RS_COLS * rows, (size_t)nb * RS_COLS * 4, hipMemcpyDeviceToHost));
+        HIPCHK(hipMemcpy(d + (size_t)nb * RS_COLS, sc.topkey + (size_t)(1 * LSD_SPEC_SLOTS + 0) * rows, (size_t)nb * 16, hipMemcpyDeviceToHost));
+        HIPCHK(hipMemcpy(d + (size_t)nb * (RS_COLS + 4), sc.topval + (size_t)(1 * LSD_SPEC_SLOTS + 0) * rows * 96, (size_t)nb * 96 * 4, hipMemcpyDeviceToHost));
         HIPCHK(hipMemcpy(d + (size_t)nb * (RS_COLS + 4 + 96), t->d_state + 1, sizeof(TrackState), hipMemcpyDeviceToHost));
       }
     }
```
